# Rorisis/Co-Occ

Measured on AMD Instinct MI355X. Metric: samples/sec (6-cam frame + sweep -> occ+render), 200x200x16 grid, higher is better.
Workload: dtype f32 (split-f16 products, fp32 accumulate)

## Files before the change

co_occ_amd/_lib.py:

```python
import ctypes
import os
import threading
import time

import torch

_HERE = os.path.dirname(os.path.abspath(__file__))
LIB_PATH = os.path.join(_HERE, "libcoocc_hip.so")

c_int, c_float, c_void_p, c_size_t, c_int64 = (ctypes.c_int, ctypes.c_float, ctypes.c_void_p,
                                               ctypes.c_size_t, ctypes.c_int64)


class ConvDesc(ctypes.Structure):
    _fields_ = [(n, c_void_p) for n in ("in_", "w", "out", "scale", "bias", "res", "gather", "out_rows", "ws")] + \
               [("ws_floats", c_int64)] + \
               [(n, c_int) for n in ("M", "Cin", "Cout", "taps", "in_stride", "out_stride", "res_stride",
                                     "B", "Xi", "Yi", "Zi", "Xo", "Yo", "Zo", "ksize", "stride", "pad",
                                     "relu", "res_mode", "splitk", "tile_hint", "kx", "ky", "kz", "px", "py", "pz",
                                     "wgroup_rows", "mfma_dtype")] + [("alpha", ctypes.c_float), ("M_dev", c_void_p), ("gather_stride", c_int), ("out16", c_void_p), ("out16_stride", c_int), ("out_h2", c_int),
                                                                   ("out_h2_twin", c_void_p), ("tile_sem", c_void_p), ("tile_sem_ints", c_int),
                                                                  ("alpha_dev", c_void_p), ("sx", c_int), ("sy", c_int), ("sz", c_int)]


class SearchDesc(ctypes.Structure):
    _fields_ = [("cat4", c_void_p), ("pts", c_void_p), ("pts_rows", c_int), ("pts_stride", c_int)] + \
               [(n, c_int) for n in ("C", "X", "Y", "Z", "K", "fps_num", "max_cluster")] + \
               [("radius", ctypes.c_float), ("dist_thresh", ctypes.c_float), ("offsets", c_void_p), ("noff", c_int)] + \
               [(n, c_void_p) for n in ("lin", "counts", "near_img", "near_pts", "rows", "rows_p", "ws")] + \
               [("ws_bytes", ctypes.c_size_t), ("counts_host", c_void_p)]


P, I, F, Z, L = c_void_p, c_int, c_float, c_size_t, c_int64
SIGNATURES = {
    "coocc_last_error": (ctypes.c_char_p, []),
    "coocc_abi_version": (I, []),
    "coocc_device_cu_count": (I, [P]),
    "coocc_stream_create_cu_mask": (I, [P, I, P]),
    "coocc_stream_destroy": (I, [P]),
    "coocc_event_create": (I, [I, P]),
    "coocc_event_destroy": (I, [P]),
    "coocc_event_record": (I, [P, P]),
    "coocc_stream_wait_event": (I, [P, P]),
    "coocc_event_synchronize": (I, [P]),
    "coocc_event_query": (I, [P]),
    "coocc_event_elapsed_ms": (I, [P, P, P]),
    "coocc_ncdhw_to_ndhwc": (I, [P, P, I, I, I, I, I, P]),
    "coocc_rows_to_bf16": (I, [P, I, L, I, P, P]),
    "coocc_rows_to_h2": (I, [P, I, L, I, F, P, P]),
    "coocc_rows_to_h2_ex": (I, [P, I, L, I, F, P, P, P]),
    "coocc_rows_to_h2_gather": (I, [P, I, P, L, P, I, F, P, P]),
    "coocc_rows_to_f16": (I, [P, I, L, I, P, P]),
    "coocc_wino_input_h2": (I, [P, I, I, I, I, I, I, I, P, I, L, F, P]),
    "coocc_wino_input_h2_ex": (I, [P, I, I, I, I, I, I, I, P, I, L, F, P, P]),
    "coocc_ndhwc_to_ncdhw": (I, [P, P, I, I, I, I, I, P]),
    "coocc_fuser_prepare": (I, [P, P, P, P, P, I, I, I, P]),
    "coocc_fuser_prepare_rows": (I, [P, I, I, P, I, I, P, P, P, I, I, I, P]),
    "coocc_compact_flags": (I, [P, I, P, P, P, Z, P]),
    "coocc_compact_flags_ex": (I, [P, I, P, P, P, P, Z, P]),
    "coocc_lin_to_coords": (I, [P, I, I, I, I, P, P, P]),
    "coocc_furthest_point_sampling": (I, [I, I, I, P, P, P, P]),
    "coocc_fps_voxels_ws": (Z, [I, I, I]),
    "coocc_fps_voxels": (I, [P, I, I, I, I, I, P, P, Z, P]),
    "coocc_fps_voxels_pair": (I, [P, I, P, P, P, I, P, P, Z, I, I, I, I, P]),
    "coocc_ball_query": (I, [I, I, I, F, F, I, P, P, P, P]),
    "coocc_knn_topk": (I, [I, I, I, P, P, P, P, P]),
    "coocc_voxel_index_map": (I, [P, I, I, P, P]),
    "coocc_voxel_index_map_dev": (I, [P, I, P, I, P, P]),
    "coocc_fine_sample_voxel_dev": (I, [P, I, I, I, I, P, I, P, I, P, P, P, I, P]),
    "coocc_fine_sample_img_dev": (I, [P, I, I, I, I, P, P, L, P, P, I, I, P]),
    "coocc_fine_mlp_pre_dev": (I, [P, I, P, I, L, P, I, P, P, P, F, P, P, P, P, F, P, P, I, P, P]),
    "coocc_fine_fused": (I, [P, I, I, I, P, I, I, I, P, P, I, P, I, P, P, P, P, F, P, P, P, P, F, P, P, I, P, P, P]),
    "coocc_fine2_pack": (I, [P, P, I, P, P, P, P, P, P, P, P, P, P]),
    "coocc_fine2_h2": (I, [P, I, I, I, I, P, I, I, I, P, P, I, P, P, P, P, F, F, I, P, P, P, P]),
    "coocc_fine_sample_img_lin": (I, [P, I, I, I, I, P, P, I, I, I, P, P, I, I, P]),
    "coocc_scatter_fine_dev": (I, [P, L, P, I, I, I, P, P, I, I, I, F, P]),
    "coocc_scatter_fine_grouped": (I, [P, I, I, P, I, P, I, I, I, I, P, F, P, P]),
    "coocc_ball_query_voxels": (I, [I, F, F, I, I, I, I, P, P, P, P, P]),
    "coocc_knn_topk_voxels": (I, [I, I, I, I, I, I, P, P, P, P, I, P, P, P, P, P]),
    "coocc_knn_assign": (I, [I, I, I, I, F, P, P, P, P, P, P]),
    "coocc_knn_threshold": (I, [I, F, P, P, P, P]),
    "coocc_index_rows_i32": (I, [P, I, P, I, P, P]),
    "coocc_conv_pack_weights": (L, [P, I, I, I, I, P]),
    "coocc_conv_fwd": (I, [ctypes.POINTER(ConvDesc), P]),
    "coocc_fuser_search_ws": (Z, [ctypes.POINTER(SearchDesc)]),
    "coocc_fuser_search": (I, [ctypes.POINTER(SearchDesc), P, P]),
    "coocc_upsample_add_trilinear": (I, [P, P, I, I, I, I, I, I, I, I, P]),
    "coocc_upsample_add_trilinear_ex": (I, [P, P, I, I, I, I, I, I, I, I, P, P]),
    "coocc_occhead_mix": (I, [P, P, I, P, P, I, I, P]),
    "coocc_occhead_mix_ex": (I, [P, P, I, P, P, I, I, P, P]),
    "coocc_argmax_flags": (I, [P, I, I, I, I, P, P]),
    "coocc_fine_sample_voxel": (I, [P, I, I, I, I, P, I, I, P, P, P, I, P]),
    "coocc_fine_sample_img": (I, [P, I, I, I, I, P, P, L, P, I, I, P]),
    "coocc_fine_mlp_pre": (I, [P, I, P, I, L, P, P, P, F, P, P, P, P, F, P, P, I, P, P]),
    "coocc_fine_mlp": (I, [P, I, P, I, L, P, P, P, P, F, P, P, P, P, F, P, P, I, P, P]),
    "coocc_groupnorm_rows": (I, [P, L, I, I, I, P, P, F, I, P]),
    "coocc_groupnorm_nhwc": (I, [P, I, I, I, I, P, P, F, I, P]),
    "coocc_scatter_fine": (I, [P, L, I, I, P, P, I, I, I, F, P]),
    "coocc_camera_mats": (I, [P, P, P, P, P, P, I, I, I, I, P, P]),
    "coocc_get_geometry": (I, [P, P, P, P, I, I, I, I, P, P]),
    "coocc_bev_pool_forward": (I, [P, P, P, P, I, I, I, I, I, I, I, P, P]),
    "coocc_bev_pool_backward": (I, [P, P, P, P, I, I, I, I, I, I, I, P, P]),
    "coocc_voxel_pool_ws": (Z, [I, I]),
    "coocc_voxel_pool": (I, [P, P, I, I, I, P, I, I, I, I, P, I, P, Z, I, P]),
    "coocc_lift_splat": (I, [P, P, P, I, I, I, I, I, I, P, I, I, I, I, P, I, P, Z, I, P]),
    "coocc_lift_splat_cams": (I, [P, P, P, P, P, P, I, I, I, I, I, I, P, I, I, I, I, P, I, P, Z, I, P]),
    "coocc_lift_splat_reuse": (I, [P, P, I, I, I, I, I, I, I, I, I, P, I, P, Z, P]),
    "coocc_bev_pool_coords": (I, [P, P, I, I, I, I, I, I, P, I, P, Z, I, P]),
    "coocc_render_nearest": (I, [P, I, I, I, P, P, I, I, I, I, P, I, P, P]),
    "coocc_render_nearest_cams": (I, [P, I, I, I, P, P, P, P, P, I, I, I, I, P, I, P, P]),
    "coocc_render_activate_table": (I, [P, I, P]),
    "coocc_upsample_maps": (I, [P, I, I, I, I, P, P, P]),
    "coocc_volume_sampling": (I, [P, I, I, I, I, P, I, P, P, P, P]),
    "coocc_raw2outputs": (I, [P, P, I, I, I, F, F, P, P, P, P]),
    "coocc_render_losses": (I, [P, P, P, P, L, I, P, P, Z, P]),
    "coocc_conv_pack_weights_dev": (L, [P, I, I, I, I, P, P]),
    "coocc_wino_pack_weights_dev": (L, [P, I, I, I, I, P, P]),
    "coocc_wino_pack_weights_h2_dev": (L, [P, I, I, I, I, P, P]),
    "coocc_conv_pack_weights_h2_dev": (L, [P, I, I, I, I, P, P]),
    "coocc_wino_gradout": (I, [P, I, I, I, I, I, I, I, P, L, P]),
    "coocc_wino_ztap_table": (I, [L, I, P, P]),
    "coocc_wino_wgrad": (I, [P, P, L, I, I, I, I, P, P, I, P, L, P]),
    "coocc_rows_to_kh2": (I, [P, I, L, L, I, F, P, P, P]),
    "coocc_wino_operand_kh2": (I, [I, P, I, I, I, I, I, I, I, P, L, F, P, P]),
    "coocc_conv_wgrad_h2": (I, [P, P, L, I, I, F, P, P, I, P, L, P]),
    "coocc_wino_wgrad_h2": (I, [P, P, L, I, I, I, I, F, P, P, I, P, L, P]),
    "coocc_conv_tap_table": (I, [I, I, I, I, I, I, I, I, I, I, I, P, P]),
    "coocc_conv_epilogue_bwd": (I, [P, I, P, I, P, I, I, I, P, I, P, I, I, P, I, P, L, P]),
    "coocc_conv_epilogue_bwd_ex": (I, [P, I, P, I, P, I, I, I, P, I, P, I, I, P, I, P, L, P, P, F, P]),
    "coocc_conv_wgrad": (I, [P, I, I, P, I, P, I, I, I, I, P, I, P, L, P]),
    "coocc_conv_wgrad_h2t": (I, [P, I, I, P, I, P, I, I, I, I, P, P, I, P, L, P]),
    "coocc_gather_rows": (I, [P, I, P, I, I, P, I, P]),
    "coocc_scatter_add_rows": (I, [P, I, P, I, I, P, I, P]),
    "coocc_voxel_pool_bwd": (I, [P, I, P, I, I, I, P, I, I, I, I, P, P]),
    "coocc_lift_splat_bwd": (I, [P, I, P, P, P, I, I, I, I, I, I, P, I, I, I, I, P, P, P]),
    "coocc_render_nearest_bwd": (I, [P, I, I, I, P, P, I, I, I, I, P, P, P, P]),
    "coocc_upsample_maps_bwd": (I, [P, P, I, I, I, I, P, P]),
    "coocc_render_losses_bwd": (I, [P, P, P, P, L, I, P, P, P, P, P]),
    "coocc_upsample_trilinear_bwd": (I, [P, P, I, I, I, I, I, I, I, I, I, P]),
    "coocc_wino_input": (I, [P, I, I, I, I, I, I, I, P, L, P]),
    "coocc_wino_input_strided": (I, [P, I, I, I, I, I, I, I, P, I, L, P]),
    "coocc_sparse_tap_sum": (I, [P, P, I, I, I, I, I, P, P, I, I, P]),
    "coocc_wino_output": (I, [P, L, I, I, I, I, I, I, P, I, P, P, P, I, I, P]),
    "coocc_wino_output_ex": (I, [P, L, I, I, I, I, I, I, P, I, P, P, P, I, I, P, P]),
    "coocc_h2_overflow": (I, [I]),
    "coocc_device_fault": (I, [I]),
    "coocc_render_heads_h2": (I, [P, I, I, I, P, P, P, P, P, P, I, P, P, P, I, P]),
    "coocc_projection_params": (I, [P, P, P, P, P, P, I, P, P, P]),
    "coocc_occhead_mix_bwd": (I, [P, P, I, P, P, P, P, I, I, P]),
    "coocc_fine_sample_voxel_bwd": (I, [P, I, I, I, I, I, P, L, P, P, P]),
    "coocc_groupnorm_rows_bwd": (I, [P, P, P, L, I, I, I, P, F, I, P, P, P, P]),
    "coocc_fine_sample_img_bwd": (I, [P, I, I, I, I, I, P, P, L, P, P]),
    "coocc_groupnorm_nhwc_bwd": (I, [P, P, P, I, I, I, I, P, F, I, P, P, P, P]),
    "coocc_voxelize_ws": (Z, [I]),
    "coocc_voxelize_hard": (I, [P, I, I, P, P, I, I, P, P, P, P, P, Z, P]),
    "coocc_vfe_mean": (I, [P, P, I, I, I, I, P, I, P]),
    "coocc_sparse_index_map": (I, [P, I, I, I, I, P, P]),
    "coocc_sparse_conv_table": (I, [P, I, I, I, I, I, I, I, P, P, P]),
    "coocc_sparse_down_flags": (I, [P, I, I, I, I, I, I, I, P, P]),
    "coocc_sparse_conv_table3": (I, [P, I, I, I, I, I, I, I, I, I, I, I, I, I, P, P, P]),
    "coocc_sparse_down_flags3": (I, [P, I, I, I, I, I, I, I, I, I, I, I, I, I, I, I, I, P, P]),
    "coocc_sparse_lin_to_coors": (I, [P, I, I, I, I, P, P, P]),
    "coocc_bn_stats": (I, [P, I, I, I, P, P, P, Z, P]),
    "coocc_bn_apply": (I, [P, I, I, P, P, P, P, F, P, I, P, P]),
    "coocc_bn_backward": (I, [P, P, P, I, I, P, P, P, F, I, P, P, P, P, P, Z, P]),
    "coocc_bn_backward_sums": (I, [P, P, P, I, I, P, P, F, I, P, P, P, Z, P]),
    "coocc_bn_backward_dx": (I, [P, P, P, I, I, P, P, P, F, I, P, P, ctypes.c_double, P, P, P]),
    "coocc_predict_labels": (I, [P, L, L, L, L, I, I, I, I, I, I, I, P, P]),
    "coocc_eval_semantic": (I, [P, L, L, L, L, I, I, I, I, P, P, I, I, I, I, I, P, P]),
    "coocc_fpn_sum": (I, [P, P, I, I, I, I, I, I, P, I, P, P]),
    "coocc_zyx_to_rows": (I, [P, P, I, I, I, I, I, I, I, P]),
    "coocc_conv_tap_table3": (I, [I] * 17 + [P, P]),
    "coocc_fpn_sum_bwd": (I, [P, I, P, P, I, I, I, I, I, I, P]),
    "coocc_lidarseg_points": (I, [P, L, L, L, L, I, I, I, I, P, L, L, I, I, P, I, I, P, P, I, P, P]),
    "coocc_render_eval_stats": (L, [P, P, P, P, I, I, I, P, P, Z, P]),
    "coocc_render_panels": (I, [P, P, P, P, I, I, I, P, P]),
    "coocc_render_eval_ssim": (L, [P, P, I, I, I, ctypes.c_double, P, P, Z, P]),
    "coocc_sparse_dgrad_table3": (I, [P] + [I] * 16 + [P, P, P, P]),
    "coocc_bn_apply_ex": (I, [P, I, I, P, P, P, P, F, P, I, P, P, P]),
    "coocc_pool_labels": (I, [P, I, I, I, I, I, I, I, P, P]),
    "coocc_occ_loss_ws": (Z, [L, I]),
    "coocc_occ_loss_fwd": (I, [P, L, I, I, P, P, I, I, I, P, P, I, P, P, P, P, Z, P]),
    "coocc_occ_loss_bwd": (I, [P, L, I, I, P, P, I, P, P, P, P, I, P]),
    "coocc_nbr_table2d": (I, [I, I, I, I, P, P]),
    "coocc_dcn_cols": (I, [P, I, P, I, I, I, I, I, I, I, I, P, P]),
    "coocc_se_gate2": (I, [P, I, I, I, I, P, P, P, P, P]),
    "coocc_cam_mean_ws": (Z, [I, I, I]),
    "coocc_cam_mean": (I, [P, I, I, I, I, P, P, Z, P]),
    "coocc_cam_bias_relu": (I, [P, I, I, I, I, P, I, P]),
    "coocc_dcn_cols_bwd": (I, [P, I, P, I, I, I, I, I, I, I, I, P, P, P, P]),
    "coocc_se_gate2_bwd_ws": (Z, [I, I, I]),
    "coocc_se_gate2_bwd": (I, [P, I, I, I, I, P, P, P, P, P, P, P, P, Z, P]),
    "coocc_cam_sum": (I, [P, I, I, I, I, P, P, Z, P]),
    "coocc_cam_add": (I, [P, P, I, I, I, P, F, P]),
    "coocc_dropout_rows": (I, [P, P, L, I, F, P, P]),
    "coocc_img_stem": (I, [P, I, I, I, P, P, P, I, I, I, P, I, P, P]),
}

_lib = None


class KernelTimer:

    def __init__(self):
        self.enabled = False
        self.only = None
        self.records = []

    class _Region:
        def __init__(self, owner, tag, work):
            self.o, self.tag, self.work = owner, tag, work

        def __enter__(self):
            lvl = int(self.o.enabled)
            self.on = lvl >= 2 or (lvl == 1 and self.work > 0 and (self.o.only is None or self.tag.startswith(self.o.only)))
            if self.on:
                self.s = torch.cuda.Event(enable_timing=True)
                self.e = torch.cuda.Event(enable_timing=True)
                self.s.record()
            return self

        def __exit__(self, *a):
            if self.on:
                self.e.record()
                self.o.records.append((self.tag, self.work, self.s, self.e))
            return False

    def region(self, tag, work=0.0):
        return KernelTimer._Region(self, tag, work)

    def summary(self):
        out = {}
        for tag, work, s, e in self.records:
            d = out.setdefault(tag, dict(launches=0, ms=0.0, work=0.0))
            d["launches"] += 1
            d["ms"] += s.elapsed_time(e)
            d["work"] += work
        return out

    def reset(self):
        self.records = []


TIMER = KernelTimer()



def load():
    global _lib
    if _lib is not None:
        return _lib
    if not os.path.exists(LIB_PATH):
        raise ImportError(
            "co_occ_amd: %s is missing -- build it with `python -c 'import __graft_entry__ as g; g.build()'` "
            "(hipcc --offload-arch=gfx950).  There is no CPU fallback." % LIB_PATH)
    lib = ctypes.CDLL(LIB_PATH)
    for name, (res, args) in SIGNATURES.items():
        fn = getattr(lib, name)
        fn.restype, fn.argtypes = res, args
    if os.environ.get("COOCC_FPS_THREADS"):
        lib.coocc_fps_voxels_set_threads(int(os.environ["COOCC_FPS_THREADS"]))
    _lib = lib
    return lib


class CooccError(RuntimeError):
    code = None


class CooccArgError(CooccError):
    """COOCC_EINVAL / COOCC_ENOMEM: the library REFUSED the call (an argument or shape an entry point does not take, a
    workspace that is too small) before launching anything -- nothing ran, the caller may take another route."""


class CooccRangeError(CooccError):
    """The split-f16 engine's range guard fired (``core.check_h2_overflow``): kernels ran and their result is not trustworthy.
    Never a reason to fall back silently."""


def check(rc):
    if rc != 0:
        cls = CooccArgError if rc in (-1, -3) else CooccError
        e = cls("libcoocc_hip: %s (code %d)" % (load().coocc_last_error().decode(), rc))
        e.code = rc
        raise e


def _device_of(args):
    for a in args:
        t = getattr(a, "_keep", None)
        if t is not None:
            return t.device
    return None


_fns = {}


def call(name, *args):
    fn = _fns.get(name)
    if fn is None:
        fn = _fns[name] = getattr(load(), name)
    dev = _device_of(args)
    if dev is not None and dev.index != torch.cuda.current_device():
        with torch.cuda.device(dev):
            with TIMER.region(name):
                check(fn(*args, stream(dev)))
        return
    if not TIMER.enabled:
        rc = fn(*args, stream(dev))
        if rc:
            check(rc)
        return
    with TIMER.region(name):
        check(fn(*args, stream(dev)))


def conv_fwd(desc, device):
    fn = load().coocc_conv_fwd
    if device.index != torch.cuda.current_device():
        with torch.cuda.device(device):
            check(fn(ctypes.byref(desc), stream(device)))
    else:
        check(fn(ctypes.byref(desc), stream(device)))


_raw_stream = getattr(torch._C, "_cuda_getCurrentRawStream", None)


def stream(device=None):
    if _raw_stream is not None:
        idx = device.index if device is not None and device.index is not None else torch.cuda.current_device()
        return c_void_p(_raw_stream(idx))
    return c_void_p(torch.cuda.current_stream(device).cuda_stream)


class DevPtr(ctypes.c_void_p):
    """c_void_p that keeps its tensor alive until the foreign call has been issued, so that
    temporaries such as ``ptr(x.contiguous())`` cannot be recycled by the caching allocator
    while later arguments of the same call are still being built."""


def ptr(t, dtype=None, strided=False, offset=0):
    if t is None:
        return c_void_p(0)
    if not t.is_cuda:
        raise CooccError("co_occ_amd ops run on the GPU only; got a %s tensor (no CPU fallback)" % t.device)
    if dtype is not None and t.dtype != dtype:
        raise CooccError("expected %s, got %s" % (dtype, t.dtype))
    if not strided and not t.is_contiguous():
        raise CooccError("tensor must be contiguous")
    p = DevPtr(t.data_ptr() + offset * t.element_size())
    p._keep = t
    return p


_blocked = threading.local()


def host_read(t):
    t0 = time.perf_counter()
    v = t.tolist()
    _blocked.s = getattr(_blocked, "s", 0.0) + time.perf_counter() - t0
    return v


def blocked_seconds():
    return getattr(_blocked, "s", 0.0)


def host_f32(vals):
    return (c_float * len(vals))(*[float(v) for v in vals])


def host_i32(vals):
    return (c_int * len(vals))(*[int(v) for v in vals])
```

co_occ_amd/csrc/knn.hip:

```cpp
#include "common.h"

typedef unsigned long long u64;

__device__ __forceinline__ u64 shfl_xor_u64(u64 v, int m) {
  unsigned lo = (unsigned)v, hi = (unsigned)(v >> 32);
  lo = __shfl_xor(lo, m);
  hi = __shfl_xor(hi, m);
  return ((u64)hi << 32) | lo;
}
template <int CTRL>
__device__ __forceinline__ u64 dpp_u64(u64 v) {
  int lo = (int)(unsigned)v, hi = (int)(unsigned)(v >> 32);
  lo = __builtin_amdgcn_update_dpp(lo, lo, CTRL, 0xF, 0xF, false);
  hi = __builtin_amdgcn_update_dpp(hi, hi, CTRL, 0xF, 0xF, false);
  return ((u64)(unsigned)hi << 32) | (unsigned)lo;
}
__device__ __forceinline__ u64 readlane_u64(u64 v, int l) {
  unsigned lo = __builtin_amdgcn_readlane((int)(unsigned)v, l);
  unsigned hi = __builtin_amdgcn_readlane((int)(unsigned)(v >> 32), l);
  return ((u64)hi << 32) | lo;
}
#define U64MAX(a, b) ((a) > (b) ? (a) : (b))
#define U64MIN(a, b) ((a) < (b) ? (a) : (b))
__device__ __forceinline__ u64 wave_max_u64(u64 v) {
// ... 300 lines not shown
    }
    sx = gl & 1023; sy = (gl >> 10) & 1023; sz = gl >> 20;
    if (tid == 0) {
      const unsigned rr = (unsigned)(rmask - (g & rmask));
      const unsigned hi = rr / (unsigned)q, lo = rr - hi * (unsigned)q;
      const unsigned rev = L ? (__brev(hi) >> (32 - L)) : 0u;
      idx[j] = (int)((lo << L) | rev);
    }
    if (dbg) { long long c4 = clock64(); tA += c1 - c0; tM += c2 - c1; tB += c3 - c2; tT += c4 - c3; }
  }
  if (dbg && lane == 0) {
    long long* o = dbg + wave * 8;
    o[0] = tA; o[1] = tM; o[2] = tB; o[3] = tT; o[4] = 0; o[5] = nd;
  }
}

#define FPSR_SLOTS 40
struct FpsRegProblem { const int32_t* lin; const FpsCell* cell; int32_t* idx; int n, L, q, RB; };
struct FpsRegArgs { FpsRegProblem p[2]; int m, Y, Z, NBY, NBZ, NB; long long* dbg; };

__global__ __launch_bounds__(1024) void k_fps_voxels_reg(FpsRegArgs a) {
  constexpr int NW = 16;
  __builtin_amdgcn_s_setprio(3);
  __shared__ unsigned wbest[2][NW];
  __shared__ int wloc[2][NW];
  const FpsRegProblem pr = a.p[blockIdx.x];
  const int tid = threadIdx.x, lane = tid & 63, wave = __builtin_amdgcn_readfirstlane(tid >> 6);
  const int RB = pr.RB, Y = a.Y, Z = a.Z, NB = a.NB, m = a.m;
  const unsigned rmask = (1u << RB) - 1u;
  const unsigned tmax = (1u << (32 - RB)) - 1u;
  long long* dbg = a.dbg;
  long long tA = 0, tM = 0, tB = 0, tT = 0, nd = 0;

  typedef unsigned u32x32 __attribute__((ext_vector_type(32)));
  typedef unsigned u32x8 __attribute__((ext_vector_type(8)));
  u32x32 ca0, ca1;
  u32x8 cb0, cb1;
  unsigned key = 0;
  int org = 0, pos = 0;
  {
    const int b = lane * NW + wave;
    if (lane < FPSR_SLOTS && b < NB) {
      int bz = b % a.NBZ; int qq = b / a.NBZ;
      org = ((qq / a.NBY) * FT_X) | (((qq % a.NBY) * FT_Y) << 10) | ((bz * FT_Z) << 20);
    }
  }
#pragma unroll
  for (int i = 0; i < FPSR_SLOTS; ++i) {
    const int b = i * NW + wave;
    unsigned k0 = 0, k1 = 0;
    if (b < NB) {
      const int r0 = pr.cell[(size_t)b * FT_P + lane].r, r1 = pr.cell[(size_t)b * FT_P + lane + 64].r;
      k0 = r0 >= 0 ? ((tmax << RB) | (rmask - (unsigned)r0)) : 0u;
      k1 = r1 >= 0 ? ((tmax << RB) | (rmask - (unsigned)r1)) : 0u;
      const unsigned best = max(k0, k1);
      const int bp = k1 > k0 ? lane + 64 : lane;
      const unsigned wb = wave_max_key(best);
      const u64 own = __ballot(best == wb);
      const int wp = __builtin_amdgcn_readlane(bp, (int)__ffsll((long long)own) - 1);
      if (lane == i) { key = wb; pos = wp; }
    }
    if (i < 32) { ca0[i] = k0; ca1[i] = k1; }
    else { cb0[i - 32] = k0; cb1[i - 32] = k1; }
  }
  if (tid == 0) pr.idx[0] = 0;
  int sx, sy, sz;
  {
    int l = pr.lin[0];
    sz = l % Z; l /= Z;
    sy = l % Y; sx = l / Y;
  }

  for (int j = 1; j < m; ++j) {
    long long c0 = dbg ? clock64() : 0;
    bool d = false;
    if (key) {
      const int x0 = org & 1023, y0 = (org >> 10) & 1023, z0 = org >> 20;
      const int dx = max(max(x0 - sx, sx - (x0 + FT_X - 1)), 0);
      const int dy = max(max(y0 - sy, sy - (y0 + FT_Y - 1)), 0);
      const int dz = max(max(z0 - sz, sz - (z0 + FT_Z - 1)), 0);
      d = (unsigned)(__mul24(dx, dx) + __mul24(dy, dy) + __mul24(dz, dz)) < (key >> RB);
    }
    u64 bal = __ballot(d);
    nd += __popcll(bal);
    const int exb = (lane >> 5) - sx, eyb = ((lane >> 3) & 3) - sy, ezb = (lane & 7) - sz;
    while (bal) {
      const int s0 = __builtin_amdgcn_readfirstlane((int)__ffsll((long long)bal) - 1);
      bal &= bal - 1;
      const int o = __builtin_amdgcn_readlane(org, s0);
      const int ex = (o & 1023) + exb, ey = ((o >> 10) & 1023) + eyb, ez = (o >> 20) + ezb;
      const int yz = __mul24(ey, ey) + __mul24(ez, ez);
      const unsigned d0 = (unsigned)(__mul24(ex, ex) + yz), d1 = (unsigned)(__mul24(ex + 2, ex + 2) + yz);
      unsigned k0, k1;
      if (s0 < 32) { k0 = ca0[s0]; k1 = ca1[s0]; }
      else { k0 = cb0[s0 - 32]; k1 = cb1[s0 - 32]; }
      if (k0) k0 = (min(d0, k0 >> RB) << RB) | (k0 & rmask);
      if (k1) k1 = (min(d1, k1 >> RB) << RB) | (k1 & rmask);
      if (s0 < 32) { ca0[s0] = k0; ca1[s0] = k1; }
      else { cb0[s0 - 32] = k0; cb1[s0 - 32] = k1; }
      const unsigned best = max(k0, k1);
      const int bp = k1 > k0 ? lane + 64 : lane;
      const unsigned wb = wave_max_key(best);
      const int wp = __builtin_amdgcn_readlane(bp, (int)__ffsll((long long)__ballot(best == wb)) - 1);
      if (lane == s0) { key = wb; pos = wp; }
    }
    long long c1 = dbg ? clock64() : 0;
    const int loc = org + (pos >> 5) + (((pos >> 3) & 3) << 10) + ((pos & 7) << 20);
    const unsigned wb = wave_max_key(key);
    if (key == wb && wb) { wbest[j & 1][wave] = wb; wloc[j & 1][wave] = loc; }
    if (!wb && lane == 0) wbest[j & 1][wave] = 0;
    long long c2 = dbg ? clock64() : 0;
    lds_barrier();
    long long c3 = dbg ? clock64() : 0;
    const int li = lane & 15;
    const unsigned mine = wbest[j & 1][li];
    const int ml = wloc[j & 1][li];
    unsigned v = mine;
    v = max(v, dpp_u32<0xB1>(v));
    v = max(v, dpp_u32<0x4E>(v));
    v = max(v, dpp_u32<0x141>(v));
    v = max(v, dpp_u32<0x140>(v));
    const unsigned g = (unsigned)__builtin_amdgcn_readfirstlane((int)v);
    const u64 own = __ballot(mine == g) & 0xFFFFull;
    const int gl = __builtin_amdgcn_readlane(ml, (int)__ffsll((long long)own) - 1);
    sx = gl & 1023; sy = (gl >> 10) & 1023; sz = gl >> 20;
    if (tid == 0) pr.idx[j] = (int)(g & rmask);
    if (dbg) { long long c4 = clock64(); tA += c1 - c0; tM += c2 - c1; tB += c3 - c2; tT += c4 - c3; }
  }
  __syncthreads();
  for (int j = 1 + tid; j < m; j += 1024) {
    const unsigned rr = rmask - (unsigned)pr.idx[j];
    const unsigned hi = rr / (unsigned)pr.q, lo = rr - hi * (unsigned)pr.q;
    const unsigned rev = pr.L ? (__brev(hi) >> (32 - pr.L)) : 0u;
    pr.idx[j] = (int)((lo << pr.L) | rev);
  }
  if (dbg && lane == 0 && blockIdx.x == 0) {
    long long* o = dbg + wave * 8;
    o[0] = tA; o[1] = tM; o[2] = tB; o[3] = tT; o[4] = 0; o[5] = nd;
  }
}

extern "C" size_t coocc_fps_voxels_ws(int X, int Y, int Z) {
  size_t nb = (size_t)((X + FT_X - 1) / FT_X) * ((Y + FT_Y - 1) / FT_Y) * ((Z + FT_Z - 1) / FT_Z);
  return nb * FT_P * sizeof(FpsCell);
}

static int g_fps_threads = 1024;
static long long* g_fps_dbg = nullptr;
extern "C" void coocc_fps_voxels_set_debug(long long* p) { g_fps_dbg = p; }
extern "C" void coocc_fps_voxels_set_threads(int t) { g_fps_threads = t; }

struct FpsPrep { int NBX, NBY, NBZ, L, q, RB, tinit, threads, R; long long NB; bool key32; };

static int fps_prepare(const int32_t* lin, int n, int X, int Y, int Z, int m, const int32_t* idx, void* ws, size_t ws_bytes,
                       hipStream_t s, FpsPrep* o) {
  COOCC_CHECK_ARG(lin && idx && ws && n > 0 && m >= 0 && X > 0 && Y > 0 && Z > 0, "fps_voxels: bad args");
  COOCC_CHECK_ARG(n < (1 << FPS_KBITS), "fps_voxels: n must be < 2^22");
  COOCC_CHECK_ARG(X <= 1020 && Y <= 1020 && Z <= 1016, "fps_voxels: grid dims must fit 10-bit packed coordinates");
  o->NBX = (X + FT_X - 1) / FT_X; o->NBY = (Y + FT_Y - 1) / FT_Y; o->NBZ = (Z + FT_Z - 1) / FT_Z;
  o->NB = (long long)o->NBX * o->NBY * o->NBZ;
  int threads = g_fps_threads;
  while (o->NB > 8ll * threads && threads < 1024) threads *= 2;
  COOCC_CHECK_ARG(o->NB <= 8ll * threads, "fps_voxels: grid has too many buckets (use coocc_furthest_point_sampling)");
  if (ws_bytes < coocc_fps_voxels_ws(X, Y, Z)) return coocc_set_error(COOCC_ENOMEM, "fps_voxels: workspace too small");
  o->threads = threads;
  o->R = (int)((o->NB + threads - 1) / threads);
  int L = 0;
  while ((2 << L) <= n && L < 10) ++L;
  const int q = (n + (1 << L) - 1) >> L;
  int RB = L;
  while ((1ll << RB) <= ((long long)q << L)) ++RB;
  const long long d2max = (long long)(X - 1) * (X - 1) + (long long)(Y - 1) * (Y - 1) + (long long)(Z - 1) * (Z - 1);
  o->key32 = RB < 31 && d2max + 1 < (1ll << (32 - RB)) - 1;
  o->tinit = o->key32 ? (int)((1u << (32 - RB)) - 1u) : 0x7FFFFFFF;
  o->L = L; o->q = q; o->RB = RB;
  if (m == 0) return COOCC_OK;
  FpsCell* cell = (FpsCell*)ws;
  COOCC_HIP(hipMemsetAsync(cell, 0xFF, sizeof(FpsCell) * (size_t)o->NB * FT_P, s));
  hipLaunchKernelGGL(k_fpsv_scatter, dim3(cdiv(n, 256)), dim3(256), 0, s, lin, n, Y, Z, o->NBY, o->NBZ, L, q, o->tinit, cell);
  COOCC_LAUNCH_CHECK("k_fpsv_scatter");
  return COOCC_OK;
}

static int g_fps_reg = -1;
static bool fps_reg_ok(const FpsPrep& o) {
  if (g_fps_reg < 0) g_fps_reg = getenv("COOCC_FPS_REG") ? atoi(getenv("COOCC_FPS_REG")) : 1;
  return g_fps_reg && o.key32 && o.NB <= (long long)FPSR_SLOTS * 16;
}

extern "C" int coocc_fps_voxels(const int32_t* lin, int n, int X, int Y, int Z, int m, int32_t* idx, void* ws,
                                size_t ws_bytes, void* stream) {
  hipStream_t s = as_stream(stream);
  FpsPrep o;
  int rc = fps_prepare(lin, n, X, Y, Z, m, idx, ws, ws_bytes, s, &o);
  if (rc != COOCC_OK || m == 0) return rc;
  FpsCell* cell = (FpsCell*)ws;
  const int NBY = o.NBY, NBZ = o.NBZ, L = o.L, q = o.q, RB = o.RB, R = o.R, threads = o.threads;
  const long long NB = o.NB;
  const bool key32 = o.key32;
  if (fps_reg_ok(o)) {
    FpsRegArgs a = {};
    a.p[0] = FpsRegProblem{lin, cell, idx, n, L, q, RB};
    a.m = m; a.Y = Y; a.Z = Z; a.NBY = NBY; a.NBZ = NBZ; a.NB = (int)NB; a.dbg = g_fps_dbg;
    hipLaunchKernelGGL(k_fps_voxels_reg, dim3(1), dim3(1024), 0, s, a);
    COOCC_LAUNCH_CHECK("k_fps_voxels_reg");
    return COOCC_OK;
  }
#define FPS_LAUNCH(T, RM, KT) \
  hipLaunchKernelGGL((k_fps_voxels<T, RM, KT>), dim3(1), dim3(T), 0, s, n, m, Y, Z, NBY, NBZ, (int)NB, lin, cell, idx, L, q, \
                     key32 ? RB : 32, g_fps_dbg)
#define FPS_PICK_R(T, KT)                     \
  do {                                        \
    if (R <= 2) FPS_LAUNCH(T, 2, KT);         \
    else if (R <= 3) FPS_LAUNCH(T, 3, KT);    \
    else if (R <= 4) FPS_LAUNCH(T, 4, KT);    \
    else if (R <= 5) FPS_LAUNCH(T, 5, KT);    \
    else if (R <= 6) FPS_LAUNCH(T, 6, KT);    \
    else FPS_LAUNCH(T, 8, KT);                \
  } while (0)
#define FPS_PICK(T)                           \
  do {                                        \
    if (key32) FPS_PICK_R(T, unsigned);       \
    else FPS_PICK_R(T, u64);                  \
  } while (0)
  if (threads == 256) FPS_PICK(256);
  else if (threads == 512) FPS_PICK(512);
  else FPS_PICK(1024);
  COOCC_LAUNCH_CHECK("k_fps_voxels");
  return COOCC_OK;
}

extern "C" int coocc_fps_voxels_pair(const int32_t* lin0, int n0, int32_t* idx0, void* ws0, const int32_t* lin1, int n1, int32_t* idx1,
                                     void* ws1, size_t ws_bytes_each, int X, int Y, int Z, int m, void* stream) {
  COOCC_CHECK_ARG(X > 0 && Y > 0 && Z > 0 && n0 > 0 && n1 > 0, "fps_voxels_pair: bad args");
  {
    const long long NB = (long long)((X + FT_X - 1) / FT_X) * ((Y + FT_Y - 1) / FT_Y) * ((Z + FT_Z - 1) / FT_Z);
    if (NB > (long long)FPSR_SLOTS * 16) return 2;
    const long long d2max = (long long)(X - 1) * (X - 1) + (long long)(Y - 1) * (Y - 1) + (long long)(Z - 1) * (Z - 1);
    for (int n : {n0, n1}) {
      int L = 0;
      while ((2 << L) <= n && L < 10) ++L;
      const int q = (n + (1 << L) - 1) >> L;
      int RB = L;
      while ((1ll << RB) <= ((long long)q << L)) ++RB;
      if (!(RB < 31 && d2max + 1 < (1ll << (32 - RB)) - 1)) return 2;
    }
    if (g_fps_reg < 0) g_fps_reg = getenv("COOCC_FPS_REG") ? atoi(getenv("COOCC_FPS_REG")) : 1;
    if (!g_fps_reg) return 2;
  }
  hipStream_t s = as_stream(stream);
  FpsPrep o0, o1;
  int rc = fps_prepare(lin0, n0, X, Y, Z, m, idx0, ws0, ws_bytes_each, s, &o0);
  if (rc != COOCC_OK) return rc;
  rc = fps_prepare(lin1, n1, X, Y, Z, m, idx1, ws1, ws_bytes_each, s, &o1);
  if (rc != COOCC_OK || m == 0) return rc;
  FpsRegArgs a = {};
  a.p[0] = FpsRegProblem{lin0, (const FpsCell*)ws0, idx0, n0, o0.L, o0.q, o0.RB};
  a.p[1] = FpsRegProblem{lin1, (const FpsCell*)ws1, idx1, n1, o1.L, o1.q, o1.RB};
  a.m = m; a.Y = Y; a.Z = Z; a.NBY = o0.NBY; a.NBZ = o0.NBZ; a.NB = (int)o0.NB; a.dbg = g_fps_dbg;
  hipLaunchKernelGGL(k_fps_voxels_reg, dim3(2), dim3(1024), 0, s, a);
  COOCC_LAUNCH_CHECK("k_fps_voxels_reg");
  return COOCC_OK;
}

__global__ __launch_bounds__(256) void k_ball_query(int n, int m, float min_r2, float max_r2, int nsample,
                                                     const float* __restrict__ new_xyz_all,
                                                     const float* __restrict__ xyz_all,
                                                     int32_t* __restrict__ idx_all) {
  const int lane = threadIdx.x & 63;
  const int c = blockIdx.x * 4 + (threadIdx.x >> 6);
  if (c >= m) return;
  const float* new_xyz = new_xyz_all + ((size_t)blockIdx.y * m + c) * 3;
  const float* xyz = xyz_all + (size_t)blockIdx.y * n * 3;
  int32_t* idx = idx_all + ((size_t)blockIdx.y * m + c) * nsample;
  const float cx = new_xyz[0], cy = new_xyz[1], cz = new_xyz[2];
  int cnt = 0, first = 0;
  for (int base = 0; base < n && cnt < nsample; base += 64) {
    int k = base + lane;
    bool hit = false;
    if (k < n) {
      float d2 = sqdist3(xyz[k * 3 + 0], xyz[k * 3 + 1], xyz[k * 3 + 2], cx, cy, cz);
      hit = (d2 == 0.f) || (d2 >= min_r2 && d2 < max_r2);
    }
    u64 bal = __ballot(hit);
    if (bal) {
      if (cnt == 0) first = base + (int)__ffsll((long long)bal) - 1;
      int slot = cnt + __popcll(bal & ((1ull << lane) - 1ull));
      if (hit && slot < nsample) idx[slot] = k;
      cnt += __popcll(bal);
    }
  }
  if (cnt > nsample) cnt = nsample;
  for (int l = cnt + lane; l < nsample; l += 64) idx[l] = first;
}

extern "C" int coocc_ball_query(int b, int n, int m, float min_radius, float max_radius, int nsample,
                                const float* new_xyz, const float* xyz, int32_t* idx, void* stream) {
  COOCC_CHECK_ARG(new_xyz && xyz && idx && b > 0 && n > 0 && m > 0 && nsample > 0, "ball_query: bad args");
  dim3 grid(cdiv(m, 4), b);
  hipLaunchKernelGGL(k_ball_query, grid, dim3(256), 0, as_stream(stream), n, m, min_radius * min_radius,
                     max_radius * max_radius, nsample, new_xyz, xyz, idx);
  COOCC_LAUNCH_CHECK("k_ball_query");
  return COOCC_OK;
}

template <int K>
__global__ __launch_bounds__(256) void k_knn_topk(int nq, int nk, const float* __restrict__ q,
                                                   const float* __restrict__ key, float* __restrict__ val,
                                                   int32_t* __restrict__ idx) {
  const int lane = threadIdx.x & 63;
  const int r = blockIdx.x * 4 + (threadIdx.x >> 6);
  if (r >= nq) return;
  const float qx = q[r * 3 + 0], qy = q[r * 3 + 1], qz = q[r * 3 + 2];
  u64 best[K];
#pragma unroll
  for (int j = 0; j < K; ++j) best[j] = ~0ull;
  for (int k = lane; k < nk; k += 64) {
    float d2 = sqdist3(qx, qy, qz, key[k * 3 + 0], key[k * 3 + 1], key[k * 3 + 2]);
    u64 kk = ((u64)__float_as_uint(d2) << 32) | (unsigned)k;
    if (kk < best[K - 1]) {
      best[K - 1] = kk;
#pragma unroll
      for (int j = K - 1; j > 0; --j) {
        if (best[j] < best[j - 1]) { u64 t = best[j]; best[j] = best[j - 1]; best[j - 1] = t; }
      }
    }
  }
#pragma unroll
  for (int o = 0; o < K; ++o) {
    u64 mn = wave_min_u64(best[0]);
    if (best[0] == mn) {
#pragma unroll
      for (int j = 0; j < K - 1; ++j) best[j] = best[j + 1];
      best[K - 1] = ~0ull;
    }
    if (lane == 0) {
      val[(size_t)r * K + o] = (float)__dsqrt_rn((double)__uint_as_float((unsigned)(mn >> 32)));
      idx[(size_t)r * K + o] = (int32_t)(unsigned)mn;
    }
  }
}

extern "C" int coocc_knn_topk(int nq, int nk, int K, const float* q, const float* key, float* val,
                              int32_t* idx, void* stream) {
  COOCC_CHECK_ARG(q && key && val && idx && nq > 0 && nk > 0, "knn_topk: bad args");
  COOCC_CHECK_ARG(K >= 1 && K <= 8 && K <= nk, "knn_topk: need 1 <= K <= min(8, nk)");
  dim3 grid(cdiv(nq, 4)), block(256);
  hipStream_t s = as_stream(stream);
  switch (K) {
    case 1: hipLaunchKernelGGL(k_knn_topk<1>, grid, block, 0, s, nq, nk, q, key, val, idx); break;
    case 2: hipLaunchKernelGGL(k_knn_topk<2>, grid, block, 0, s, nq, nk, q, key, val, idx); break;
    case 3: hipLaunchKernelGGL(k_knn_topk<3>, grid, block, 0, s, nq, nk, q, key, val, idx); break;
    case 4: hipLaunchKernelGGL(k_knn_topk<4>, grid, block, 0, s, nq, nk, q, key, val, idx); break;
    case 5: hipLaunchKernelGGL(k_knn_topk<5>, grid, block, 0, s, nq, nk, q, key, val, idx); break;
    case 6: hipLaunchKernelGGL(k_knn_topk<6>, grid, block, 0, s, nq, nk, q, key, val, idx); break;
    case 7: hipLaunchKernelGGL(k_knn_topk<7>, grid, block, 0, s, nq, nk, q, key, val, idx); break;
    default: hipLaunchKernelGGL(k_knn_topk<8>, grid, block, 0, s, nq, nk, q, key, val, idx); break;
  }
  COOCC_LAUNCH_CHECK("k_knn_topk");
  return COOCC_OK;
}

__global__ __launch_bounds__(256) void k_index_map_scatter(const int32_t* __restrict__ lin, int n, int32_t* __restrict__ map,
                                                            const int32_t* __restrict__ n_dev) {
  if (n_dev) n = min(n, *n_dev);
  int i = blockIdx.x * blockDim.x + threadIdx.x;
  if (i < n) map[lin[i]] = i;
}

__global__ __launch_bounds__(256) void k_fill_i32(int32_t* __restrict__ p, int n, int32_t v) {
  const int i = blockIdx.x * blockDim.x + threadIdx.x;
  if (i < n) p[i] = v;
}

extern "C" int coocc_voxel_index_map_dev(const int32_t* lin, int n_cap, const int32_t* n_dev, int nvox, int32_t* map, void* stream) {
  COOCC_CHECK_ARG(map && nvox > 0 && n_cap > 0 && lin && n_dev, "voxel_index_map_dev: bad args");
  static const bool fill_kernel = !(getenv("COOCC_MAP_MEMSET") && atoi(getenv("COOCC_MAP_MEMSET")) == 1);
  if (fill_kernel) hipLaunchKernelGGL(k_fill_i32, dim3(cdiv(nvox, 256)), dim3(256), 0, as_stream(stream), map, nvox, -1);
  else COOCC_HIP(hipMemsetAsync(map, 0xFF, (size_t)nvox * 4, as_stream(stream)));
  hipLaunchKernelGGL(k_index_map_scatter, dim3(cdiv(n_cap, 256)), dim3(256), 0, as_stream(stream), lin, n_cap, map, n_dev);
  COOCC_LAUNCH_CHECK("k_index_map_scatter");
  return COOCC_OK;
}

extern "C" int coocc_voxel_index_map(const int32_t* lin, int n, int nvox, int32_t* map, void* stream) {
  COOCC_CHECK_ARG(map && nvox > 0 && n >= 0 && (lin || n == 0), "voxel_index_map: bad args");
  COOCC_HIP(hipMemsetAsync(map, 0xFF, (size_t)nvox * 4, as_stream(stream)));
  if (n) {
    hipLaunchKernelGGL(k_index_map_scatter, dim3(cdiv(n, 256)), dim3(256), 0, as_stream(stream), lin, n, map, (const int32_t*)nullptr);
    COOCC_LAUNCH_CHECK("k_index_map_scatter");
  }
  return COOCC_OK;
}

__global__ __launch_bounds__(256) void k_ball_query_vox(int m, float min_r2, float max_r2, int R, int nsample, int X, int Y, int Z,
                                                         const int32_t* __restrict__ centre_ord, const int32_t* __restrict__ lin_q,
                                                         const int32_t* __restrict__ map_q, int32_t* __restrict__ idx_all) {
  const int lane = threadIdx.x & 63;
  const int c = blockIdx.x * 4 + (threadIdx.x >> 6);
  if (c >= m) return;
  int32_t* idx = idx_all + (size_t)c * nsample;
  const int v0 = lin_q[centre_ord[c]];
  const int cz = v0 % Z, cy = (v0 / Z) % Y, cx = v0 / (Z * Y);
  const int x0 = max(cx - R, 0), x1 = min(cx + R, X - 1);
  const int y0 = max(cy - R, 0), y1 = min(cy + R, Y - 1);
  const int z0 = max(cz - R, 0), z1 = min(cz + R, Z - 1);
  const int wy = y1 - y0 + 1, wz = z1 - z0 + 1;
  const int total = (x1 - x0 + 1) * wy * wz;
  int cnt = 0, first = 0;
  for (int base = 0; base < total && cnt < nsample; base += 64) {
    const int t = base + lane;
    bool hit = false;
    int ord = -1;
    if (t < total) {
      const int iz = z0 + t % wz, r = t / wz;
      const int iy = y0 + r % wy, ix = x0 + r / wy;
      ord = map_q[(ix * Y + iy) * Z + iz];
      const float d2 = sqdist3((float)ix, (float)iy, (float)iz, (float)cx, (float)cy, (float)cz);
      hit = ord >= 0 && ((d2 == 0.f) || (d2 >= min_r2 && d2 < max_r2));
    }
    const u64 bal = __ballot(hit);
    if (bal) {
      if (cnt == 0) first = __shfl(ord, (int)__ffsll((long long)bal) - 1);
      const int slot = cnt + __popcll(bal & ((1ull << lane) - 1ull));
      if (hit && slot < nsample) idx[slot] = ord;
      cnt += __popcll(bal);
    }
  }
  if (cnt > nsample) cnt = nsample;
  for (int l = cnt + lane; l < nsample; l += 64) idx[l] = first;
}

extern "C" int coocc_ball_query_voxels(int m, float min_radius, float max_radius, int nsample, int X, int Y, int Z,
                                       const int32_t* centre_ord, const int32_t* lin_q, const int32_t* map_q, int32_t* idx,
                                       void* stream) {
  COOCC_CHECK_ARG(m > 0 && nsample > 0 && X > 0 && Y > 0 && Z > 0 && centre_ord && lin_q && map_q && idx, "ball_query_voxels: bad args");
  COOCC_CHECK_ARG(max_radius >= 0.f && max_radius < 4096.f, "ball_query_voxels: bad radius");
  const float max_r2 = max_radius * max_radius;
  int R = (int)ceilf(max_radius);
  while (R > 0 && (float)(R * R) >= max_r2) --R;
  hipLaunchKernelGGL(k_ball_query_vox, dim3(cdiv(m, 4)), dim3(256), 0, as_stream(stream), m, min_radius * min_radius, max_r2, R,
                     nsample, X, Y, Z, centre_ord, lin_q, map_q, idx);
  COOCC_LAUNCH_CHECK("k_ball_query_vox");
  return COOCC_OK;
}

template <int K>
__global__ __launch_bounds__(256) void k_knn_topk_vox(int nq, int X, int Y, int Z, const int32_t* __restrict__ rep_ord,
                                                       const int32_t* __restrict__ lin_q, const int32_t* __restrict__ map_k,
                                                       const uint32_t* __restrict__ offsets, int noff, float* __restrict__ val,
                                                       int32_t* __restrict__ idx) {
  const int lane = threadIdx.x & 63;
  const int r = blockIdx.x * 4 + (threadIdx.x >> 6);
  if (r >= nq) return;
  const int v0 = lin_q[rep_ord[r]];
  const int cz = v0 % Z, cy = (v0 / Z) % Y, cx = v0 / (Z * Y);
  int found = 0;
  for (int base = 0; base < noff && found < K; base += 64) {
    const int t = base + lane;
    int ord = -1;
    float d2 = 0.f;
    if (t < noff) {
      const uint32_t o = offsets[t];
      const int dx = (int)(o & 255u) - 128, dy = (int)((o >> 8) & 255u) - 128, dz = (int)((o >> 16) & 255u) - 128;
      const int ix = cx + dx, iy = cy + dy, iz = cz + dz;
      if ((unsigned)ix < (unsigned)X && (unsigned)iy < (unsigned)Y && (unsigned)iz < (unsigned)Z) {
        ord = map_k[(ix * Y + iy) * Z + iz];
        d2 = sqdist3((float)cx, (float)cy, (float)cz, (float)ix, (float)iy, (float)iz);
      }
    }
    const u64 bal = __ballot(ord >= 0);
    const int p = found + __popcll(bal & ((1ull << lane) - 1ull));
    if (ord >= 0 && p < K) {
      val[(size_t)r * K + p] = (float)__dsqrt_rn((double)d2);
      idx[(size_t)r * K + p] = ord;
    }
    found += __popcll(bal);
  }
  if (found < K && lane == 0) idx[(size_t)r * K] = -2;
}

template <int K>
__global__ __launch_bounds__(256) void k_knn_topk_unresolved(int nq, int nk, const float* __restrict__ q,
                                                              const float* __restrict__ key, float* __restrict__ val,
                                                              int32_t* __restrict__ idx) {
  const int lane = threadIdx.x & 63;
  const int r = blockIdx.x * 4 + (threadIdx.x >> 6);
  if (r >= nq || idx[(size_t)r * K] != -2) return;
  const float qx = q[r * 3 + 0], qy = q[r * 3 + 1], qz = q[r * 3 + 2];
  u64 best[K];
#pragma unroll
  for (int j = 0; j < K; ++j) best[j] = ~0ull;
  for (int k = lane; k < nk; k += 64) {
    float d2 = sqdist3(qx, qy, qz, key[k * 3 + 0], key[k * 3 + 1], key[k * 3 + 2]);
    u64 kk = ((u64)__float_as_uint(d2) << 32) | (unsigned)k;
    if (kk < best[K - 1]) {
      best[K - 1] = kk;
#pragma unroll
      for (int j = K - 1; j > 0; --j) {
        if (best[j] < best[j - 1]) { u64 t = best[j]; best[j] = best[j - 1]; best[j - 1] = t; }
      }
    }
  }
#pragma unroll
  for (int o = 0; o < K; ++o) {
    u64 mn = wave_min_u64(best[0]);
    if (best[0] == mn) {
#pragma unroll
      for (int j = 0; j < K - 1; ++j) best[j] = best[j + 1];
      best[K - 1] = ~0ull;
    }
    if (lane == 0) {
      val[(size_t)r * K + o] = (float)__dsqrt_rn((double)__uint_as_float((unsigned)(mn >> 32)));
      idx[(size_t)r * K + o] = (int32_t)(unsigned)mn;
    }
  }
}

template <int K>
static void launch_topk_vox(int nq, int nk, int X, int Y, int Z, const int32_t* rep_ord, const int32_t* lin_q, const int32_t* map_k,
                            const uint32_t* offsets, int noff, const float* q, const float* key, float* val, int32_t* idx,
                            hipStream_t s) {
  hipLaunchKernelGGL(k_knn_topk_vox<K>, dim3(cdiv(nq, 4)), dim3(256), 0, s, nq, X, Y, Z, rep_ord, lin_q, map_k, offsets, noff, val, idx);
  hipLaunchKernelGGL(k_knn_topk_unresolved<K>, dim3(cdiv(nq, 4)), dim3(256), 0, s, nq, nk, q, key, val, idx);
}

extern "C" int coocc_knn_topk_voxels(int nq, int nk, int K, int X, int Y, int Z, const int32_t* rep_ord, const int32_t* lin_q,
                                     const int32_t* map_k, const uint32_t* offsets, int noff, const float* q, const float* key,
                                     float* val, int32_t* idx, void* stream) {
  COOCC_CHECK_ARG(nq > 0 && nk > 0 && X > 0 && Y > 0 && Z > 0 && rep_ord && lin_q && map_k && offsets && noff > 0 && q && key &&
                      val && idx, "knn_topk_voxels: bad args");
  COOCC_CHECK_ARG(K >= 1 && K <= 8 && K <= nk, "knn_topk_voxels: need 1 <= K <= min(8, nk)");
  hipStream_t s = as_stream(stream);
  switch (K) {
    case 1: launch_topk_vox<1>(nq, nk, X, Y, Z, rep_ord, lin_q, map_k, offsets, noff, q, key, val, idx, s); break;
    case 2: launch_topk_vox<2>(nq, nk, X, Y, Z, rep_ord, lin_q, map_k, offsets, noff, q, key, val, idx, s); break;
    case 3: launch_topk_vox<3>(nq, nk, X, Y, Z, rep_ord, lin_q, map_k, offsets, noff, q, key, val, idx, s); break;
    case 4: launch_topk_vox<4>(nq, nk, X, Y, Z, rep_ord, lin_q, map_k, offsets, noff, q, key, val, idx, s); break;
    case 5: launch_topk_vox<5>(nq, nk, X, Y, Z, rep_ord, lin_q, map_k, offsets, noff, q, key, val, idx, s); break;
    case 6: launch_topk_vox<6>(nq, nk, X, Y, Z, rep_ord, lin_q, map_k, offsets, noff, q, key, val, idx, s); break;
    case 7: launch_topk_vox<7>(nq, nk, X, Y, Z, rep_ord, lin_q, map_k, offsets, noff, q, key, val, idx, s); break;
    default: launch_topk_vox<8>(nq, nk, X, Y, Z, rep_ord, lin_q, map_k, offsets, noff, q, key, val, idx, s); break;
  }
  COOCC_LAUNCH_CHECK("k_knn_topk_vox");
  return COOCC_OK;
}

__global__ void k_assign_winner(int nc, int K, int ns, int nq, float thresh, const float* __restrict__ val,
                                const int32_t* __restrict__ group, int32_t* __restrict__ winner) {
  int i = blockIdx.x * blockDim.x + threadIdx.x;
  if (i >= nc * ns) return;
  int c = i / ns;
  int qi = group[i];
  if (i != c * ns && qi == group[c * ns]) return;
  for (int k = 0; k < K; ++k)
    if (val[c * K + k] < thresh) atomicMax(&winner[(size_t)k * nq + qi], c);
}

__global__ void k_assign_lookup(int K, int nq, const int32_t* __restrict__ nn,
                                const int32_t* __restrict__ winner, int32_t* __restrict__ out) {
  int i = blockIdx.x * blockDim.x + threadIdx.x;
  if (i >= K * nq) return;
  int k = i / nq;
  int w = winner[i];
  out[i] = w >= 0 ? nn[w * K + k] : -1;
}

extern "C" int coocc_knn_assign(int nc, int K, int ns, int nq, float dist_thresh, const float* val,
                                const int32_t* nn, const int32_t* group, int32_t* winner, int32_t* out,
                                void* stream) {
  COOCC_CHECK_ARG(val && nn && group && winner && out && nc > 0 && K > 0 && ns > 0 && nq > 0, "knn_assign: bad args");
  hipStream_t s = as_stream(stream);
  COOCC_HIP(hipMemsetAsync(winner, 0xFF, sizeof(int32_t) * (size_t)K * nq, s));
  hipLaunchKernelGGL(k_assign_winner, dim3(cdiv((long long)nc * ns, 256)), dim3(256), 0, s, nc, K, ns, nq,
                     dist_thresh, val, group, winner);
  hipLaunchKernelGGL(k_assign_lookup, dim3(cdiv((long long)K * nq, 256)), dim3(256), 0, s, K, nq, nn, winner, out);
  COOCC_LAUNCH_CHECK("knn_assign");
  return COOCC_OK;
}

__global__ void k_knn_threshold(int nq, float thresh, const float* __restrict__ val,
                                const int32_t* __restrict__ nn, int32_t* __restrict__ out) {
  int i = blockIdx.x * blockDim.x + threadIdx.x;
  if (i < nq) out[i] = val[i] < thresh ? nn[i] : -1;
}

extern "C" int coocc_knn_threshold(int nq, float dist_thresh, const float* val, const int32_t* nn,
                                   int32_t* out, void* stream) {
  COOCC_CHECK_ARG(val && nn && out && nq > 0, "knn_threshold: bad args");
  hipLaunchKernelGGL(k_knn_threshold, dim3(cdiv(nq, 256)), dim3(256), 0, as_stream(stream), nq, dist_thresh, val, nn, out);
  COOCC_LAUNCH_CHECK("k_knn_threshold");
  return COOCC_OK;
}

__global__ void k_index_rows(const int32_t* __restrict__ base, int nbase, const int32_t* __restrict__ sel, int n,
                             int32_t* __restrict__ rows) {
  int i = blockIdx.x * blockDim.x + threadIdx.x;
  if (i >= n) return;
  int s = sel[i];
  if (s < 0) s += nbase;
  rows[i] = (s >= 0 && s < nbase) ? base[s] : -1;
}

extern "C" int coocc_index_rows_i32(const int32_t* base, int nbase, const int32_t* sel, int n, int32_t* rows,
                                    void* stream) {
  COOCC_CHECK_ARG(base && sel && rows && nbase > 0 && n >= 0, "index_rows: bad args");
  if (n == 0) return COOCC_OK;
  hipLaunchKernelGGL(k_index_rows, dim3(cdiv(n, 256)), dim3(256), 0, as_stream(stream), base, nbase, sel, n, rows);
  COOCC_LAUNCH_CHECK("k_index_rows");
  return COOCC_OK;
}
```

co_occ_amd/csrc/layout.hip:

```cpp
#include <stdarg.h>
#include <stdlib.h>

#include "common.h"

typedef float f32x4 __attribute__((ext_vector_type(4)));

static thread_local char g_err[512] = "";

int coocc_set_error(int code, const char* fmt, ...) {
  va_list ap;
  va_start(ap, fmt);
  vsnprintf(g_err, sizeof(g_err), fmt, ap);
  va_end(ap);
  return code;
}

extern "C" const char* coocc_last_error(void) { return g_err; }
extern "C" int coocc_abi_version(void) { return 1; }

#define TV 64
#define TC 128

__global__ __launch_bounds__(256) void k_ncdhw_to_ndhwc(const float* __restrict__ src,
                                                         float* __restrict__ dst, int C, int V,
                                                         int dst_stride, int dst_coff) {
  __shared__ float tile[TV][TC + 1];
  const int b = blockIdx.y;
  const int v0 = blockIdx.x * TV;
  const int t = threadIdx.x;
  const int c0 = blockIdx.z * TC;
  const int cn = min(TC, C - c0);
  if (cn == TC) {
    const int v = v0 + (t & 63);
    const float* sp = src + ((size_t)b * C + c0 + (t >> 6)) * V + v;
    float r[TC / 4];
#pragma unroll
    for (int k = 0; k < TC / 4; ++k) r[k] = v < V ? sp[(size_t)(4 * k) * V] : 0.f;
#pragma unroll
    for (int k = 0; k < TC / 4; ++k) tile[t & 63][(t >> 6) + 4 * k] = r[k];
    __syncthreads();
#pragma unroll 8
    for (int i = t; i < TV * TC; i += 256) {
      const int vv = i >> 7, c = i & (TC - 1);
      if (v0 + vv < V) dst[((size_t)b * V + v0 + vv) * dst_stride + dst_coff + c0 + c] = tile[vv][c];
    }
    return;
  }
  for (int c = t >> 6; c < cn; c += 4) {
    int v = v0 + (t & 63);
    tile[t & 63][c] = v < V ? src[((size_t)b * C + c0 + c) * V + v] : 0.f;
  }
  __syncthreads();
  for (int i = t; i < TV * cn; i += 256) {
    int v = i / cn, c = i - v * cn;
    if (v0 + v < V) dst[((size_t)b * V + v0 + v) * dst_stride + dst_coff + c0 + c] = tile[v][c];
  }
}

__global__ __launch_bounds__(256) void k_ndhwc_to_ncdhw(const float* __restrict__ src,
                                                         float* __restrict__ dst, int C, int V,
                                                         int src_stride, int src_coff) {
  __shared__ float tile[TV][TC + 1];
  const int b = blockIdx.y;
  const int v0 = blockIdx.x * TV;
  const int t = threadIdx.x;
  for (int c0 = 0; c0 < C; c0 += TC) {
    const int cn = min(TC, C - c0);
    for (int i = t; i < TV * cn; i += 256) {
      int v = i / cn, c = i - v * cn;
      tile[v][c] = (v0 + v < V) ? src[((size_t)b * V + v0 + v) * src_stride + src_coff + c0 + c] : 0.f;
    }
    __syncthreads();
    for (int c = t >> 6; c < cn; c += 4) {
      int v = v0 + (t & 63);
      if (v < V) dst[((size_t)b * C + c0 + c) * V + v] = tile[t & 63][c];
    }
    __syncthreads();
  }
}

extern "C" int coocc_ncdhw_to_ndhwc(const float* src, float* dst, int B, int C, int V, int dst_stride,
                                    int dst_coff, void* stream) {
  COOCC_CHECK_ARG(src && dst && B > 0 && C > 0 && V > 0 && dst_stride >= dst_coff + C, "ncdhw_to_ndhwc: bad args");
  dim3 grid(cdiv(V, TV), B, cdiv(C, TC));
  hipLaunchKernelGGL(k_ncdhw_to_ndhwc, grid, dim3(256), 0, as_stream(stream), src, dst, C, V, dst_stride, dst_coff);
  COOCC_LAUNCH_CHECK("k_ncdhw_to_ndhwc");
  return COOCC_OK;
}

extern "C" int coocc_ndhwc_to_ncdhw(const float* src, float* dst, int B, int C, int V, int src_stride,
                                    int src_coff, void* stream) {
  COOCC_CHECK_ARG(src && dst && B > 0 && C > 0 && V > 0 && src_stride >= src_coff + C, "ndhwc_to_ncdhw: bad args");
  dim3 grid(cdiv(V, TV), B);
  hipLaunchKernelGGL(k_ndhwc_to_ncdhw, grid, dim3(256), 0, as_stream(stream), src, dst, C, V, src_stride, src_coff);
  COOCC_LAUNCH_CHECK("k_ndhwc_to_ncdhw");
  return COOCC_OK;
}

__global__ __launch_bounds__(256) void k_fuser_prepare(const float* __restrict__ img,
                                                        const float* __restrict__ pts,
                                                        float* __restrict__ cat4,
                                                        uint8_t* __restrict__ flag_img,
                                                        uint8_t* __restrict__ flag_pts, int C, int V) {
  __shared__ float tile[TV][TC + 1];
  const int b = blockIdx.y;
  const int v0 = blockIdx.x * TV;
  const int t = threadIdx.x;
  const int stride = 4 * C;
  for (int mod = 0; mod < 2; ++mod) {
    const float* src = mod ? pts : img;
    uint8_t* flags = mod ? flag_pts : flag_img;
    float rsum = 0.f;
    for (int c0 = 0; c0 < C; c0 += TC) {
      const int cn = min(TC, C - c0);
      for (int c = t >> 6; c < cn; c += 4) {
        int v = v0 + (t & 63);
        tile[t & 63][c] = v < V ? src[((size_t)b * C + c0 + c) * V + v] : 0.f;
      }
      __syncthreads();
      if (t < TV)
        for (int c = 0; c < cn; ++c) rsum += tile[t][c];
      for (int i = t; i < TV * cn; i += 256) {
        int v = i / cn, c = i - v * cn;
        if (v0 + v < V) cat4[((size_t)b * V + v0 + v) * stride + mod * C + c0 + c] = tile[v][c];
      }
      __syncthreads();
    }
    if (t < TV && v0 + t < V) flags[(size_t)b * V + v0 + t] = rsum != 0.f ? 1 : 0;
  }
  for (int i = t; i < TV * 2 * C; i += 256) {
    int v = i / (2 * C), c = i - v * 2 * C;
    if (v0 + v < V) cat4[((size_t)b * V + v0 + v) * stride + 2 * C + c] = 0.f;
  }
}

extern "C" int coocc_fuser_prepare(const float* img, const float* pts, float* cat4, uint8_t* flag_img,
                                   uint8_t* flag_pts, int B, int C, int V, void* stream) {
  COOCC_CHECK_ARG(img && pts && cat4 && flag_img && flag_pts && B > 0 && C > 0 && V > 0, "fuser_prepare: bad args");
  dim3 grid(cdiv(V, TV), B);
  hipLaunchKernelGGL(k_fuser_prepare, grid, dim3(256), 0, as_stream(stream), img, pts, cat4, flag_img, flag_pts, C, V);
  COOCC_LAUNCH_CHECK("k_fuser_prepare");
  return COOCC_OK;
}

__global__ __launch_bounds__(256) void k_fuser_prepare_rows(const float* __restrict__ img, int img_rows, int img_stride,
                                                             const float* __restrict__ pts, int pts_rows, int pts_stride,
                                                             float* __restrict__ cat4, uint8_t* __restrict__ flag_img,
                                                             uint8_t* __restrict__ flag_pts, int C, int V) {
  __shared__ float tile[TV][TC + 1];
  const int b = blockIdx.y;
  const int v0 = blockIdx.x * TV;
  const int t = threadIdx.x;
  const int stride = 4 * C;
  for (int mod = 0; mod < 2; ++mod) {
    const float* src = mod ? pts : img;
    const int rows = mod ? pts_rows : img_rows, sstride = mod ? pts_stride : img_stride;
    uint8_t* flags = mod ? flag_pts : flag_img;
    const bool in_place = rows && src == cat4 + mod * C && sstride == stride;
    float rsum = 0.f;
    for (int c0 = 0; c0 < C; c0 += TC) {
      const int cn = min(TC, C - c0);
      if (rows) {
        if (cn == TC) {
          for (int i = t; i < TV * (TC / 4); i += 256) {
            const int v = i / (TC / 4), c = (i % (TC / 4)) * 4;
            f32x4 q = {0.f, 0.f, 0.f, 0.f};
            if (v0 + v < V) q = *(const f32x4*)(src + ((size_t)b * V + v0 + v) * sstride + c0 + c);
            tile[v][c] = q[0]; tile[v][c + 1] = q[1]; tile[v][c + 2] = q[2]; tile[v][c + 3] = q[3];
          }
        } else {
          for (int i = t; i < TV * cn; i += 256) {
            int v = i / cn, c = i - v * cn;
            tile[v][c] = v0 + v < V ? src[((size_t)b * V + v0 + v) * sstride + c0 + c] : 0.f;
          }
        }
      } else {
        for (int c = t >> 6; c < cn; c += 4) {
          int v = v0 + (t & 63);
          tile[t & 63][c] = v < V ? src[((size_t)b * C + c0 + c) * V + v] : 0.f;
        }
      }
      __syncthreads();
      if (t < TV)
        for (int c = 0; c < cn; ++c) rsum += tile[t][c];
      if (!in_place)
        for (int i = t; i < TV * cn; i += 256) {
          int v = i / cn, c = i - v * cn;
          if (v0 + v < V) cat4[((size_t)b * V + v0 + v) * stride + mod * C + c0 + c] = tile[v][c];
        }
      __syncthreads();
    }
    if (t < TV && v0 + t < V) flags[(size_t)b * V + v0 + t] = rsum != 0.f ? 1 : 0;
  }
  for (int i = t; i < TV * 2 * C; i += 256) {
    int v = i / (2 * C), c = i - v * 2 * C;
    if (v0 + v < V) cat4[((size_t)b * V + v0 + v) * stride + 2 * C + c] = 0.f;
  }
}

constexpr int FV = 256, FC = 32;
__global__ __launch_bounds__(256) void k_fuser_prepare_rows_fast(const float* __restrict__ img, int img_rows, int img_stride,
                                                                  const float* __restrict__ pts, int pts_rows, int pts_stride,
                                                                  float* __restrict__ cat4, uint8_t* __restrict__ flag_img,
                                                                  uint8_t* __restrict__ flag_pts, int C, int V) {
  __shared__ float tile[FV][FC + 1];
  const int b = blockIdx.y;
  const int v0 = blockIdx.x * FV;
  const int t = threadIdx.x;
  const int stride = 4 * C;
  const int rv = t >> 3, rc = (t & 7) * 4;
  for (int mod = 0; mod < 2; ++mod) {
    const float* src = mod ? pts : img;
    const int rows = mod ? pts_rows : img_rows, sstride = mod ? pts_stride : img_stride;
    uint8_t* flags = mod ? flag_pts : flag_img;
    const bool in_place = rows && src == cat4 + mod * C && sstride == stride;
    float rsum = 0.f;
    for (int c0 = 0; c0 < C; c0 += FC) {
      if (rows) {
#pragma unroll
        for (int ps = 0; ps < FV / 32; ++ps) {
          const int v = ps * 32 + rv;
          f32x4 q = {0.f, 0.f, 0.f, 0.f};
          if (v0 + v < V) q = *(const f32x4*)(src + ((size_t)b * V + v0 + v) * sstride + c0 + rc);
          tile[v][rc] = q[0]; tile[v][rc + 1] = q[1]; tile[v][rc + 2] = q[2]; tile[v][rc + 3] = q[3];
        }
        __syncthreads();
#pragma unroll
        for (int c = 0; c < FC; ++c) rsum += tile[t][c];
      } else {
#pragma unroll 8
        for (int c = 0; c < FC; ++c) {
          const float x = v0 + t < V ? src[((size_t)b * C + c0 + c) * V + v0 + t] : 0.f;
          rsum += x;
          tile[t][c] = x;
        }
        __syncthreads();
      }
      if (!in_place) {
#pragma unroll
        for (int ps = 0; ps < FV / 32; ++ps) {
          const int v = ps * 32 + rv;
          if (v0 + v < V) {
            const f32x4 q = {tile[v][rc], tile[v][rc + 1], tile[v][rc + 2], tile[v][rc + 3]};
            *(f32x4*)(cat4 + ((size_t)b * V + v0 + v) * stride + mod * C + c0 + rc) = q;
          }
        }
      }
      __syncthreads();
    }
    if (v0 + t < V) flags[(size_t)b * V + v0 + t] = rsum != 0.f ? 1 : 0;
  }
  const int vec_per_row = C >> 1;
  const f32x4 z = {0.f, 0.f, 0.f, 0.f};
  if (vec_per_row <= 256 && 256 % vec_per_row == 0) {
    const int vpp = 256 / vec_per_row, tv = t / vec_per_row, c = (t - tv * vec_per_row) * 4;
    for (int v = tv; v < FV; v += vpp)
      if (v0 + v < V) *(f32x4*)(cat4 + ((size_t)b * V + v0 + v) * stride + 2 * C + c) = z;
  } else {
    for (int i = t; i < FV * vec_per_row; i += 256) {
      const int v = i / vec_per_row, c = (i - v * vec_per_row) * 4;
      if (v0 + v < V) *(f32x4*)(cat4 + ((size_t)b * V + v0 + v) * stride + 2 * C + c) = z;
    }
  }
}

extern "C" int coocc_fuser_prepare_rows(const float* img, int img_rows, int img_stride, const float* pts, int pts_rows,
                                        int pts_stride, float* cat4, uint8_t* flag_img, uint8_t* flag_pts, int B, int C, int V,
                                        void* stream) {
  COOCC_CHECK_ARG(img && pts && cat4 && flag_img && flag_pts && B > 0 && C > 0 && V > 0, "fuser_prepare_rows: bad args");
  COOCC_CHECK_ARG((!img_rows || img_stride >= C) && (!pts_rows || pts_stride >= C), "fuser_prepare_rows: row stride < C");
  const bool vec_ok = C % FC == 0 && ((uintptr_t)cat4 & 15) == 0 && (!img_rows || (img_stride % 4 == 0 && ((uintptr_t)img & 15) == 0)) &&
                      (!pts_rows || (pts_stride % 4 == 0 && ((uintptr_t)pts & 15) == 0));
  if (vec_ok) {
    hipLaunchKernelGGL(k_fuser_prepare_rows_fast, dim3(cdiv(V, FV), B), dim3(256), 0, as_stream(stream), img, img_rows, img_stride,
                       pts, pts_rows, pts_stride, cat4, flag_img, flag_pts, C, V);
    COOCC_LAUNCH_CHECK("k_fuser_prepare_rows_fast");
    return COOCC_OK;
  }
  dim3 grid(cdiv(V, TV), B);
  hipLaunchKernelGGL(k_fuser_prepare_rows, grid, dim3(256), 0, as_stream(stream), img, img_rows, img_stride, pts, pts_rows,
                     pts_stride, cat4, flag_img, flag_pts, C, V);
  COOCC_LAUNCH_CHECK("k_fuser_prepare_rows");
  return COOCC_OK;
}

#define CB 1024

__global__ __launch_bounds__(256) void k_flag_count(const uint8_t* __restrict__ flags, int total,
                                                     int32_t* __restrict__ blk) {
  __shared__ int wsum[4];
  int base = blockIdx.x * CB + threadIdx.x * 4;
  int c = 0;
  for (int j = 0; j < 4; ++j)
    if (base + j < total) c += flags[base + j] != 0;
  for (int o = 32; o > 0; o >>= 1) c += __shfl_down(c, o);
  if ((threadIdx.x & 63) == 0) wsum[threadIdx.x >> 6] = c;
  __syncthreads();
  if (threadIdx.x == 0) blk[blockIdx.x] = wsum[0] + wsum[1] + wsum[2] + wsum[3];
}

__global__ __launch_bounds__(1024) void k_scan_blocks(int32_t* __restrict__ blk, int nblk,
                                                       int32_t* __restrict__ count) {
  __shared__ int wsum[16];
  __shared__ int carry_s;
  if (threadIdx.x == 0) carry_s = 0;
  __syncthreads();
  for (int base = 0; base < nblk; base += 1024) {
    int i = base + threadIdx.x;
    int v = i < nblk ? blk[i] : 0;
    int inc = v;
    for (int o = 1; o < 64; o <<= 1) {
      int n = __shfl_up(inc, o);
      if ((threadIdx.x & 63) >= o) inc += n;
    }
    if ((threadIdx.x & 63) == 63) wsum[threadIdx.x >> 6] = inc;
    __syncthreads();
    int woff = 0;
    for (int w = 0; w < (int)(threadIdx.x >> 6); ++w) woff += wsum[w];
    int carry = carry_s;
    if (i < nblk) blk[i] = carry + woff + inc - v;
    __syncthreads();
    if (threadIdx.x == 1023) carry_s = carry + woff + inc;
    __syncthreads();
  }
  if (threadIdx.x == 0) *count = carry_s;
}

__global__ __launch_bounds__(256) void k_flag_write(const uint8_t* __restrict__ flags, int total,
                                                     const int32_t* __restrict__ blk,
                                                     int32_t* __restrict__ lin, int32_t* __restrict__ map) {
  __shared__ int wsum[4];
  int base = blockIdx.x * CB + threadIdx.x * 4;
  int f[4], c = 0;
  for (int j = 0; j < 4; ++j) {
    f[j] = (base + j < total) && flags[base + j] != 0;
    c += f[j];
  }
  int inc = c;
  for (int o = 1; o < 64; o <<= 1) {
    int n = __shfl_up(inc, o);
    if ((threadIdx.x & 63) >= o) inc += n;
  }
  if ((threadIdx.x & 63) == 63) wsum[threadIdx.x >> 6] = inc;
  __syncthreads();
  int off = blk[blockIdx.x] + inc - c;
  for (int w = 0; w < (int)(threadIdx.x >> 6); ++w) off += wsum[w];
  for (int j = 0; j < 4; ++j) {
    if (map && base + j < total) map[base + j] = f[j] ? off : -1;
    if (f[j]) lin[off++] = base + j;
  }
}

__device__ __forceinline__ int block_sum256(int v, int* s) {
  for (int o = 32; o > 0; o >>= 1) v += __shfl_xor(v, o);
  __syncthreads();
  if ((threadIdx.x & 63) == 0) s[threadIdx.x >> 6] = v;
  __syncthreads();
  return s[0] + s[1] + s[2] + s[3];
}

__device__ __forceinline__ int nonzero_bytes(uint32_t x) {
  return __popc((((x & 0x7f7f7f7fu) + 0x7f7f7f7fu) | x) & 0x80808080u);
}

#define ONE_PASS_MAX (128 * CB)
#define TWO_PASS_MAX_BLOCKS 2048
template <bool FROM_FLAGS>
__global__ __launch_bounds__(256) void k_flag_write_px(const uint8_t* __restrict__ flags, int total,
                                                        const int32_t* __restrict__ blk, int32_t* __restrict__ count,
                                                        int32_t* __restrict__ lin, int32_t* __restrict__ map) {
  __shared__ int wsum[4], psum[4];
  int before = 0;
  if (FROM_FLAGS) {
    const uint4* w = (const uint4*)flags;
    const int nw = blockIdx.x * (CB / 16);
    for (int i0 = threadIdx.x; i0 < nw; i0 += 256 * 8) {
      uint4 x[8];
#pragma unroll
      for (int k = 0; k < 8; ++k) x[k] = i0 + k * 256 < nw ? w[i0 + k * 256] : make_uint4(0u, 0u, 0u, 0u);
#pragma unroll
      for (int k = 0; k < 8; ++k) before += nonzero_bytes(x[k].x) + nonzero_bytes(x[k].y) + nonzero_bytes(x[k].z) + nonzero_bytes(x[k].w);
    }
  } else {
    for (int i = threadIdx.x; i < (int)blockIdx.x; i += 256) before += blk[i];
  }
  before = block_sum256(before, psum);
  int base = blockIdx.x * CB + threadIdx.x * 4;
  int f[4], c = 0;
  for (int j = 0; j < 4; ++j) {
    f[j] = (base + j < total) && flags[base + j] != 0;
    c += f[j];
  }
  int inc = c;
  for (int o = 1; o < 64; o <<= 1) {
    int n = __shfl_up(inc, o);
    if ((threadIdx.x & 63) >= o) inc += n;
  }
  if ((threadIdx.x & 63) == 63) wsum[threadIdx.x >> 6] = inc;
  __syncthreads();
  int off = before + inc - c;
  for (int w = 0; w < (int)(threadIdx.x >> 6); ++w) off += wsum[w];
  if (blockIdx.x == gridDim.x - 1 && threadIdx.x == 255) *count = off + c;
  for (int j = 0; j < 4; ++j) {
    if (map && base + j < total) map[base + j] = f[j] ? off : -1;
    if (f[j]) lin[off++] = base + j;
  }
}

extern "C" int coocc_compact_flags_ex(const uint8_t* flags, int total, int32_t* lin, int32_t* count, int32_t* map, void* ws,
                                      size_t ws_bytes, void* stream);
extern "C" int coocc_compact_flags(const uint8_t* flags, int total, int32_t* lin, int32_t* count, void* ws,
                                   size_t ws_bytes, void* stream) {
  return coocc_compact_flags_ex(flags, total, lin, count, nullptr, ws, ws_bytes, stream);
}
extern "C" int coocc_compact_flags_ex(const uint8_t* flags, int total, int32_t* lin, int32_t* count, int32_t* map, void* ws,
                                      size_t ws_bytes, void* stream) {
  COOCC_CHECK_ARG(flags && lin && count && ws && total > 0, "compact_flags: bad args");
  int nblk = (int)cdiv(total, CB);
  if (ws_bytes < sizeof(int32_t) * (size_t)nblk) return coocc_set_error(COOCC_ENOMEM, "compact_flags: workspace too small");
  int32_t* blk = (int32_t*)ws;
  const char* e = getenv("COOCC_COMPACT_SCAN");
  if (e && e[0] == '1') {
    hipLaunchKernelGGL(k_flag_count, dim3(nblk), dim3(256), 0, as_stream(stream), flags, total, blk);
    hipLaunchKernelGGL(k_scan_blocks, dim3(1), dim3(1024), 0, as_stream(stream), blk, nblk, count);
    hipLaunchKernelGGL(k_flag_write, dim3(nblk), dim3(256), 0, as_stream(stream), flags, total, blk, lin, map);
  } else if (total <= ONE_PASS_MAX && ((uintptr_t)flags & 15) == 0) {
    hipLaunchKernelGGL(k_flag_write_px<true>, dim3(nblk), dim3(256), 0, as_stream(stream), flags, total, blk, count, lin, map);
  } else if (nblk <= TWO_PASS_MAX_BLOCKS) {
    hipLaunchKernelGGL(k_flag_count, dim3(nblk), dim3(256), 0, as_stream(stream), flags, total, blk);
    hipLaunchKernelGGL(k_flag_write_px<false>, dim3(nblk), dim3(256), 0, as_stream(stream), flags, total, blk, count, lin, map);
  } else {
    hipLaunchKernelGGL(k_flag_count, dim3(nblk), dim3(256), 0, as_stream(stream), flags, total, blk);
    hipLaunchKernelGGL(k_scan_blocks, dim3(1), dim3(1024), 0, as_stream(stream), blk, nblk, count);
    hipLaunchKernelGGL(k_flag_write, dim3(nblk), dim3(256), 0, as_stream(stream), flags, total, blk, lin, map);
  }
  COOCC_LAUNCH_CHECK("compact_flags");
  return COOCC_OK;
}

__global__ void k_lin_to_coords(const int32_t* __restrict__ lin, int n, int X, int Y, int Z,
                                float* __restrict__ xyz, int64_t* __restrict__ bxyz) {
  int i = blockIdx.x * blockDim.x + threadIdx.x;
  if (i >= n) return;
  int l = lin[i];
  int z = l % Z; l /= Z;
  int y = l % Y; l /= Y;
  int x = l % X; int b = l / X;
  if (xyz) { xyz[i * 3 + 0] = (float)x; xyz[i * 3 + 1] = (float)y; xyz[i * 3 + 2] = (float)z; }
  if (bxyz) { bxyz[i * 4 + 0] = b; bxyz[i * 4 + 1] = x; bxyz[i * 4 + 2] = y; bxyz[i * 4 + 3] = z; }
}

extern "C" int coocc_lin_to_coords(const int32_t* lin, int n, int X, int Y, int Z, float* xyz, int64_t* bxyz,
                                   void* stream) {
  COOCC_CHECK_ARG(lin && n >= 0 && X > 0 && Y > 0 && Z > 0, "lin_to_coords: bad args");
  if (n == 0) return COOCC_OK;
  hipLaunchKernelGGL(k_lin_to_coords, dim3(cdiv(n, 256)), dim3(256), 0, as_stream(stream), lin, n, X, Y, Z, xyz, bxyz);
  COOCC_LAUNCH_CHECK("k_lin_to_coords");
  return COOCC_OK;
}

extern "C" int coocc_device_cu_count(int* n) {
  COOCC_CHECK_ARG(n, "device_cu_count: null");
  int dev = 0;
  COOCC_HIP(hipGetDevice(&dev));
  hipDeviceProp_t prop;
  COOCC_HIP(hipGetDeviceProperties(&prop, dev));
  *n = prop.multiProcessorCount;
  return COOCC_OK;
}

extern "C" int coocc_stream_create_cu_mask(const uint32_t* mask_host, int nwords, void** stream_out) {
  COOCC_CHECK_ARG(mask_host && nwords > 0 && stream_out, "stream_create_cu_mask: bad args");
  hipStream_t s = nullptr;
  COOCC_HIP(hipExtStreamCreateWithCUMask(&s, (uint32_t)nwords, mask_host));
  *stream_out = (void*)s;
  return COOCC_OK;
}

extern "C" int coocc_stream_destroy(void* stream) {
  COOCC_CHECK_ARG(stream, "stream_destroy: null");
  COOCC_HIP(hipStreamDestroy(as_stream(stream)));
  return COOCC_OK;
}

extern "C" int coocc_event_create(int flags, void** event_out) {
  COOCC_CHECK_ARG(event_out && (flags & ~3) == 0, "event_create: bad args");
  hipEvent_t e = nullptr;
  COOCC_HIP(hipEventCreateWithFlags(&e, hipEventDisableSystemFence | ((flags & 1) ? 0u : hipEventDisableTiming) |
                                            ((flags & 2) ? hipEventBlockingSync : 0u)));
  *event_out = (void*)e;
  return COOCC_OK;
}
extern "C" int coocc_event_destroy(void* event) {
  COOCC_CHECK_ARG(event, "event_destroy: null");
  COOCC_HIP(hipEventDestroy((hipEvent_t)event));
  return COOCC_OK;
}
extern "C" int coocc_event_record(void* event, void* stream) {
  COOCC_CHECK_ARG(event, "event_record: null");
  COOCC_HIP(hipEventRecord((hipEvent_t)event, as_stream(stream)));
  return COOCC_OK;
}
extern "C" int coocc_stream_wait_event(void* stream, void* event) {
  COOCC_CHECK_ARG(event, "stream_wait_event: null");
  COOCC_HIP(hipStreamWaitEvent(as_stream(stream), (hipEvent_t)event, 0));
  return COOCC_OK;
}
extern "C" int coocc_event_synchronize(void* event) {
  COOCC_CHECK_ARG(event, "event_synchronize: null");
  COOCC_HIP(hipEventSynchronize((hipEvent_t)event));
  return COOCC_OK;
}
extern "C" int coocc_event_query(void* event) {
  COOCC_CHECK_ARG(event, "event_query: null");
  const hipError_t e = hipEventQuery((hipEvent_t)event);
  if (e == hipSuccess) return 1;
  if (e == hipErrorNotReady) { (void)hipGetLastError(); return 0; }
  return coocc_set_error(COOCC_EHIP, "hipEventQuery failed: %s", hipGetErrorString(e));
}
extern "C" int coocc_event_elapsed_ms(void* start, void* stop, float* ms) {
  COOCC_CHECK_ARG(start && stop && ms, "event_elapsed_ms: null");
  COOCC_HIP(hipEventElapsedTime(ms, (hipEvent_t)start, (hipEvent_t)stop));
  return COOCC_OK;
}
```

co_occ_amd/csrc/search.hip:

```cpp
#include <stdlib.h>
#include <string.h>

#include "common.h"

__global__ __launch_bounds__(256) void k_gather_xyz(const float* __restrict__ xyz, const int32_t* __restrict__ idx, int m,
                                                     float* __restrict__ out) {
  const int i = blockIdx.x * blockDim.x + threadIdx.x;
  if (i >= m) return;
  const int s = idx[i];
  out[i * 3 + 0] = xyz[s * 3 + 0]; out[i * 3 + 1] = xyz[s * 3 + 1]; out[i * 3 + 2] = xyz[s * 3 + 2];
}

static size_t align256(size_t v) { return (v + 255) & ~(size_t)255; }

struct SearchWs {
  uint8_t* flags;
  int32_t* cws;
  float* xyz;
  int32_t* maps;
  int32_t* rep[2];
  float* rep_xyz[2];
  float* val[2];
  int32_t* nn[2];
  int32_t* group[2];
  int32_t* winner[2];
  void* fps[2];
  size_t fps_bytes;
  size_t total;
};

static SearchWs carve(char* base, int V, int K, int fps_num, int max_cluster, int X, int Y, int Z) {
  SearchWs w;
  size_t o = 0;
  auto take = [&](size_t bytes) { char* p = base ? base + o : nullptr; o += align256(bytes); return p; };
  w.flags = (uint8_t*)take((size_t)2 * V);
  w.cws = (int32_t*)take((size_t)2 * (V / 1024 + 2) * 4);
  w.xyz = (float*)take((size_t)2 * V * 3 * 4);
  w.maps = (int32_t*)take((size_t)2 * V * 4);
  w.fps_bytes = coocc_fps_voxels_ws(X, Y, Z);
  for (int d = 0; d < 2; ++d) {
    w.rep[d] = (int32_t*)take((size_t)fps_num * 4);
    w.rep_xyz[d] = (float*)take((size_t)fps_num * 3 * 4);
    w.val[d] = (float*)take((size_t)fps_num * K * 4);
    w.nn[d] = (int32_t*)take((size_t)fps_num * K * 4);
    w.group[d] = (int32_t*)take((size_t)fps_num * max_cluster * 4);
    w.winner[d] = (int32_t*)take((size_t)K * V * 4);
    w.fps[d] = take(w.fps_bytes);
  }
  w.total = o;
  return w;
}

extern "C" size_t coocc_fuser_search_ws(const coocc_search_desc* d) {
  if (!d || d->X <= 0 || d->Y <= 0 || d->Z <= 0 || d->K <= 0) return 0;
  return carve(nullptr, d->X * d->Y * d->Z, d->K, d->fps_num, d->max_cluster, d->X, d->Y, d->Z).total;
}

#define SRC(call)                    \
  do {                               \
    int rc__ = (call);               \
    if (rc__ != COOCC_OK) return rc__; \
  } while (0)

extern "C" int coocc_fuser_search(coocc_search_desc* d, void* stream, void* side_stream) {
  COOCC_CHECK_ARG(d && d->cat4 && d->pts && d->lin && d->counts && d->rows && d->rows_p && d->near_img && d->near_pts && d->ws &&
                      d->offsets && d->counts_host, "fuser_search: null pointer");
  COOCC_CHECK_ARG(d->C > 0 && d->X > 0 && d->Y > 0 && d->Z > 0 && d->K >= 1 && d->K <= 8 && d->fps_num > 0 && d->max_cluster > 0 &&
                      d->noff > 0, "fuser_search: bad sizes");
  COOCC_CHECK_ARG(stream != side_stream && side_stream, "fuser_search: needs a second stream for the img <- pts direction");
  const int V = d->X * d->Y * d->Z, K = d->K, C = d->C;
  SearchWs w = carve((char*)d->ws, V, K, d->fps_num, d->max_cluster, d->X, d->Y, d->Z);
  COOCC_CHECK_ARG(d->ws_bytes >= w.total, "fuser_search: workspace smaller than coocc_fuser_search_ws()");
  hipStream_t s0 = as_stream(stream), s1 = as_stream(side_stream);
  static const int sdiag = [] { const char* e = getenv("COOCC_SEARCH_DIAG_SKIP"); return e ? atoi(e) : 0; }();
  int32_t* lin_img = d->lin;
  int32_t* lin_pts = d->lin + V;

  SRC(coocc_fuser_prepare_rows(d->cat4, 1, 4 * C, d->pts, d->pts_rows, d->pts_stride, d->cat4, w.flags, w.flags + V, 1, C, V, stream));
  SRC(coocc_compact_flags(w.flags, V, lin_img, d->counts, w.cws, (size_t)(V / 1024 + 2) * 4, stream));
  SRC(coocc_compact_flags(w.flags + V, V, lin_pts, d->counts + 1, w.cws + (V / 1024 + 2), (size_t)(V / 1024 + 2) * 4, stream));
  if (!((sdiag & 4) && d->counts_host[0] > 0)) COOCC_HIP(hipMemcpyAsync(d->counts_host, d->counts, 8, hipMemcpyDeviceToHost, s0));
  if (!((sdiag & 4) && d->counts_host[0] > 0)) {
    static const bool fence = [] { const char* e = getenv("COOCC_SEARCH_COUNT_FENCE"); return e && e[0] == '1'; }();
    hipEvent_t got;
    COOCC_HIP(hipEventCreateWithFlags(&got, hipEventBlockingSync | hipEventDisableTiming | (fence ? 0u : hipEventDisableSystemFence)));
    const hipError_t e1 = hipEventRecord(got, s0);
    const hipError_t e2 = e1 == hipSuccess ? hipEventSynchronize(got) : e1;
    (void)hipEventDestroy(got);
    if (e2 != hipSuccess) return coocc_set_error(COOCC_EHIP, "fuser_search: waiting for the voxel counts failed: %s", hipGetErrorString(e2));
  }
  const int Ni = d->counts_host[0], Np = d->counts_host[1];
  if (Ni <= d->fps_num || Np <= d->fps_num) return COOCC_SEARCH_SMALL;

  float* xyz_img = w.xyz;
  float* xyz_pts = w.xyz + (size_t)V * 3;
  SRC(coocc_lin_to_coords(lin_img, Ni, d->X, d->Y, d->Z, xyz_img, nullptr, stream));
  SRC(coocc_lin_to_coords(lin_pts, Np, d->X, d->Y, d->Z, xyz_pts, nullptr, stream));
  int32_t* map_img = w.maps;
  int32_t* map_pts = w.maps + V;
  SRC(coocc_voxel_index_map(lin_img, Ni, V, map_img, stream));
  SRC(coocc_voxel_index_map(lin_pts, Np, V, map_pts, stream));

  const int pair_rc = (sdiag & 1) ? COOCC_OK
                                  : coocc_fps_voxels_pair(lin_pts, Np, w.rep[0], w.fps[0], lin_img, Ni, w.rep[1], w.fps[1], w.fps_bytes, d->X, d->Y,
                                                          d->Z, d->fps_num, stream);
  if (pair_rc != COOCC_OK && pair_rc != 2) return pair_rc;
  const bool paired = pair_rc == COOCC_OK;
  hipEvent_t fork = nullptr, join = nullptr;
  COOCC_HIP(hipEventCreateWithFlags(&fork, hipEventDisableTiming | hipEventDisableSystemFence));
  if (hipEventCreateWithFlags(&join, hipEventDisableTiming | hipEventDisableSystemFence) != hipSuccess) {
    (void)hipEventDestroy(fork);
    return coocc_set_error(COOCC_EHIP, "fuser_search: hipEventCreate failed");
  }
  bool forked = false;
  auto finish = [&](int rc) -> int {
    if (forked) {
      if (hipEventRecord(join, s1) != hipSuccess || hipStreamWaitEvent(s0, join, 0) != hipSuccess) {
        if (rc == COOCC_OK) rc = coocc_set_error(COOCC_EHIP, "fuser_search: joining the side stream failed");
      }
    }
    (void)hipEventDestroy(fork);
    (void)hipEventDestroy(join);
    return rc;
  };
#define SRF(call)                                \
  do {                                           \
    int rc__ = (call);                           \
    if (rc__ != COOCC_OK) return finish(rc__);   \
  } while (0)
  void* side_q = paired ? stream : side_stream;
  if (!paired) {
    if (hipEventRecord(fork, s0) != hipSuccess || hipStreamWaitEvent(s1, fork, 0) != hipSuccess)
      return finish(coocc_set_error(COOCC_EHIP, "fuser_search: forking the side stream failed"));
    forked = true;
  }

  auto direction = [&](int dd, void* st, const int32_t* lin_q, int Q, const float* xyz_q, const int32_t* map_q, int Nk,
                       const float* xyz_k, const int32_t* map_k, int32_t* near) -> int {
    if (sdiag & 2) return COOCC_OK;
    if (!paired) SRC(coocc_fps_voxels(lin_q, Q, d->X, d->Y, d->Z, d->fps_num, w.rep[dd], w.fps[dd], w.fps_bytes, st));
    hipLaunchKernelGGL(k_gather_xyz, dim3(cdiv(d->fps_num, 256)), dim3(256), 0, as_stream(st), xyz_q, w.rep[dd], d->fps_num, w.rep_xyz[dd]);
    COOCC_LAUNCH_CHECK("k_gather_xyz");
    SRC(coocc_knn_topk_voxels(d->fps_num, Nk, K, d->X, d->Y, d->Z, w.rep[dd], lin_q, map_k, d->offsets, d->noff, w.rep_xyz[dd], xyz_k,
                              w.val[dd], w.nn[dd], st));
    SRC(coocc_ball_query_voxels(d->fps_num, 0.f, d->radius, d->max_cluster, d->X, d->Y, d->Z, w.rep[dd], lin_q, map_q, w.group[dd], st));
    SRC(coocc_knn_assign(d->fps_num, K, d->max_cluster, Q, d->dist_thresh, w.val[dd], w.nn[dd], w.group[dd], w.winner[dd], near, st));
    return COOCC_OK;
  };
  SRF(direction(1, side_q, lin_img, Ni, xyz_img, map_img, Np, xyz_pts, map_pts, d->near_pts));
  for (int k = 0; k < K && !(sdiag & 2); ++k)
    SRF(coocc_index_rows_i32(K == 1 ? lin_pts : lin_img, K == 1 ? Np : Ni, d->near_pts + (size_t)k * Ni, Ni, d->rows_p + (size_t)k * V, side_q));
  SRF(direction(0, stream, lin_pts, Np, xyz_pts, map_pts, Ni, xyz_img, map_img, d->near_img));
  for (int k = 0; k < K && !(sdiag & 2); ++k)
    SRF(coocc_index_rows_i32(lin_img, Ni, d->near_img + (size_t)k * Np, Np, d->rows + (size_t)k * V, stream));
#undef SRF
  return finish(COOCC_OK);
}
```

co_occ_amd/fuser.py:

```python
import torch
from torch import nn

from . import _lib, streams
from ._lib import call, ptr
from . import core as _core_mod
from .core import PackCache, PackedConv, Rows, conv_rows, gather_conv_rows
from .registry import FUSION_LAYERS

_I32, _F32, _I64 = torch.int32, torch.float32, torch.int64


_side = {}


def _side_stream(dev, cur, which=0):
    key = (dev.index, cur.cuda_stream, which)
    if key not in _side:
        _side[key] = streams.side_stream_for(cur, which) or torch.cuda.Stream(device=dev, priority=getattr(cur, "priority", 0))
    return _side[key]


FPS_HIGH_PRIORITY = __import__("os").environ.get("COOCC_FPS_HIGH_PRIORITY", "0") != "0"
_fps_hi = {}
FPS_MAX_BUCKETS = 8 * 1024


def _fps_voxels(q_lin, grid, fps_num, which=0, home=None):
    dev = q_lin.device
    cur = torch.cuda.current_stream(dev)
    fstream = streams.fps_stream_for(home if home is not None else cur, which)
    if fstream is None and FPS_HIGH_PRIORITY:
        key = (dev.index, cur.cuda_stream, which)
        if key not in _fps_hi:
            _fps_hi[key] = torch.cuda.Stream(device=dev, priority=-1)
        fstream = _fps_hi[key]
    if fstream is not None:
        fstream.wait_stream(cur)
        with torch.cuda.stream(fstream):
            out = _fps_voxels_on_current(q_lin, grid, fps_num)
        cur.wait_stream(fstream)
        out.record_stream(cur)
        q_lin.record_stream(fstream)
        return out
    return _fps_voxels_on_current(q_lin, grid, fps_num)


def _fps_voxels_on_current(q_lin, grid, fps_num):
    dev = q_lin.device
    X, Y, Z = grid
    ws = _core_mod.stream_buffer(dev, "fps", int(_lib.load().coocc_fps_voxels_ws(X, Y, Z)), torch.uint8)
    out = torch.empty(1, fps_num, device=dev, dtype=_I32)
    call("coocc_fps_voxels", ptr(q_lin), q_lin.numel(), X, Y, Z, fps_num, ptr(out), ptr(ws), ws.numel())
    return out


GRID_SEARCH = __import__("os").environ.get("COOCC_GRID_SEARCH", "1") != "0"
SPLIT_C0 = __import__("os").environ.get("COOCC_SPLIT_C0", "0" if _core_mod.CONV_ENGINE == "h2" else "1") != "0"
SPLIT_C0_MAX_DENSITY = 0.30
DENSE_C0_MAX_VOXELS = 100000
_offset_tables = {}


def offset_table(Z, device, radius=16):
    key = (int(Z), device.index, radius)
    if key not in _offset_tables:
        import numpy as np
        r = np.arange(-radius, radius + 1)
        zr = np.arange(-min(radius, Z - 1), min(radius, Z - 1) + 1)
        dx, dy, dz = np.meshgrid(r, r, zr, indexing="ij")
        dx, dy, dz = dx.ravel(), dy.ravel(), dz.ravel()
        d2 = dx * dx + dy * dy + dz * dz
        keep = d2 <= radius * radius
        dx, dy, dz, d2 = dx[keep], dy[keep], dz[keep], d2[keep]
        order = np.lexsort((dz, dy, dx, d2))
        packed = ((dx[order] + 128) | ((dy[order] + 128) << 8) | ((dz[order] + 128) << 16)).astype(np.int64)
        _offset_tables[key] = torch.from_numpy(packed.astype(np.uint32).view(np.int32)).to(device)
    return _offset_tables[key]


def _fps_nn_xyz(query_xyz, key_xyz, fps_num, radius, max_cluster_samples, dist_thresh, num, q_lin=None, grid=None,
                which=0, home=None, k_lin=None):
    dev = query_xyz.device
    Q, Nk = query_xyz.shape[0], key_xyz.shape[0]
    if Q <= fps_num:
        if num != 1:
            raise IndexError("too many indices for tensor of dimension 1")
        out = torch.full((1, Q), -1, device=dev, dtype=_I32)
        if Q == 0 or Nk == 0:
            return out
        val = torch.empty(Q, 1, device=dev, dtype=_F32)
        nn_ = torch.empty(Q, 1, device=dev, dtype=_I32)
        call("coocc_knn_topk", Q, Nk, 1, ptr(query_xyz), ptr(key_xyz), ptr(val), ptr(nn_))
        call("coocc_knn_threshold", Q, float(dist_thresh), ptr(val), ptr(nn_), ptr(out))
        return out
    if q_lin is not None and grid is not None and (grid[0] + 3) // 4 * ((grid[1] + 3) // 4) * ((grid[2] + 7) // 8) <= FPS_MAX_BUCKETS:
        repr_idx = _fps_voxels(q_lin, grid, fps_num, which, home)
    else:
        repr_idx = torch.empty(1, fps_num, device=dev, dtype=_I32)
        temp = torch.empty(1, Q, device=dev, dtype=_F32)
        call("coocc_furthest_point_sampling", 1, Q, fps_num, ptr(query_xyz), ptr(temp), ptr(repr_idx))
    repr_xyz = query_xyz[repr_idx[0].long()].contiguous()
    val = torch.empty(fps_num, num, device=dev, dtype=_F32)
    nn_ = torch.empty(fps_num, num, device=dev, dtype=_I32)
    group = torch.empty(fps_num, max_cluster_samples, device=dev, dtype=_I32)
    if GRID_SEARCH and q_lin is not None and k_lin is not None and grid is not None:
        X, Y, Z = grid
        maps = torch.empty(2, X * Y * Z, device=dev, dtype=_I32)
        call("coocc_voxel_index_map", ptr(q_lin), Q, X * Y * Z, ptr(maps[0]))
        call("coocc_voxel_index_map", ptr(k_lin), Nk, X * Y * Z, ptr(maps[1]))
        off = offset_table(Z, dev)
        rep = repr_idx[0].contiguous()
        call("coocc_knn_topk_voxels", fps_num, Nk, num, X, Y, Z, ptr(rep), ptr(q_lin), ptr(maps[1]), ptr(off), off.numel(),
             ptr(repr_xyz), ptr(key_xyz), ptr(val), ptr(nn_))
        call("coocc_ball_query_voxels", fps_num, 0.0, float(radius), max_cluster_samples, X, Y, Z, ptr(rep), ptr(q_lin),
             ptr(maps[0]), ptr(group))
    else:
        call("coocc_knn_topk", fps_num, Nk, num, ptr(repr_xyz), ptr(key_xyz), ptr(val), ptr(nn_))
        call("coocc_ball_query", 1, Q, fps_num, 0.0, float(radius), max_cluster_samples, ptr(repr_xyz), ptr(query_xyz),
             ptr(group))
    winner = torch.empty(num, Q, device=dev, dtype=_I32)
    out = torch.empty(num, Q, device=dev, dtype=_I32)
    call("coocc_knn_assign", fps_num, num, max_cluster_samples, Q, float(dist_thresh), ptr(val), ptr(nn_), ptr(group),
         ptr(winner), ptr(out))
    return out


def _as_rows_view(x):
    if isinstance(x, Rows):
        return x
    if x.dim() != 5 or not x.is_cuda or x.dtype != _F32:
        return None
    B, C, X, Y, Z = x.shape
    sb, sc, sx, sy, sz = x.stride()
    S = sz
    if sc != 1 or S < C or S % 4 or sy != Z * S or sx != Y * Z * S or (B > 1 and sb != X * Y * Z * S):
        return None
    off = x.storage_offset()
    coff = off % S
    if coff + C > S or (x.data_ptr() - 4 * coff) % 16:
        return None
    base = torch.as_strided(x, (B * X * Y * Z, S), (S, 1), off - coff)
    return Rows(base, B, X, Y, Z, C, coff)


_concat_buffers = {}


def _register_concat(t):
    import weakref
    for k in [k for k, r in _concat_buffers.items() if r() is None]:
        del _concat_buffers[k]
    _concat_buffers[t.data_ptr()] = weakref.ref(t)


def _is_concat(t):
    r = _concat_buffers.get(t.data_ptr())
    base = r() if r is not None else None
    return base is not None and base.data_ptr() == t.data_ptr() and base.numel() == t.numel()


class SearchSlot:

    def __init__(self, C, knum, grid, device):
        X, Y, Z = grid
        V = X * Y * Z
        self.grid, self.C, self.V = (X, Y, Z), C, V
        self.cat4 = torch.empty(V, 4 * C, device=device, dtype=_F32)
        _register_concat(self.cat4)
        self.lin = torch.zeros(2, V, device=device, dtype=_I32)
        self.counts = torch.zeros(2, device=device, dtype=_I32)
        self.rows = torch.zeros(knum, V, device=device, dtype=_I32)
        self.rows_p = torch.zeros(knum, V, device=device, dtype=_I32)

        self.knum = knum
        self.near = torch.zeros(2, knum * V, device=device, dtype=_I32)
        self._native = None

    def img_rows(self):
        X, Y, Z = self.grid
        return Rows(self.cat4, 1, X, Y, Z, self.C, 0, persistent=True)

    def native_desc(self):
        if self._native is None:
            import ctypes
            X, Y, Z = self.grid
            d = _lib.SearchDesc()
            d.cat4 = self.cat4.data_ptr()
            d.C, d.X, d.Y, d.Z, d.K = self.C, X, Y, Z, self.knum
            d.fps_num, d.max_cluster, d.radius, d.dist_thresh = 2048, 200, 6.0, 13.3
            off = offset_table(Z, self.cat4.device)
            d.offsets, d.noff = off.data_ptr(), off.numel()
            d.lin, d.counts = self.lin.data_ptr(), self.counts.data_ptr()
            d.near_img, d.near_pts = self.near[0].data_ptr(), self.near[1].data_ptr()
            d.rows, d.rows_p = self.rows.data_ptr(), self.rows_p.data_ptr()
            need = int(_lib.load().coocc_fuser_search_ws(ctypes.byref(d)))
            ws = torch.empty(need, device=self.cat4.device, dtype=torch.uint8)
            d.ws, d.ws_bytes = ws.data_ptr(), need
            host = (ctypes.c_int32 * 2)()
            d.counts_host = ctypes.addressof(host)
            self._native = (d, ws, host, off)
        return self._native


class SearchResult:

    def __init__(self, cat4, lin_img, lin_pts):
        self.cat4, self.lin_img, self.lin_pts = cat4, lin_img, lin_pts
        self.rows = self.rows_p = self.near_img = self.near_pts = None
        self.done_main = self.done_side = None
        self.keep = ()
        self.slot = None
        self.counts = (lin_img.numel(), lin_pts.numel())

    def tensors(self):
        out = [self.cat4.t, self.lin_img, self.lin_pts]
        out += [t for t in (self.rows, self.rows_p, self.near_img, self.near_pts) if t is not None]
        return out + [t for t in self.keep if torch.is_tensor(t)]


@FUSION_LAYERS.register_module()
class BiFuser_N(nn.Module):
    def __init__(self, in_channels, out_channels, knum=1, norm_cfg=None):
        super().__init__()
        self.in_channels, self.out_channels, self.knum = in_channels, out_channels, knum
        self.con_enc = nn.Sequential(
            nn.Conv3d(in_channels * 4, out_channels * 2, 3, padding=1, bias=False),
            nn.BatchNorm3d(out_channels * 2), nn.ReLU(True),
            nn.Conv3d(in_channels * 2, out_channels, 3, padding=1, bias=False),
            nn.BatchNorm3d(out_channels), nn.ReLU(True))
        self.knn_enc = nn.Sequential(nn.Linear(in_channels * knum, out_channels), nn.ReLU())
        self._packs = PackCache(self)
        self.last_counts = None
        self.output_readers = None

    def set_conenc_tiles(self, tiles):
        self.conenc_tiles = None if tiles is None else (int(tiles[0]), int(tiles[1]))
        _core_mod.invalidate_packs(self)

    def _packed(self):
        def build():
            d = build_packs()
            import os
            from . import core as _core
            default = "4,4" if _core.CONV_ENGINE == "h2" else "2,2"
            forced = getattr(self, "conenc_tiles", None)
            t0, t3 = forced if forced is not None else [int(v) for v in os.environ.get("COOCC_CONENC_TILES", default).split(",")]
            d["c0"].wino_tile, d["c3"].wino_tile = t0, t3
            d["c0_dense"].wino_tile = t0
            d["conenc_tiles"] = (t0, t3)
            d["conenc_tiles_large"] = (t0, t3) if ("COOCC_CONENC_TILES" in os.environ or forced is not None) else (2, 2)
            return d

        def build_packs():
            C, W0 = self.in_channels, self.con_enc[0].weight
            Co = W0.shape[0]
            dense_idx = list(range(0, C)) + list(range(3 * C, 4 * C))
            w_cols = W0[:, C:3 * C].reshape(Co, 2 * C, 27).permute(2, 0, 1).reshape(27 * Co, 2 * C).contiguous()
            return dict(
                c0_dense=PackedConv(W0[:, dense_idx].contiguous(), bn=self.con_enc[1], ksize=3, pad=1),
                c0_sparse=PackedConv(w_cols),
                c0=PackedConv(self.con_enc[0].weight, bn=self.con_enc[1], ksize=3, pad=1),
                c3=PackedConv(self.con_enc[3].weight, bn=self.con_enc[4], ksize=3, pad=1),
                knn=PackedConv(self.knn_enc[0].weight, bias=self.knn_enc[0].bias, tap_major=True, taps=self.knum))
        return self._packs.get_modules((self.con_enc, self.knn_enc), build)

    def fps_NN_fast(self, query, key, fps_num, radius, max_cluster_samples, dist_thresh, num):
        q = query[:, 1:].float().contiguous()
        k = key[:, 1:].float().contiguous()
        out = _fps_nn_xyz(q, k, fps_num, radius, max_cluster_samples, dist_thresh, num).long()
        return out[0] if num == 1 else out

    def concat_buffer(self, B, X, Y, Z, device):
        C = self.in_channels
        cat4 = torch.empty(B * X * Y * Z, 4 * C, device=device, dtype=_F32)
        _register_concat(cat4)
        return Rows(cat4, B, X, Y, Z, C, 0)

    def search(self, img_voxel_feats, pts_voxel_feats, slot=None):
        img_r, pts_r = _as_rows_view(img_voxel_feats), _as_rows_view(pts_voxel_feats)
        one = img_r if img_r is not None else img_voxel_feats
        if isinstance(one, Rows):
            B, C, X, Y, Z = one.B, one.C, one.X, one.Y, one.Z
            dev = one.t.device
        else:
            B, C, X, Y, Z = one.shape
            dev = one.device
        V = X * Y * Z
        if dev.type != "cuda":
            raise _lib.CooccError("BiFuser_N runs on the GPU only (no CPU fallback)")
        flags = torch.empty(2, B * V, device=dev, dtype=torch.uint8)
        if img_r is None and pts_r is None:
            img = img_voxel_feats.float().contiguous()
            pts = pts_voxel_feats.float().contiguous()
            cat4 = torch.empty(B * V, 4 * C, device=dev, dtype=_F32)
            call("coocc_fuser_prepare", ptr(img), ptr(pts), ptr(cat4), ptr(flags[0]), ptr(flags[1]), B, C, V)
        else:
            in_place = (img_r is not None and img_r.t.shape[1] == 4 * C and img_r.coff == 0 and img_r.t.is_contiguous()
                        and (_is_concat(img_r.t) or (slot is not None and img_r.t.data_ptr() == slot.cat4.data_ptr())))
            if slot is not None:
                assert in_place and img_r.t.data_ptr() == slot.cat4.data_ptr() and B == 1, \
                    "search(slot=...): the camera rows must already sit in slot 0 of the slot's concat buffer"
            cat4 = img_r.t if in_place else torch.empty(B * V, 4 * C, device=dev, dtype=_F32)
            img = img_r if img_r is not None else img_voxel_feats.float().contiguous()
            pts = pts_r if pts_r is not None else pts_voxel_feats.float().contiguous()
            src = lambda r: (r.data(), 1, r.stride) if isinstance(r, Rows) else (ptr(r), 0, 0)
            call("coocc_fuser_prepare_rows", *src(img), *src(pts), ptr(cat4), ptr(flags[0]), ptr(flags[1]), B, C, V)
        assert slot is None or (img_r is not None or pts_r is not None), "search(slot=...) takes channels-last producers"
        lin = slot.lin if slot is not None else torch.empty(2, B * V, device=dev, dtype=_I32)
        counts = slot.counts if slot is not None else torch.empty(2, device=dev, dtype=_I32)
        ws = torch.empty(2, B * V // 1024 + 2, device=dev, dtype=_I32)
        for i in range(2):
            call("coocc_compact_flags", ptr(flags[i]), B * V, ptr(lin[i]), ptr(counts[i:i + 1]), ptr(ws[i]),
                 ws[i].numel() * 4)
        Ni, Np = (int(v) for v in _lib.host_read(counts))
        self.last_counts = (Ni, Np)
        lin_img, lin_pts = lin[0, :Ni], lin[1, :Np]
        xyz = torch.empty(Ni + Np, 3, device=dev, dtype=_F32)
        if Ni:
            call("coocc_lin_to_coords", ptr(lin_img), Ni, X, Y, Z, ptr(xyz[:Ni]), None)
        if Np:
            call("coocc_lin_to_coords", ptr(lin_pts), Np, X, Y, Z, ptr(xyz[Ni:]), None)
        xyz_img, xyz_pts = xyz[:Ni], xyz[Ni:]
        K = self.knum
        kw = dict(fps_num=2048, radius=6, max_cluster_samples=200, dist_thresh=13.3, num=K)
        sr = SearchResult(Rows(cat4, B, X, Y, Z, 4 * C), lin_img, lin_pts)
        sr.slot = slot
        cur = torch.cuda.current_stream(dev)
        if Np and Ni:
            vox = (X, Y, Z) if B == 1 else None
            side = _side_stream(dev, cur)
            side.wait_stream(cur)
            with torch.cuda.stream(side):
                sr.near_pts = _fps_nn_xyz(xyz_img, xyz_pts, q_lin=lin_img if vox else None, k_lin=lin_pts if vox else None, grid=vox,
                                          which=1, home=cur, **kw)
                sr.rows_p = slot.rows_p[:, :Ni] if slot is not None else torch.empty(K, Ni, device=dev, dtype=_I32)
                base, nbase = (lin_pts, Np) if K == 1 else (lin_img, Ni)
                for k in range(K):
                    call("coocc_index_rows_i32", ptr(base), nbase, ptr(sr.near_pts[k]), Ni, ptr(sr.rows_p[k]))
                sr.done_side = streams.new_event()
                sr.done_side.record()
            sr.near_img = _fps_nn_xyz(xyz_pts, xyz_img, q_lin=lin_pts if vox else None, k_lin=lin_img if vox else None, grid=vox,
                                      which=0, home=cur, **kw)
            sr.rows = slot.rows[:, :Np] if slot is not None else torch.empty(K, Np, device=dev, dtype=_I32)
            for k in range(K):
                call("coocc_index_rows_i32", ptr(lin_img), Ni, ptr(sr.near_img[k]), Np, ptr(sr.rows[k]))
            sr.keep = (xyz, lin, img, pts)
        elif Np or Ni:
            raise IndexError("BiFuser_N: one modality has no non-empty voxel (the reference fails on empty keys)")
        sr.done_main = streams.new_event()
        sr.done_main.record()
        return sr

    def search_native(self, pts_voxel_feats, slot):
        import ctypes
        X, Y, Z = slot.grid
        dev = slot.cat4.device
        pts_r = _as_rows_view(pts_voxel_feats)
        B = pts_r.B if pts_r is not None else pts_voxel_feats.shape[0]
        if B != 1 or (X + 3) // 4 * ((Y + 3) // 4) * ((Z + 7) // 8) > FPS_MAX_BUCKETS:
            return self.search(slot.img_rows().as_ncdhw(), pts_voxel_feats, slot=slot)
        d, _, host, _ = slot.native_desc()
        if pts_r is not None:
            d.pts, d.pts_rows, d.pts_stride = pts_r.t.data_ptr() + 4 * pts_r.coff, 1, pts_r.stride
            keep = pts_r.t
        else:
            keep = pts_voxel_feats.float().contiguous()
            d.pts, d.pts_rows, d.pts_stride = keep.data_ptr(), 0, 0
        cur = torch.cuda.current_stream(dev)
        side = _side_stream(dev, cur)
        rc = _lib.load().coocc_fuser_search(ctypes.byref(d), ctypes.c_void_p(cur.cuda_stream), ctypes.c_void_p(side.cuda_stream))
        if rc == 1:
            return self.search(slot.img_rows().as_ncdhw(), pts_voxel_feats, slot=slot)
        _lib.check(rc)
        Ni, Np = int(host[0]), int(host[1])
        self.last_counts = (Ni, Np)
        K, V = self.knum, slot.V
        sr = SearchResult(Rows(slot.cat4, 1, X, Y, Z, 4 * self.in_channels), slot.lin[0, :Ni], slot.lin[1, :Np])
        sr.slot = slot
        sr.near_img = slot.near[0, :K * Np].view(K, Np)
        sr.near_pts = slot.near[1, :K * Ni].view(K, Ni)
        sr.rows, sr.rows_p = slot.rows[:, :Np], slot.rows_p[:, :Ni]
        sr.keep = (keep,)
        sr.done_main = streams.new_event()
        sr.done_main.record()
        sr.done_side = sr.done_main
        return sr

    def finish(self, sr):
        cat4 = sr.cat4.t
        dev = cat4.device
        C = self.in_channels
        cur = torch.cuda.current_stream(dev)
        packs = self._packed()
        sr.done_main.wait(cur)
        for t in sr.tensors():
            t.record_stream(cur)
        if sr.rows is not None and sr.slot is not None:
            sr.done_side.wait(cur)
            self.finish_static(sr.slot)
            self.last_near = (sr.near_img, sr.near_pts)
        elif sr.rows is not None:
            sr.done_side.wait(cur)
            h2 = self._g1_h2(cat4, packs)
            gather_conv_rows(cat4, 0, packs["knn"], sr.rows, sr.lin_pts, cat4, 2 * C, C, C, src_h2=h2)
            gather_conv_rows(cat4, C, packs["knn"], sr.rows_p, sr.lin_img, cat4, 3 * C, 0, C, src_h2=h2)
            self.last_near = (sr.near_img, sr.near_pts)
        return sr.cat4, (sr.lin_img, sr.lin_pts)

    def _g1_h2(self, cat4, packs):
        import os
        from . import core
        if os.environ.get("COOCC_G1_H2_ONCE", "1") == "0":
            return None
        sh = core.g1_sources_h2(cat4, self.in_channels, packs["knn"])
        return None if sh is None else (sh, 0, 2 * self.in_channels)

    def finish_static(self, slot):
        C = self.in_channels
        packs = self._packed()
        cat4 = slot.cat4
        h2 = self._g1_h2(cat4, packs)
        gather_conv_rows(cat4, 0, packs["knn"], slot.rows, slot.lin[1], cat4, 2 * C, C, C, count_dev=slot.counts[1:2], src_h2=h2)
        gather_conv_rows(cat4, C, packs["knn"], slot.rows_p, slot.lin[0], cat4, 3 * C, 0, C, count_dev=slot.counts[0:1], src_h2=h2)
        X, Y, Z = slot.grid
        return Rows(cat4, 1, X, Y, Z, 4 * C)

    def forward_static(self, slot):
        packs = self._packed()
        cat4 = self.finish_static(slot)
        x = self.con_enc0(cat4, slot.lin[1], packs, count_dev=slot.counts[1:2])
        return conv_rows(x, packs["c3"], relu=True, twin_for=self._readers())

    def finish_bookkeeping(self, sr):
        cur = torch.cuda.current_stream(sr.cat4.t.device)
        sr.done_main.wait(cur)
        if sr.done_side is not None:
            sr.done_side.wait(cur)
        for t in sr.tensors():
            t.record_stream(cur)
        if sr.rows is not None:
            self.last_near = (sr.near_img, sr.near_pts)

    def fuse(self, img_voxel_feats, pts_voxel_feats, search=None):
        return self.finish(search if search is not None else self.search(img_voxel_feats, pts_voxel_feats))

    def forward(self, img_voxel_feats, pts_voxel_feats, search=None):
        if not (img_voxel_feats.t if isinstance(img_voxel_feats, Rows) else img_voxel_feats).is_cuda:
            raise _lib.CooccError("BiFuser_N runs on the GPU only (no CPU fallback)")
        if self.training:
            from . import autograd as ag
            assert img_voxel_feats.shape[0] == 1, "BiFuser_N training path: batch size 1 per GPU (samples_per_gpu=1 upstream)"
            with torch.no_grad():
                sr = search if search is not None else self.search(img_voxel_feats.detach(), pts_voxel_feats.detach())
            (ri, geom), (rp, _) = ag.rows_from_ncdhw(img_voxel_feats), ag.rows_from_ncdhw(pts_voxel_feats)
            self.finish_bookkeeping(sr)
            x, g = ag.con_enc_train(self.con_enc, ag.fuser_fuse_train(self, ri, rp, sr), geom)
            return ag.ncdhw_from_rows(x, g)
        packs = self._packed()
        cat4, (_, lin_pts) = self.fuse(img_voxel_feats, pts_voxel_feats, search)
        x = self.con_enc0(cat4, lin_pts, packs)
        x = conv_rows(x, packs["c3"], relu=True, twin_for=self._readers())
        return x.as_ncdhw()

    def _readers(self):
        return tuple(self.output_readers()) if self.output_readers is not None else ()

    @staticmethod
    def c0_capacity(V):
        return int(SPLIT_C0_MAX_DENSITY * V)

    def con_enc0(self, cat4, lin_pts, packs, count_dev=None):
        from . import core
        C, V, dev = self.in_channels, cat4.V * cat4.B, cat4.t.device
        Np = int(lin_pts.numel())
        pd = packs["c0_dense"]
        if "conenc_tiles" in packs:
            t0, t3 = packs["conenc_tiles_large"] if cat4.V > DENSE_C0_MAX_VOXELS else packs["conenc_tiles"]
            packs["c0"].wino_tile = pd.wino_tile = t0
            packs["c3"].wino_tile = t3
        split = SPLIT_C0 or (core.CONV_ENGINE == "h2" and V > DENSE_C0_MAX_VOXELS and "COOCC_SPLIT_C0" not in __import__("os").environ)
        plan = core.wino_plan(cat4, pd, V, 1) if (split and core.CONV_DTYPE == "f32") else None
        if count_dev is not None:
            if plan is None or cat4.B != 1:
                return conv_rows(cat4, packs["c0"], relu=True)
            Np = self.c0_capacity(V)
        elif plan is None or Np == 0 or Np > SPLIT_C0_MAX_DENSITY * V or cat4.B != 1:
            return conv_rows(cat4, packs["c0"], relu=True)
        ps = packs["c0_sparse"]
        Co = pd.Cout
        P = core.scratch(dev, "c0P", Np * 27 * Co)
        src = ptr(cat4.t, offset=cat4.coff + C)
        d = core.conv_desc(dev, in_=src, w=ptr(ps.w), out=ptr(P), gather=ptr(lin_pts), M=Np, Cin=2 * C, Cout=27 * Co, taps=1,
                           in_stride=cat4.stride, out_stride=27 * Co, B=1, Yi=1, Zi=1, Xo=1, Yo=1, Zo=1,
                           Xi=V,
                           ksize=1, stride=1, splitk=1, tile_hint=core.TILE_HINT)
        if count_dev is not None:
            d.M_dev, d.gather_stride = ptr(count_dev, _I32), lin_pts.numel()
        h2 = core.CONV_ENGINE == "h2" and core.H2_DIRECT and (2 * C) % 32 == 0
        if h2:
            rh = core.scratch(dev, "c0rows", Np * 2 * C)
            call("coocc_rows_to_h2_gather", src, cat4.stride, ptr(lin_pts), Np, ptr(count_dev, _I32) if count_dev is not None else None,
                 2 * C, 1.0, ptr(rh))
            d.in_, d.in_stride, d.w, d.gather, d.gather_stride = ptr(rh), 2 * C, ptr(ps.h2_pack()), None, 0
            d.Xi, d.Xo = Np, Np
            d.mfma_dtype, d.alpha = 3, 1.0
        core.launch_conv(d, dev, "k_gemm_h2w c0-sparse" if h2 else lambda: core.conv_kernel_name(Np, 27 * Co, True) + " c0-sparse",
                         2.0 * Np * 2 * C * 27 * Co)
        vmap = torch.empty(V, device=dev, dtype=_I32)
        if count_dev is not None:
            call("coocc_voxel_index_map_dev", ptr(lin_pts), int(lin_pts.numel()), ptr(count_dev, _I32), V, ptr(vmap))
        else:
            call("coocc_voxel_index_map", ptr(lin_pts), Np, V, ptr(vmap))
        S = core.Rows(torch.empty(V, Co, device=dev, dtype=_F32), cat4.B, cat4.X, cat4.Y, cat4.Z, Co)
        call("coocc_sparse_tap_sum", ptr(P), ptr(vmap), cat4.B, cat4.X, cat4.Y, cat4.Z, Co, ptr(pd.scale), ptr(S.t), Co, int(Np))
        out = core.Rows(torch.empty(V, Co, device=dev, dtype=_F32), cat4.B, cat4.X, cat4.Y, cat4.Z, Co)
        return core.conv_rows_wino(cat4, pd, out, True, S, plan, in_ranges=[(0, C), (3 * C, C)])
```

co_occ_amd/serving.py:

```python
import collections
import os
import threading
import time
from concurrent.futures import ThreadPoolExecutor

import torch

from . import core, graph as cg, streams as cstreams_

CAM_KEYS = ("rots", "trans", "intrins", "post_rots", "post_trans", "bda")


def _tensors_of(obj):
    if torch.is_tensor(obj):
        yield obj
    elif isinstance(obj, dict):
        for v in obj.values():
            yield from _tensors_of(v)
    elif isinstance(obj, (list, tuple)):
        for v in obj:
            yield from _tensors_of(v)


class Ticket:

    __slots__ = ("pipe", "index", "slot", "frame", "search", "out", "done", "copy", "events", "fallback", "ready", "pts_vol", "stream")

    def __init__(self, pipe, index, slot, frame, copy):
        self.pipe, self.index, self.slot, self.frame, self.copy = pipe, index, slot, frame, copy
        self.search = self.out = self.done = self.events = self.pts_vol = self.stream = None
        self.fallback = False
        self.ready = cstreams_.new_event()
        self.ready.record(torch.cuda.current_stream(pipe.dev))

    def result(self, wait=True):
        self.pipe._issue_through(self.index)
        if wait:
            self.done.synchronize()
            core.check_h2_overflow()
        return self.out


_DIAG_SKIP = int(os.environ.get("COOCC_SERVING_DIAG_SKIP", "0"))
SLOT_WAIT_HOST = os.environ.get("COOCC_SLOT_WAIT", "host") != "device"


def _clone_frame_item(v):
    if torch.is_tensor(v):
        return v.detach().clone()
    if isinstance(v, (list, tuple)):
        return type(v)(_clone_frame_item(x) for x in v)
    return v


class ServingPipeline:

    def __init__(self, model, example, slots=6, dense_streams=3, ahead=0, render=None, search_priority=0, after_replay=None,
                 time_dense=False, after_done=None):
        assert not model.training, "ServingPipeline serves the eval-mode (folded-BN) path"
        self.model = model
        pts = example.get("pts")
        if pts is None:
            with torch.no_grad():
                pts = model.extract_pts_feat(example["points"])[0]
        self.dev = dev = pts.device
        _, _, X, Y, Z = pts.shape
        self.grid = (X, Y, Z)
        self.render = (X >= 100 and Y >= 100 and Z >= 8 and model.use_rendering) if render is None else render
        self.n = n = max(1, int(slots))
        self.ndense = max(1, min(int(dense_streams), max(1, n - 1)))
        most = max(1, n - self.ndense) if n > 1 else 1
        self.ahead = most if ahead <= 0 else max(1, min(int(ahead), most))
        self.after_replay, self.after_done, self.time_dense = after_replay, after_done, time_dense
        self.dense_streams = [torch.cuda.Stream(device=dev) for _ in range(self.ndense)]
        self.search_streams = [torch.cuda.Stream(device=dev, priority=search_priority) for _ in range(n)]
        self.slots = [cg.make_slot(model, self.grid, dev) for _ in range(n)]
        self.static = [self._make_static(example) for _ in range(n)]
        self.slot_done = [None] * n
        self.graphs = [None] * n
        self.tpool = ThreadPoolExecutor(self.ahead)
        self.fallbacks = 0
        self.dense_ev = []
        self.trace = [] if os.environ.get("COOCC_SERVING_TRACE", "0") == "1" else None
        self._lock = threading.Lock()
        self._pending = collections.deque()
        self._queue = collections.deque()
        self._submitted = self._issued = 0
        self._issued_of_slot = [0] * n
        self._dispatched_of_slot = [0] * n
        self._last_sr = [None] * n
        self._example = {k: _clone_frame_item(v) for k, v in example.items()}
        self.recaptures = 0
        self._capture(example)
        self._watch = core.WeightWatch(model)

    def _make_static(self, fr):
        dev = self.dev
        cams = fr.get("cams")
        tr = fr["transform"]
        size = tr[-1]
        size = tuple(int(v[0]) if torch.is_tensor(v) else int(v) for v in size)
        st = dict(img_feats=[torch.empty_like(fr["img_feats"][0], device=dev)],
                  cams=tuple(torch.empty_like(t, device=dev) for t in cams) if cams is not None else None,
                  transform=tuple(torch.empty_like(t, device=dev) if torch.is_tensor(t) else t for t in tr[:-1]) + (size,),
                  gemo=None)
        if cams is None:
            st["gemo"] = torch.empty_like(fr["gemo"], device=dev) if fr.get("gemo") is not None else None
        return st

    def _copy_in(self, k, fr):
        st = self.static[k]
        st["img_feats"][0].copy_(fr["img_feats"][0], non_blocking=True)
        if st["cams"] is not None:
            for d, s in zip(st["cams"], fr["cams"]):
                d.copy_(s, non_blocking=True)
        for d, s in zip(st["transform"][:-1], fr["transform"][:-1]):
            if torch.is_tensor(d):
                d.copy_(s, non_blocking=True)
        if st["gemo"] is not None:
            st["gemo"].copy_(fr["gemo"], non_blocking=True)

    def _mark(self, t, tag):
        if self.trace is not None:
            self.trace.append((t.index, tag, time.perf_counter()))

    def _search(self, t):
        k, fr = t.slot, t.frame
        torch.cuda.set_device(self.dev)
        self._mark(t, "search_begin")
        st = self.search_streams[k]
        with torch.cuda.stream(st), torch.no_grad():
            t.ready.wait(st)
            if self.slot_done[k] is not None:
                if SLOT_WAIT_HOST:
                    self.slot_done[k].synchronize()
                else:
                    self.slot_done[k].wait(st)
            if self.time_dense:
                e0 = cstreams_.new_event(timing=True)
                e0.record()
            for v in _tensors_of(fr):
                if v.is_cuda:
                    v.record_stream(st)
            diag = _DIAG_SKIP if t.index >= 0 else 0
            if not diag & 1:
                self._copy_in(k, fr)
            pts = fr.get("pts")
            if pts is None:
                pts = self.model.extract_pts_feat(fr["points"])[0]
            t.pts_vol = pts
            self._mark(t, "search_native")
            slot = self.slots[k]
            if diag & 6 and fr.get("depth") is not None and self._last_sr[k] is not None:
                if not diag & 2:
                    self.model.img_view_transformer.lift_splat(fr["depth"], fr["ctx"], cams=fr["cams"], out=slot.img_rows())
                if not diag & 4:
                    sr = self.model.occ_fuser.search_native(pts, slot)
                else:
                    sr = self._last_sr[k]
                    sr.done_main = cstreams_.new_event()
                    sr.done_main.record()
                    sr.done_side = sr.done_main
            elif fr.get("depth") is not None:
                sr = cg.search_into_slot(self.model, slot, fr["depth"], fr["ctx"], fr["cams"], pts)
                self._last_sr[k] = sr
            else:
                vol = fr["img_voxel_feats"]
                slot.img_rows().as_ncdhw().copy_(vol)
                sr = self.model.occ_fuser.search_native(pts, slot) if cg.NATIVE_SEARCH else \
                    self.model.occ_fuser.search(slot.img_rows().as_ncdhw(), pts, slot=slot)
            if self.time_dense:
                if sr.done_side is not None:
                    sr.done_side.wait(st)
                e1 = cstreams_.new_event(timing=True)
                e1.record()
                t.events = (e0, e1)
        self._mark(t, "search_end")
        return sr

    def _capture(self, example):
        for k in range(self.n):
            t = Ticket(self, -1, k, example, False)
            sr = self._search(t)
            ds = self.dense_streams[k % self.ndense]
            sr.done_main.wait(ds)
            if sr.done_side is not None:
                sr.done_side.wait(ds)
            self.graphs[k] = cg.DenseGraph(self.model, self.slots[k], self.static[k], ds, render=self.render).capture()
        torch.cuda.synchronize(self.dev)
        core.check_h2_overflow()

    def submit(self, frame, copy=False):
        if self._watch.changed():
            self._recapture()
        with self._lock:
            i = self._submitted
            self._submitted += 1
            t = Ticket(self, i, i % self.n, frame, copy)
            self._pending.append(t)
        self._pump()
        return t

    def _pump(self, block_until=None):
        while True:
            with self._lock:
                while self._pending and len(self._queue) < self.ahead:
                    t = self._pending[0]
                    if self._dispatched_of_slot[t.slot] > self._issued_of_slot[t.slot]:
                        break
                    self._pending.popleft()
                    self._dispatched_of_slot[t.slot] += 1
                    self._mark(t, "dispatch")
                    t.search = self.tpool.submit(self._search, t)
                    self._queue.append(t)
                head = self._queue[0] if self._queue else None
            if head is None:
                return
            must = block_until is not None and self._issued <= block_until
            if not (must or head.search.done()):
                return
            sr = head.search.result()
            self._mark(head, "issue_begin")
            self._issue(head, sr)
            self._mark(head, "issue_end")
            with self._lock:
                self._queue.popleft()
                self._issued += 1
                self._issued_of_slot[head.slot] += 1

    def _issue_through(self, index):
        if self._issued <= index:
            self._pump(block_until=index)
        assert self._issued > index

    def _issue(self, t, sr):
        k = t.slot
        ds = self.dense_streams[k % self.ndense]
        sr.done_main.wait(ds)
        if sr.done_side is not None:
            sr.done_side.wait(ds)
        with torch.cuda.stream(ds), torch.no_grad():
            if self.time_dense:
                e0 = cstreams_.new_event(timing=True)
                e0.record()
            g = self.graphs[k]
            if g.fits(sr.counts):
                out = g.replay()
            else:
                self.fallbacks += 1
                t.fallback = True
                st = self.static[k]
                vf = self.model.occ_fuser(self.slots[k].img_rows().as_ncdhw(), t.pts_vol, search=sr)
                cam_geo = None
                if self.render and st["cams"] is not None:
                    cam_geo = self.model.img_view_transformer._camera_mats(*st["cams"])
                    cam_geo = (cam_geo[0].reshape(-1, cam_geo[0].shape[-1]),) + tuple(cam_geo[1:])
                out = self.model.decode(vf, st["gemo"], st["img_feats"], st["transform"], self.render, cam_geo=cam_geo)
            if self.time_dense:
                e1 = cstreams_.new_event(timing=True)
                e1.record()
                self.dense_ev.append((e0, e1, t.index, t.events))
            if t.copy:
                out = {kk: (v.clone() if torch.is_tensor(v) else (v.as_ncdhw().clone() if isinstance(v, core.Rows) else v))
                       for kk, v in out.items()}
            if self.after_replay is not None:
                self.after_replay(out)
            ev = cstreams_.new_event(blocking=True)
            ev.record()
        self.slot_done[k] = ev
        if self.after_done is not None:
            self.after_done(out, ev)
        t.out, t.done, t.stream = out, ev, ds
        t.frame = t.pts_vol = None
# ... 36 lines not shown
```

include/coocc_hip.h:

```cpp
#ifndef COOCC_HIP_H
#define COOCC_HIP_H

#include <stddef.h>
#include <stdint.h>

#ifdef __cplusplus
extern "C" {
#endif

#define COOCC_OK 0
#define COOCC_EINVAL (-1)
#define COOCC_EHIP (-2)
#define COOCC_ENOMEM (-3)

const char* coocc_last_error(void);
int coocc_abi_version(void);

int coocc_device_cu_count(int* n);
int coocc_stream_create_cu_mask(const uint32_t* mask_host, int nwords, void** stream_out);
int coocc_stream_destroy(void* stream);

int coocc_event_create(int flags, void** event_out);
int coocc_event_destroy(void* event);
int coocc_event_record(void* event, void* stream);
int coocc_stream_wait_event(void* stream, void* event);
int coocc_event_synchronize(void* event);
int coocc_event_query(void* event);
int coocc_event_elapsed_ms(void* start, void* stop, float* ms);


int coocc_ncdhw_to_ndhwc(const float* src, float* dst, int B, int C, int V, int dst_stride,
                         int dst_coff, void* stream);
int coocc_ndhwc_to_ncdhw(const float* src, float* dst, int B, int C, int V, int src_stride,
                         int src_coff, void* stream);

int coocc_fuser_prepare(const float* img, const float* pts, float* cat4, uint8_t* flag_img,
                        uint8_t* flag_pts, int B, int C, int V, void* stream);
int coocc_fuser_prepare_rows(const float* img, int img_rows, int img_stride, const float* pts, int pts_rows,
                             int pts_stride, float* cat4, uint8_t* flag_img, uint8_t* flag_pts, int B, int C, int V,
                             void* stream);

int coocc_compact_flags(const uint8_t* flags, int total, int32_t* lin, int32_t* count, void* ws,
                        size_t ws_bytes, void* stream);
int coocc_compact_flags_ex(const uint8_t* flags, int total, int32_t* lin, int32_t* count, int32_t* map, void* ws,
                           size_t ws_bytes, void* stream);
int coocc_lin_to_coords(const int32_t* lin, int n, int X, int Y, int Z, float* xyz, int64_t* bxyz,
                        void* stream);


int coocc_furthest_point_sampling(int b, int n, int m, const float* points, float* temp,
                                  int32_t* idx, void* stream);

size_t coocc_fps_voxels_ws(int X, int Y, int Z);
int coocc_fps_voxels(const int32_t* lin, int n, int X, int Y, int Z, int m, int32_t* idx, void* ws,
                     size_t ws_bytes, void* stream);
int coocc_fps_voxels_pair(const int32_t* lin0, int n0, int32_t* idx0, void* ws0, const int32_t* lin1, int n1, int32_t* idx1,
                          void* ws1, size_t ws_bytes_each, int X, int Y, int Z, int m, void* stream);

int coocc_ball_query(int b, int n, int m, float min_radius, float max_radius, int nsample,
                     const float* new_xyz, const float* xyz, int32_t* idx, void* stream);

#define COOCC_SEARCH_SMALL 1
typedef struct coocc_search_desc {
  float* cat4;
  const float* pts;
  int pts_rows, pts_stride;
  int C, X, Y, Z, K;
  int fps_num, max_cluster;
  float radius, dist_thresh;
  const uint32_t* offsets;
  int noff;
  int32_t* lin;
  int32_t* counts;
  int32_t* near_img;
  int32_t* near_pts;
  int32_t* rows;
  int32_t* rows_p;
  void* ws;
  size_t ws_bytes;
  int32_t* counts_host;
} coocc_search_desc;
size_t coocc_fuser_search_ws(const coocc_search_desc* d);
int coocc_fuser_search(coocc_search_desc* d, void* stream, void* side_stream);

int coocc_voxel_index_map(const int32_t* lin, int n, int nvox, int32_t* map, void* stream);
int coocc_voxel_index_map_dev(const int32_t* lin, int n_cap, const int32_t* n_dev, int nvox, int32_t* map, void* stream);
int coocc_ball_query_voxels(int m, float min_radius, float max_radius, int nsample, int X, int Y, int Z,
                            const int32_t* centre_ord, const int32_t* lin_q, const int32_t* map_q, int32_t* idx,
                            void* stream);
int coocc_knn_topk_voxels(int nq, int nk, int K, int X, int Y, int Z, const int32_t* rep_ord, const int32_t* lin_q,
                          const int32_t* map_k, const uint32_t* offsets, int noff, const float* q, const float* key,
                          float* val, int32_t* idx, void* stream);

int coocc_knn_topk(int nq, int nk, int K, const float* q, const float* key, float* val,
                   int32_t* idx, void* stream);

int coocc_knn_assign(int nc, int K, int ns, int nq, float dist_thresh, const float* val,
                     const int32_t* nn, const int32_t* group, int32_t* winner, int32_t* out,
                     void* stream);
int coocc_knn_threshold(int nq, float dist_thresh, const float* val, const int32_t* nn,
                        int32_t* out, void* stream);
int coocc_index_rows_i32(const int32_t* base, int nbase, const int32_t* sel, int n, int32_t* rows,
                         void* stream);


int64_t coocc_conv_pack_weights(const float* w_host, int Cout, int Cin, int taps, int tap_major,
                                float* packed_host);

typedef struct coocc_conv_desc {
  const float* in;
  const float* w;
  float* out;
  const float* scale;
  const float* bias;
  const float* res;
  const int32_t* gather;
  const int32_t* out_rows;
  float* ws;
  int64_t ws_floats;
  int M, Cin, Cout, taps;
  int in_stride, out_stride, res_stride;
  int B, Xi, Yi, Zi, Xo, Yo, Zo, ksize, stride, pad;
  int relu, res_mode;
  int splitk;
  int tile_hint;
  int kx, ky, kz;
  int px, py, pz;
  int wgroup_rows;
  int mfma_dtype;
  float alpha;
  const int32_t* M_dev;
  int gather_stride;
  void* out16;
  int out16_stride;
  int out_h2;
  void* out_h2_twin;
  int32_t* tile_sem;
  int tile_sem_ints;
  const float* alpha_dev;
  int sx, sy, sz;
} coocc_conv_desc;

int coocc_conv_fwd(const coocc_conv_desc* d, void* stream);

int coocc_rows_to_bf16(const float* in, int in_stride, int64_t rows, int C, void* out_bf16, void* stream);

int coocc_rows_to_h2(const float* in, int in_stride, int64_t rows, int C, float scale, void* out_h2, void* stream);
int coocc_rows_to_h2_ex(const float* in, int in_stride, int64_t rows, int C, float scale, const float* scale_dev, void* out_h2,
                        void* stream);
int coocc_rows_to_f16(const float* in, int in_stride, int64_t rows, int C, void* out_f16, void* stream);
int coocc_rows_to_h2_gather(const float* in, int in_stride, const int32_t* row_ids, int64_t n_cap, const int32_t* n_dev,
                            int C, float scale, void* out_h2, void* stream);

int coocc_wino_input(const float* in, int in_stride, int B, int X, int Y, int Z, int C, int tile, float* V,
                     int64_t group_rows, void* stream);
int coocc_wino_input_strided(const float* in, int in_stride, int B, int X, int Y, int Z, int C, int tile, float* V,
                             int vstride, int64_t group_rows, void* stream);
int coocc_wino_input_h2(const float* in, int in_stride, int B, int X, int Y, int Z, int C, int tile, void* V,
                        int vstride, int64_t group_rows, float scale, void* stream);
int coocc_wino_input_h2_ex(const float* in, int in_stride, int B, int X, int Y, int Z, int C, int tile, void* V,
                           int vstride, int64_t group_rows, float scale, const float* scale_dev, void* stream);
int coocc_sparse_tap_sum(const float* P, const int32_t* map, int B, int X, int Y, int Z, int Cout, const float* scale,
                         float* S, int s_stride, int p_rows, void* stream);
int coocc_wino_output(const float* Mb, int64_t group_rows, int B, int X, int Y, int Z, int C, int tile, float* out,
                      int out_stride, const float* scale, const float* bias, const float* res, int res_stride,
                      int relu, void* stream);
int coocc_wino_output_ex(const float* Mb, int64_t group_rows, int B, int X, int Y, int Z, int C, int tile, float* out,
                         int out_stride, const float* scale, const float* bias, const float* res, int res_stride,
                         int relu, void* out_h2_twin, void* stream);
int coocc_render_heads_h2(const void* x_h2, int V, int Cin, int width, const void* ws0_pack, const float* bs0,
                          const float* ws1, const float* bs1, const void* const* wr_packs_host,
                          const float* const* br_host, int n_rgb_hidden, const float* wr_out, const float* br_out,
                          float* table, int activate, void* stream);
int64_t coocc_wino_pack_weights_h2_dev(const float* w, int Cout, int Cin, int tile, int dgrad, void* packed, void* stream);
int64_t coocc_conv_pack_weights_h2_dev(const float* w, int Cout, int Cin, int taps, int mode, void* packed, void* stream);
int coocc_h2_overflow(int reset);
#define COOCC_FAULT_SPARSE_ORDINAL 1
int coocc_device_fault(int reset);
int64_t coocc_wino_pack_weights_dev(const float* w, int Cout, int Cin, int tile, int dgrad, float* packed, void* stream);
int coocc_wino_gradout(const float* dy, int dy_stride, int B, int X, int Y, int Z, int C, int tile, float* dM,
                       int64_t group_rows, void* stream);
int coocc_wino_ztap_table(int64_t rows_total, int Z, int32_t* table, void* stream);
int coocc_wino_wgrad(const float* V, const float* dM, int64_t group_rows, int Z, int Cin, int Cout, int tile,
                     const int32_t* ztap_table, float* dw, int accumulate, float* ws, int64_t ws_floats,
                     void* stream);
int coocc_rows_to_kh2(const float* x, int stride, int64_t rows, int64_t rows_pad, int C, float scale, const float* scale_dev,
                      void* out_kh2, void* stream);
int coocc_wino_operand_kh2(int which, const float* x, int x_stride, int B, int X, int Y, int Z, int C, int tile, void* out_kh2,
                           int64_t group_rows, float scale, const float* scale_dev, void* stream);
int coocc_conv_wgrad_h2(const void* x_kh2, const void* dy_kh2, int64_t rows_pad, int Cin, int Cout, float alpha,
                        const float* alpha_dev, float* dw, int accumulate, float* ws, int64_t ws_floats, void* stream);
int coocc_wino_wgrad_h2(const void* V_kh2, const void* dM_kh2, int64_t group_rows, int Z, int Cin, int Cout, int tile,
                        float alpha, const float* alpha_dev, float* dw, int accumulate, float* ws, int64_t ws_floats,
                        void* stream);

int64_t coocc_conv_pack_weights_dev(const float* w, int Cout, int Cin, int taps, int mode, float* packed,
                                    void* stream);
int coocc_conv_tap_table(int B, int Xi, int Yi, int Zi, int Xo, int Yo, int Zo, int ksize, int stride, int pad,
                         int dgrad, int32_t* table, void* stream);
int coocc_conv_epilogue_bwd(const float* dout, int dout_stride, const float* out, int out_stride,
                            const float* scale, int M, int C, int relu, float* dacc, int dacc_stride,
                            float* dres, int dres_stride, int dres_accumulate, float* dbias,
                            int dbias_accumulate, float* ws, int64_t ws_floats, void* stream);
#define COOCC_AMAX_WORDS 2048
int coocc_conv_epilogue_bwd_ex(const float* dout, int dout_stride, const float* out, int out_stride,
                               const float* scale, int M, int C, int relu, float* dacc, int dacc_stride,
                               float* dres, int dres_stride, int dres_accumulate, float* dbias,
                               int dbias_accumulate, float* ws, int64_t ws_floats, uint32_t* amax_word, float* scale2,
                               float target, void* stream);
int coocc_conv_wgrad(const float* in, int in_rows, int in_stride, const float* dacc, int dacc_stride,
                     const int32_t* table, int M, int Cin, int Cout, int taps, float* dw, int accumulate,
                     float* ws, int64_t ws_floats, void* stream);
int coocc_conv_wgrad_h2t(const float* in, int in_rows, int in_stride, const float* dacc, int dacc_stride,
                         const int32_t* table, int M, int Cin, int Cout, int taps, const float* scale2,
                         float* dw, int accumulate, float* ws, int64_t ws_floats, void* stream);

int coocc_gather_rows(const float* src, int src_stride, const int32_t* idx, int n, int C, float* dst,
                      int dst_stride, void* stream);
int coocc_scatter_add_rows(const float* src, int src_stride, const int32_t* idx, int n, int C, float* dst,
                           int dst_stride, void* stream);
int coocc_voxel_pool_bwd(const float* dout, int dout_stride, const float* geom, int npts, int pts_per_batch,
                         int C, const float* lo_dx_host, int B, int X, int Y, int Z, float* dx, void* stream);
int coocc_lift_splat_bwd(const float* dout, int dout_stride, const float* depth, const float* feat_nhwc,
                         const float* geom, int N, int D, int H, int W, int C, int pts_per_batch,
                         const float* lo_dx_host, int B, int X, int Y, int Z, float* d_depth,
                         float* d_feat_nhwc, void* stream);
int coocc_render_nearest_bwd(const float* table, int X, int Y, int Z, const float* geom, const float* zvals,
                             int N, int D, int H, int W, const float* bounds_host, const float* dmaps,
                             float* dtable, void* stream);
int coocc_upsample_maps_bwd(const float* drgbs, const float* ddepths, int N, int H, int W, int scale,
                            float* dmaps, void* stream);
int coocc_render_losses_bwd(const float* rgbs, const float* depths, const float* rgb_gt, const float* depth_gt,
                            int64_t npix, int D, const float* losses_out, const float* gl, float* drgbs,
                            float* ddepths, void* stream);

int coocc_upsample_trilinear_bwd(const float* dfine, float* dcoarse, int B, int C, int Xc, int Yc, int Zc, int Xf,
// ... 245 lines not shown
```

Measured before the change: 269.7.

## Batch fuser voxel search into paired kernels and fuse small input copies

```diff
diff --git a/co_occ_amd/_lib.py b/co_occ_amd/_lib.py
--- a/co_occ_amd/_lib.py
+++ b/co_occ_amd/_lib.py
@@ -28,7 +28,17 @@
                [(n, c_int) for n in ("C", "X", "Y", "Z", "K", "fps_num", "max_cluster")] + \
                [("radius", ctypes.c_float), ("dist_thresh", ctypes.c_float), ("offsets", c_void_p), ("noff", c_int)] + \
                [(n, c_void_p) for n in ("lin", "counts", "near_img", "near_pts", "rows", "rows_p", "ws")] + \
-               [("ws_bytes", ctypes.c_size_t), ("counts_host", c_void_p)]
+               [("ws_bytes", ctypes.c_size_t), ("counts_host", c_void_p), ("g1_h2", c_void_p)]
+
+
+class VoxSearchDir(ctypes.Structure):
+    _fields_ = [(n, c_void_p) for n in ("rep", "lin_q", "map_q", "map_k", "xyz_q", "xyz_k", "val", "nn", "group", "winner", "near", "base",
+                                        "rows")] + [(n, c_int) for n in ("nbase", "rows_stride", "nq", "nk")]
+
+
+class VoxSearchPair(ctypes.Structure):
+    _fields_ = [("dir", VoxSearchDir * 2)] + [(n, c_int) for n in ("ndir", "m", "K", "nsample", "X", "Y", "Z", "noff")] + \
+               [(n, ctypes.c_float) for n in ("min_radius", "max_radius", "dist_thresh")] + [("offsets", c_void_p)]
 
 
 P, I, F, Z, L = c_void_p, c_int, c_float, c_size_t, c_int64
@@ -56,13 +66,17 @@
     "coocc_ndhwc_to_ncdhw": (I, [P, P, I, I, I, I, I, P]),
     "coocc_fuser_prepare": (I, [P, P, P, P, P, I, I, I, P]),
     "coocc_fuser_prepare_rows": (I, [P, I, I, P, I, I, P, P, P, I, I, I, P]),
+    "coocc_fuser_prepare_rows_h2": (I, [P, I, I, P, I, I, P, P, P, I, I, I, P, P]),
     "coocc_compact_flags": (I, [P, I, P, P, P, Z, P]),
     "coocc_compact_flags_ex": (I, [P, I, P, P, P, P, Z, P]),
+    "coocc_copy_many": (I, [P, P, P, I, P]),
     "coocc_lin_to_coords": (I, [P, I, I, I, I, P, P, P]),
     "coocc_furthest_point_sampling": (I, [I, I, I, P, P, P, P]),
     "coocc_fps_voxels_ws": (Z, [I, I, I]),
     "coocc_fps_voxels": (I, [P, I, I, I, I, I, P, P, Z, P]),
     "coocc_fps_voxels_pair": (I, [P, I, P, P, P, I, P, P, Z, I, I, I, I, P]),
+    "coocc_fps_voxels_pair_ex": (I, [P, I, P, P, P, I, P, P, Z, I, I, I, I, I, P]),
+    "coocc_search_tables": (I, [P, I, P, P, P, P, I, P, P, P, Z, I, I, I, P]),
     "coocc_ball_query": (I, [I, I, I, F, F, I, P, P, P, P]),
     "coocc_knn_topk": (I, [I, I, I, P, P, P, P, P]),
     "coocc_voxel_index_map": (I, [P, I, I, P, P]),
@@ -85,6 +99,7 @@
     "coocc_conv_fwd": (I, [ctypes.POINTER(ConvDesc), P]),
     "coocc_fuser_search_ws": (Z, [ctypes.POINTER(SearchDesc)]),
     "coocc_fuser_search": (I, [ctypes.POINTER(SearchDesc), P, P]),
+    "coocc_voxel_search_pair": (I, [ctypes.POINTER(VoxSearchPair), P]),
     "coocc_upsample_add_trilinear": (I, [P, P, I, I, I, I, I, I, I, I, P]),
     "coocc_upsample_add_trilinear_ex": (I, [P, P, I, I, I, I, I, I, I, I, P, P]),
     "coocc_occhead_mix": (I, [P, P, I, P, P, I, I, P]),
@@ -316,6 +331,27 @@
         check(fn(*args, stream(dev)))
 
 
+COPY_MANY_MAX = 16
+COPY_MANY_BYTES = 64 << 10
+
+
+def copy_many(pairs):
+    small = []
+    for d, s in pairs:
+        if (s.is_cuda and s.device == d.device and s.dtype == d.dtype and s.shape == d.shape and s.is_contiguous() and d.is_contiguous()
+                and d.numel() * d.element_size() <= COPY_MANY_BYTES):
+            small.append((d, s))
+        else:
+            d.copy_(s, non_blocking=True)
+    for i in range(0, len(small), COPY_MANY_MAX):
+        part = small[i:i + COPY_MANY_MAX]
+        n = len(part)
+        src = (c_void_p * n)(*[s.data_ptr() for _, s in part])
+        dst = (c_void_p * n)(*[d.data_ptr() for d, _ in part])
+        nb = (c_int64 * n)(*[d.numel() * d.element_size() for d, _ in part])
+        check(load().coocc_copy_many(src, dst, nb, n, stream(part[0][0].device)))
+
+
 def conv_fwd(desc, device):
     fn = load().coocc_conv_fwd
     if device.index != torch.cuda.current_device():
diff --git a/co_occ_amd/csrc/knn.hip b/co_occ_amd/csrc/knn.hip
--- a/co_occ_amd/csrc/knn.hip
+++ b/co_occ_amd/csrc/knn.hip
@@ -476,8 +476,20 @@
 
 struct FpsPrep { int NBX, NBY, NBZ, L, q, RB, tinit, threads, R; long long NB; bool key32; };
 
+static void fps_layout(int n, int X, int Y, int Z, int* L_, int* q_, int* RB_, bool* key32_, int* tinit_) {
+  int L = 0;
+  while ((2 << L) <= n && L < 10) ++L;
+  const int q = (n + (1 << L) - 1) >> L;
+  int RB = L;
+  while ((1ll << RB) <= ((long long)q << L)) ++RB;
+  const long long d2max = (long long)(X - 1) * (X - 1) + (long long)(Y - 1) * (Y - 1) + (long long)(Z - 1) * (Z - 1);
+  const bool key32 = RB < 31 && d2max + 1 < (1ll << (32 - RB)) - 1;
+  *L_ = L; *q_ = q; *RB_ = RB; *key32_ = key32;
+  *tinit_ = key32 ? (int)((1u << (32 - RB)) - 1u) : 0x7FFFFFFF;
+}
+
 static int fps_prepare(const int32_t* lin, int n, int X, int Y, int Z, int m, const int32_t* idx, void* ws, size_t ws_bytes,
-                       hipStream_t s, FpsPrep* o) {
+                       hipStream_t s, FpsPrep* o, bool fill = true) {
   COOCC_CHECK_ARG(lin && idx && ws && n > 0 && m >= 0 && X > 0 && Y > 0 && Z > 0, "fps_voxels: bad args");
   COOCC_CHECK_ARG(n < (1 << FPS_KBITS), "fps_voxels: n must be < 2^22");
   COOCC_CHECK_ARG(X <= 1020 && Y <= 1020 && Z <= 1016, "fps_voxels: grid dims must fit 10-bit packed coordinates");
@@ -489,19 +501,11 @@
   if (ws_bytes < coocc_fps_voxels_ws(X, Y, Z)) return coocc_set_error(COOCC_ENOMEM, "fps_voxels: workspace too small");
   o->threads = threads;
   o->R = (int)((o->NB + threads - 1) / threads);
-  int L = 0;
-  while ((2 << L) <= n && L < 10) ++L;
-  const int q = (n + (1 << L) - 1) >> L;
-  int RB = L;
-  while ((1ll << RB) <= ((long long)q << L)) ++RB;
-  const long long d2max = (long long)(X - 1) * (X - 1) + (long long)(Y - 1) * (Y - 1) + (long long)(Z - 1) * (Z - 1);
-  o->key32 = RB < 31 && d2max + 1 < (1ll << (32 - RB)) - 1;
-  o->tinit = o->key32 ? (int)((1u << (32 - RB)) - 1u) : 0x7FFFFFFF;
-  o->L = L; o->q = q; o->RB = RB;
-  if (m == 0) return COOCC_OK;
+  fps_layout(n, X, Y, Z, &o->L, &o->q, &o->RB, &o->key32, &o->tinit);
+  if (m == 0 || !fill) return COOCC_OK;
   FpsCell* cell = (FpsCell*)ws;
   COOCC_HIP(hipMemsetAsync(cell, 0xFF, sizeof(FpsCell) * (size_t)o->NB * FT_P, s));
-  hipLaunchKernelGGL(k_fpsv_scatter, dim3(cdiv(n, 256)), dim3(256), 0, s, lin, n, Y, Z, o->NBY, o->NBZ, L, q, o->tinit, cell);
+  hipLaunchKernelGGL(k_fpsv_scatter, dim3(cdiv(n, 256)), dim3(256), 0, s, lin, n, Y, Z, o->NBY, o->NBZ, o->L, o->q, o->tinit, cell);
   COOCC_LAUNCH_CHECK("k_fpsv_scatter");
   return COOCC_OK;
 }
@@ -554,29 +558,28 @@
   return COOCC_OK;
 }
 
-extern "C" int coocc_fps_voxels_pair(const int32_t* lin0, int n0, int32_t* idx0, void* ws0, const int32_t* lin1, int n1, int32_t* idx1,
-                                     void* ws1, size_t ws_bytes_each, int X, int Y, int Z, int m, void* stream) {
+static bool fps_pair_eligible(int n0, int n1, int X, int Y, int Z) {
+  const long long NB = (long long)((X + FT_X - 1) / FT_X) * ((Y + FT_Y - 1) / FT_Y) * ((Z + FT_Z - 1) / FT_Z);
+  if (NB > (long long)FPSR_SLOTS * 16) return false;
+  for (int n : {n0, n1}) {
+    int L, q, RB, tinit;
+    bool key32;
+    fps_layout(n, X, Y, Z, &L, &q, &RB, &key32, &tinit);
+    if (!key32) return false;
+  }
+  if (g_fps_reg < 0) g_fps_reg = getenv("COOCC_FPS_REG") ? atoi(getenv("COOCC_FPS_REG")) : 1;
+  return g_fps_reg != 0;
+}
+
+extern "C" int coocc_fps_voxels_pair_ex(const int32_t* lin0, int n0, int32_t* idx0, void* ws0, const int32_t* lin1, int n1, int32_t* idx1,
+                                        void* ws1, size_t ws_bytes_each, int X, int Y, int Z, int m, int tables_ready, void* stream) {
   COOCC_CHECK_ARG(X > 0 && Y > 0 && Z > 0 && n0 > 0 && n1 > 0, "fps_voxels_pair: bad args");
-  {
-    const long long NB = (long long)((X + FT_X - 1) / FT_X) * ((Y + FT_Y - 1) / FT_Y) * ((Z + FT_Z - 1) / FT_Z);
-    if (NB > (long long)FPSR_SLOTS * 16) return 2;
-    const long long d2max = (long long)(X - 1) * (X - 1) + (long long)(Y - 1) * (Y - 1) + (long long)(Z - 1) * (Z - 1);
-    for (int n : {n0, n1}) {
-      int L = 0;
-      while ((2 << L) <= n && L < 10) ++L;
-      const int q = (n + (1 << L) - 1) >> L;
-      int RB = L;
-      while ((1ll << RB) <= ((long long)q << L)) ++RB;
-      if (!(RB < 31 && d2max + 1 < (1ll << (32 - RB)) - 1)) return 2;
-    }
-    if (g_fps_reg < 0) g_fps_reg = getenv("COOCC_FPS_REG") ? atoi(getenv("COOCC_FPS_REG")) : 1;
-    if (!g_fps_reg) return 2;
-  }
+  if (!fps_pair_eligible(n0, n1, X, Y, Z)) return 2;
   hipStream_t s = as_stream(stream);
   FpsPrep o0, o1;
-  int rc = fps_prepare(lin0, n0, X, Y, Z, m, idx0, ws0, ws_bytes_each, s, &o0);
+  int rc = fps_prepare(lin0, n0, X, Y, Z, m, idx0, ws0, ws_bytes_each, s, &o0, !tables_ready);
   if (rc != COOCC_OK) return rc;
-  rc = fps_prepare(lin1, n1, X, Y, Z, m, idx1, ws1, ws_bytes_each, s, &o1);
+  rc = fps_prepare(lin1, n1, X, Y, Z, m, idx1, ws1, ws_bytes_each, s, &o1, !tables_ready);
   if (rc != COOCC_OK || m == 0) return rc;
   FpsRegArgs a = {};
   a.p[0] = FpsRegProblem{lin0, (const FpsCell*)ws0, idx0, n0, o0.L, o0.q, o0.RB};
@@ -585,6 +588,68 @@
   hipLaunchKernelGGL(k_fps_voxels_reg, dim3(2), dim3(1024), 0, s, a);
   COOCC_LAUNCH_CHECK("k_fps_voxels_reg");
   return COOCC_OK;
+}
+
+extern "C" int coocc_fps_voxels_pair(const int32_t* lin0, int n0, int32_t* idx0, void* ws0, const int32_t* lin1, int n1, int32_t* idx1,
+                                     void* ws1, size_t ws_bytes_each, int X, int Y, int Z, int m, void* stream) {
+  return coocc_fps_voxels_pair_ex(lin0, n0, idx0, ws0, lin1, n1, idx1, ws1, ws_bytes_each, X, Y, Z, m, 0, stream);
+}
+
+struct SearchTableProblem { const int32_t* lin; const int32_t* map; float* xyz; FpsCell* cell; int n, L, q, tinit; };
+struct SearchTableArgs { SearchTableProblem p[2]; int X, Y, Z, NBY, NBZ, ncell; };
+
+__global__ __launch_bounds__(256) void k_search_tables(SearchTableArgs a) {
+  const SearchTableProblem& p = a.p[blockIdx.y];
+  const int i = blockIdx.x * blockDim.x + threadIdx.x;
+  if (i < p.n) {
+    int l = p.lin[i];
+    const int z = l % a.Z; l /= a.Z;
+    const int y = l % a.Y, x = l / a.Y;
+    p.xyz[i * 3 + 0] = (float)x; p.xyz[i * 3 + 1] = (float)y; p.xyz[i * 3 + 2] = (float)z;
+  }
+  if (p.cell && i < a.ncell) {
+    const int b = i / FT_P, pos = i - b * FT_P;
+    const int bz = b % a.NBZ, t = b / a.NBZ;
+    const int by = t % a.NBY, bx = t / a.NBY;
+    const int x = bx * FT_X + pos / (FT_Y * FT_Z), y = by * FT_Y + (pos / FT_Z) % FT_Y, z = bz * FT_Z + pos % FT_Z;
+    FpsCell c{-1, -1};
+    if (x < a.X && y < a.Y && z < a.Z) {
+      const int k = p.map[(x * a.Y + y) * a.Z + z];
+      if (k >= 0) {
+        const unsigned rev = p.L ? (__brev((unsigned)k & ((1u << p.L) - 1u)) >> (32 - p.L)) : 0u;
+        c = FpsCell{p.tinit, (int)(rev * (unsigned)p.q + ((unsigned)k >> p.L))};
+      }
+    }
+    p.cell[i] = c;
+  }
+}
+
+extern "C" int coocc_search_tables(const int32_t* lin0, int n0, const int32_t* map0, float* xyz0, void* cell0, const int32_t* lin1, int n1,
+                                   const int32_t* map1, float* xyz1, void* cell1, size_t ws_bytes_each, int X, int Y, int Z, void* stream) {
+  COOCC_CHECK_ARG(lin0 && lin1 && xyz0 && xyz1 && n0 > 0 && n1 > 0 && X > 0 && Y > 0 && Z > 0, "search_tables: bad args");
+  COOCC_CHECK_ARG((cell0 != nullptr) == (cell1 != nullptr) && (!cell0 || (map0 && map1)), "search_tables: cell tables need both workspaces and both maps");
+  COOCC_CHECK_ARG((long long)X * Y * Z < (1ll << 31) && n0 <= (long long)X * Y * Z && n1 <= (long long)X * Y * Z, "search_tables: bad sizes");
+  const bool cells = cell0 && fps_pair_eligible(n0, n1, X, Y, Z);
+  if (cells && ws_bytes_each < coocc_fps_voxels_ws(X, Y, Z)) return coocc_set_error(COOCC_ENOMEM, "search_tables: workspace too small");
+  SearchTableArgs a = {};
+  const int32_t* lin[2] = {lin0, lin1};
+  const int32_t* map[2] = {map0, map1};
+  float* xyz[2] = {xyz0, xyz1};
+  void* cell[2] = {cell0, cell1};
+  const int n[2] = {n0, n1};
+  for (int i = 0; i < 2; ++i) {
+    int L, q, RB, tinit;
+    bool key32;
+    fps_layout(n[i], X, Y, Z, &L, &q, &RB, &key32, &tinit);
+    a.p[i] = SearchTableProblem{lin[i], map[i], xyz[i], cells ? (FpsCell*)cell[i] : nullptr, n[i], L, q, tinit};
+  }
+  a.X = X; a.Y = Y; a.Z = Z;
+  a.NBY = (Y + FT_Y - 1) / FT_Y; a.NBZ = (Z + FT_Z - 1) / FT_Z;
+  a.ncell = cells ? (int)(coocc_fps_voxels_ws(X, Y, Z) / sizeof(FpsCell)) : 0;
+  const int work = a.ncell > n0 ? (a.ncell > n1 ? a.ncell : n1) : (n0 > n1 ? n0 : n1);
+  hipLaunchKernelGGL(k_search_tables, dim3(cdiv(work, 256), 2), dim3(256), 0, as_stream(stream), a);
+  COOCC_LAUNCH_CHECK("k_search_tables");
+  return cell0 && !cells ? 2 : COOCC_OK;
 }
 
 __global__ __launch_bounds__(256) void k_ball_query(int n, int m, float min_r2, float max_r2, int nsample,
@@ -717,13 +782,24 @@
   return COOCC_OK;
 }
 
-__global__ __launch_bounds__(256) void k_ball_query_vox(int m, float min_r2, float max_r2, int R, int nsample, int X, int Y, int Z,
-                                                         const int32_t* __restrict__ centre_ord, const int32_t* __restrict__ lin_q,
-                                                         const int32_t* __restrict__ map_q, int32_t* __restrict__ idx_all) {
+struct VoxSearchArgs {
+  coocc_vox_search_dir p[2];
+  int m, K, ns, X, Y, Z, noff, R, xyz_is_rep;
+  float min_r2, max_r2, thresh;
+  const uint32_t* offsets;
+};
+
+__global__ __launch_bounds__(256) void k_ball_query_vox(VoxSearchArgs a) {
+  const coocc_vox_search_dir& p = a.p[blockIdx.y];
+  const int m = a.m, R = a.R, nsample = a.ns, X = a.X, Y = a.Y, Z = a.Z;
+  const float min_r2 = a.min_r2, max_r2 = a.max_r2;
+  const int32_t* __restrict__ centre_ord = p.rep;
+  const int32_t* __restrict__ lin_q = p.lin_q;
+  const int32_t* __restrict__ map_q = p.map_q;
   const int lane = threadIdx.x & 63;
   const int c = blockIdx.x * 4 + (threadIdx.x >> 6);
   if (c >= m) return;
-  int32_t* idx = idx_all + (size_t)c * nsample;
+  int32_t* idx = p.group + (size_t)c * nsample;
   const int v0 = lin_q[centre_ord[c]];
   const int cz = v0 % Z, cy = (v0 / Z) % Y, cx = v0 / (Z * Y);
   const int x0 = max(cx - R, 0), x1 = min(cx + R, X - 1);
@@ -763,17 +839,28 @@
   const float max_r2 = max_radius * max_radius;
   int R = (int)ceilf(max_radius);
   while (R > 0 && (float)(R * R) >= max_r2) --R;
-  hipLaunchKernelGGL(k_ball_query_vox, dim3(cdiv(m, 4)), dim3(256), 0, as_stream(stream), m, min_radius * min_radius, max_r2, R,
-                     nsample, X, Y, Z, centre_ord, lin_q, map_q, idx);
+  VoxSearchArgs a = {};
+  a.p[0].rep = centre_ord; a.p[0].lin_q = lin_q; a.p[0].map_q = map_q; a.p[0].group = idx;
+  a.m = m; a.ns = nsample; a.X = X; a.Y = Y; a.Z = Z; a.R = R; a.min_r2 = min_radius * min_radius; a.max_r2 = max_r2;
+  hipLaunchKernelGGL(k_ball_query_vox, dim3(cdiv(m, 4)), dim3(256), 0, as_stream(stream), a);
   COOCC_LAUNCH_CHECK("k_ball_query_vox");
   return COOCC_OK;
 }
 
 template <int K>
-__global__ __launch_bounds__(256) void k_knn_topk_vox(int nq, int X, int Y, int Z, const int32_t* __restrict__ rep_ord,
-                                                       const int32_t* __restrict__ lin_q, const int32_t* __restrict__ map_k,
-                                                       const uint32_t* __restrict__ offsets, int noff, float* __restrict__ val,
-                                                       int32_t* __restrict__ idx) {
+__global__ __launch_bounds__(256) void k_knn_topk_vox(VoxSearchArgs a) {
+  const coocc_vox_search_dir& p = a.p[blockIdx.y];
+  const int nq = a.m, X = a.X, Y = a.Y, Z = a.Z, noff = a.noff;
+  const int32_t* __restrict__ rep_ord = p.rep;
+  const int32_t* __restrict__ lin_q = p.lin_q;
+  const int32_t* __restrict__ map_k = p.map_k;
+  const uint32_t* __restrict__ offsets = a.offsets;
+  float* __restrict__ val = p.val;
+  int32_t* __restrict__ idx = p.nn;
+  if (p.winner) {
+    const long long nw = (long long)K * p.nq;
+    for (long long i = (long long)blockIdx.x * blockDim.x + threadIdx.x; i < nw; i += (long long)gridDim.x * blockDim.x) p.winner[i] = -1;
+  }
   const int lane = threadIdx.x & 63;
   const int r = blockIdx.x * 4 + (threadIdx.x >> 6);
   if (r >= nq) return;
@@ -805,13 +892,18 @@
 }
 
 template <int K>
-__global__ __launch_bounds__(256) void k_knn_topk_unresolved(int nq, int nk, const float* __restrict__ q,
-                                                              const float* __restrict__ key, float* __restrict__ val,
-                                                              int32_t* __restrict__ idx) {
+__global__ __launch_bounds__(256) void k_knn_topk_unresolved(VoxSearchArgs a) {
+  const coocc_vox_search_dir& p = a.p[blockIdx.y];
+  const int nq = a.m, nk = p.nk;
+  const float* __restrict__ q = p.xyz_q;
+  const float* __restrict__ key = p.xyz_k;
+  float* __restrict__ val = p.val;
+  int32_t* __restrict__ idx = p.nn;
   const int lane = threadIdx.x & 63;
   const int r = blockIdx.x * 4 + (threadIdx.x >> 6);
   if (r >= nq || idx[(size_t)r * K] != -2) return;
-  const float qx = q[r * 3 + 0], qy = q[r * 3 + 1], qz = q[r * 3 + 2];
+  const int qr = a.xyz_is_rep ? r : p.rep[r];
+  const float qx = q[qr * 3 + 0], qy = q[qr * 3 + 1], qz = q[qr * 3 + 2];
   u64 best[K];
 #pragma unroll
   for (int j = 0; j < K; ++j) best[j] = ~0ull;
@@ -841,12 +933,20 @@
   }
 }
 
-template <int K>
-static void launch_topk_vox(int nq, int nk, int X, int Y, int Z, const int32_t* rep_ord, const int32_t* lin_q, const int32_t* map_k,
-                            const uint32_t* offsets, int noff, const float* q, const float* key, float* val, int32_t* idx,
-                            hipStream_t s) {
-  hipLaunchKernelGGL(k_knn_topk_vox<K>, dim3(cdiv(nq, 4)), dim3(256), 0, s, nq, X, Y, Z, rep_ord, lin_q, map_k, offsets, noff, val, idx);
-  hipLaunchKernelGGL(k_knn_topk_unresolved<K>, dim3(cdiv(nq, 4)), dim3(256), 0, s, nq, nk, q, key, val, idx);
+static void launch_topk_vox(const VoxSearchArgs& a, int ndir, hipStream_t s) {
+  const dim3 grid(cdiv(a.m, 4), ndir), block(256);
+#define TOPK_VOX(KK)                                                            \
+  case KK:                                                                      \
+    hipLaunchKernelGGL(k_knn_topk_vox<KK>, grid, block, 0, s, a);               \
+    hipLaunchKernelGGL(k_knn_topk_unresolved<KK>, grid, block, 0, s, a);        \
+    break
+  switch (a.K) {
+    TOPK_VOX(1); TOPK_VOX(2); TOPK_VOX(3); TOPK_VOX(4); TOPK_VOX(5); TOPK_VOX(6); TOPK_VOX(7);
+    default:
+      hipLaunchKernelGGL(k_knn_topk_vox<8>, grid, block, 0, s, a);
+      hipLaunchKernelGGL(k_knn_topk_unresolved<8>, grid, block, 0, s, a);
+  }
+#undef TOPK_VOX
 }
 
 extern "C" int coocc_knn_topk_voxels(int nq, int nk, int K, int X, int Y, int Z, const int32_t* rep_ord, const int32_t* lin_q,
@@ -855,23 +955,22 @@
   COOCC_CHECK_ARG(nq > 0 && nk > 0 && X > 0 && Y > 0 && Z > 0 && rep_ord && lin_q && map_k && offsets && noff > 0 && q && key &&
                       val && idx, "knn_topk_voxels: bad args");
   COOCC_CHECK_ARG(K >= 1 && K <= 8 && K <= nk, "knn_topk_voxels: need 1 <= K <= min(8, nk)");
-  hipStream_t s = as_stream(stream);
-  switch (K) {
-    case 1: launch_topk_vox<1>(nq, nk, X, Y, Z, rep_ord, lin_q, map_k, offsets, noff, q, key, val, idx, s); break;
-    case 2: launch_topk_vox<2>(nq, nk, X, Y, Z, rep_ord, lin_q, map_k, offsets, noff, q, key, val, idx, s); break;
-    case 3: launch_topk_vox<3>(nq, nk, X, Y, Z, rep_ord, lin_q, map_k, offsets, noff, q, key, val, idx, s); break;
-    case 4: launch_topk_vox<4>(nq, nk, X, Y, Z, rep_ord, lin_q, map_k, offsets, noff, q, key, val, idx, s); break;
-    case 5: launch_topk_vox<5>(nq, nk, X, Y, Z, rep_ord, lin_q, map_k, offsets, noff, q, key, val, idx, s); break;
-    case 6: launch_topk_vox<6>(nq, nk, X, Y, Z, rep_ord, lin_q, map_k, offsets, noff, q, key, val, idx, s); break;
-    case 7: launch_topk_vox<7>(nq, nk, X, Y, Z, rep_ord, lin_q, map_k, offsets, noff, q, key, val, idx, s); break;
-    default: launch_topk_vox<8>(nq, nk, X, Y, Z, rep_ord, lin_q, map_k, offsets, noff, q, key, val, idx, s); break;
-  }
+  VoxSearchArgs a = {};
+  a.p[0].rep = rep_ord; a.p[0].lin_q = lin_q; a.p[0].map_k = map_k; a.p[0].xyz_q = q; a.p[0].xyz_k = key; a.p[0].val = val; a.p[0].nn = idx;
+  a.p[0].nk = nk;
+  a.m = nq; a.K = K; a.X = X; a.Y = Y; a.Z = Z; a.noff = noff; a.offsets = offsets; a.xyz_is_rep = 1;
+  launch_topk_vox(a, 1, as_stream(stream));
   COOCC_LAUNCH_CHECK("k_knn_topk_vox");
   return COOCC_OK;
 }
 
-__global__ void k_assign_winner(int nc, int K, int ns, int nq, float thresh, const float* __restrict__ val,
-                                const int32_t* __restrict__ group, int32_t* __restrict__ winner) {
+__global__ void k_assign_winner(VoxSearchArgs a) {
+  const coocc_vox_search_dir& p = a.p[blockIdx.y];
+  const int nc = a.m, K = a.K, ns = a.ns, nq = p.nq;
+  const float thresh = a.thresh;
+  const float* __restrict__ val = p.val;
+  const int32_t* __restrict__ group = p.group;
+  int32_t* __restrict__ winner = p.winner;
   int i = blockIdx.x * blockDim.x + threadIdx.x;
   if (i >= nc * ns) return;
   int c = i / ns;
@@ -881,13 +980,20 @@
     if (val[c * K + k] < thresh) atomicMax(&winner[(size_t)k * nq + qi], c);
 }
 
-__global__ void k_assign_lookup(int K, int nq, const int32_t* __restrict__ nn,
-                                const int32_t* __restrict__ winner, int32_t* __restrict__ out) {
+__global__ void k_assign_lookup(VoxSearchArgs a) {
+  const coocc_vox_search_dir& p = a.p[blockIdx.y];
+  const int K = a.K, nq = p.nq;
   int i = blockIdx.x * blockDim.x + threadIdx.x;
   if (i >= K * nq) return;
   int k = i / nq;
-  int w = winner[i];
-  out[i] = w >= 0 ? nn[w * K + k] : -1;
+  int w = p.winner[i];
+  const int o = w >= 0 ? p.nn[w * K + k] : -1;
+  p.near[i] = o;
+  if (p.rows) {
+    int s = o;
+    if (s < 0) s += p.nbase;
+    p.rows[(size_t)k * p.rows_stride + (i - k * nq)] = (s >= 0 && s < p.nbase) ? p.base[s] : -1;
+  }
 }
 
 extern "C" int coocc_knn_assign(int nc, int K, int ns, int nq, float dist_thresh, const float* val,
@@ -896,10 +1002,45 @@
   COOCC_CHECK_ARG(val && nn && group && winner && out && nc > 0 && K > 0 && ns > 0 && nq > 0, "knn_assign: bad args");
   hipStream_t s = as_stream(stream);
   COOCC_HIP(hipMemsetAsync(winner, 0xFF, sizeof(int32_t) * (size_t)K * nq, s));
-  hipLaunchKernelGGL(k_assign_winner, dim3(cdiv((long long)nc * ns, 256)), dim3(256), 0, s, nc, K, ns, nq,
-                     dist_thresh, val, group, winner);
-  hipLaunchKernelGGL(k_assign_lookup, dim3(cdiv((long long)K * nq, 256)), dim3(256), 0, s, K, nq, nn, winner, out);
+  VoxSearchArgs a = {};
+  a.p[0].val = const_cast<float*>(val); a.p[0].nn = const_cast<int32_t*>(nn); a.p[0].group = const_cast<int32_t*>(group);
+  a.p[0].winner = winner; a.p[0].near = out; a.p[0].nq = nq;
+  a.m = nc; a.K = K; a.ns = ns; a.thresh = dist_thresh;
+  hipLaunchKernelGGL(k_assign_winner, dim3(cdiv((long long)nc * ns, 256)), dim3(256), 0, s, a);
+  hipLaunchKernelGGL(k_assign_lookup, dim3(cdiv((long long)K * nq, 256)), dim3(256), 0, s, a);
   COOCC_LAUNCH_CHECK("knn_assign");
+  return COOCC_OK;
+}
+
+extern "C" int coocc_voxel_search_pair(const coocc_vox_search_pair* d, void* stream) {
+  COOCC_CHECK_ARG(d && (d->ndir == 1 || d->ndir == 2), "voxel_search_pair: null descriptor or ndir not 1 / 2");
+  COOCC_CHECK_ARG(d->m > 0 && d->nsample > 0 && d->X > 0 && d->Y > 0 && d->Z > 0 && d->offsets && d->noff > 0 && d->K >= 1 && d->K <= 8,
+                  "voxel_search_pair: bad sizes");
+  COOCC_CHECK_ARG(d->max_radius >= 0.f && d->max_radius < 4096.f, "voxel_search_pair: bad radius");
+  int nq_max = 0;
+  for (int i = 0; i < d->ndir; ++i) {
+    const coocc_vox_search_dir& p = d->dir[i];
+    COOCC_CHECK_ARG(p.rep && p.lin_q && p.map_q && p.map_k && p.xyz_q && p.xyz_k && p.val && p.nn && p.group && p.winner && p.near,
+                    "voxel_search_pair: null pointer");
+    COOCC_CHECK_ARG(p.nq > 0 && p.nk >= d->K && (long long)d->K * p.nq < (1ll << 31), "voxel_search_pair: bad list sizes");
+    COOCC_CHECK_ARG(!p.rows || (p.base && p.nbase > 0 && p.rows_stride >= p.nq), "voxel_search_pair: bad row table");
+    nq_max = p.nq > nq_max ? p.nq : nq_max;
+  }
+  hipStream_t s = as_stream(stream);
+  VoxSearchArgs a = {};
+  for (int i = 0; i < d->ndir; ++i) a.p[i] = d->dir[i];
+  a.m = d->m; a.K = d->K; a.ns = d->nsample; a.X = d->X; a.Y = d->Y; a.Z = d->Z; a.noff = d->noff; a.offsets = d->offsets;
+  a.thresh = d->dist_thresh;
+  a.min_r2 = d->min_radius * d->min_radius;
+  a.max_r2 = d->max_radius * d->max_radius;
+  int R = (int)ceilf(d->max_radius);
+  while (R > 0 && (float)(R * R) >= a.max_r2) --R;
+  a.R = R;
+  launch_topk_vox(a, d->ndir, s);
+  hipLaunchKernelGGL(k_ball_query_vox, dim3(cdiv(a.m, 4), d->ndir), dim3(256), 0, s, a);
+  hipLaunchKernelGGL(k_assign_winner, dim3(cdiv((long long)a.m * a.ns, 256), d->ndir), dim3(256), 0, s, a);
+  hipLaunchKernelGGL(k_assign_lookup, dim3(cdiv((long long)a.K * nq_max, 256), d->ndir), dim3(256), 0, s, a);
+  COOCC_LAUNCH_CHECK("voxel_search_pair");
   return COOCC_OK;
 }
 
diff --git a/co_occ_amd/csrc/layout.hip b/co_occ_amd/csrc/layout.hip
--- a/co_occ_amd/csrc/layout.hip
+++ b/co_occ_amd/csrc/layout.hip
@@ -2,8 +2,9 @@
 #include <stdlib.h>
 
 #include "common.h"
-
-typedef float f32x4 __attribute__((ext_vector_type(4)));
+#include "h2_rows.h"
+
+int coocc_h2_flag_ptr(int** out);
 
 static thread_local char g_err[512] = "";
 
@@ -199,17 +200,20 @@
 }
 
 constexpr int FV = 256, FC = 32;
+template <bool H2>
 __global__ __launch_bounds__(256) void k_fuser_prepare_rows_fast(const float* __restrict__ img, int img_rows, int img_stride,
                                                                   const float* __restrict__ pts, int pts_rows, int pts_stride,
                                                                   float* __restrict__ cat4, uint8_t* __restrict__ flag_img,
-                                                                  uint8_t* __restrict__ flag_pts, int C, int V) {
+                                                                  uint8_t* __restrict__ flag_pts, int C, int V,
+                                                                  void* __restrict__ out_h2, int* __restrict__ h2_flag) {
   __shared__ float tile[FV][FC + 1];
   const int b = blockIdx.y;
   const int v0 = blockIdx.x * FV;
   const int t = threadIdx.x;
   const int stride = 4 * C;
   const int rv = t >> 3, rc = (t & 7) * 4;
-  for (int mod = 0; mod < 2; ++mod) {
+  const int part = gridDim.z == 3 ? (int)blockIdx.z : -1;
+  for (int mod = part < 0 ? 0 : part; mod < (part < 0 ? 2 : min(part + 1, 2)); ++mod) {
     const float* src = mod ? pts : img;
     const int rows = mod ? pts_rows : img_rows, sstride = mod ? pts_stride : img_stride;
     uint8_t* flags = mod ? flag_pts : flag_img;
@@ -221,7 +225,13 @@
         for (int ps = 0; ps < FV / 32; ++ps) {
           const int v = ps * 32 + rv;
           f32x4 q = {0.f, 0.f, 0.f, 0.f};
-          if (v0 + v < V) q = *(const f32x4*)(src + ((size_t)b * V + v0 + v) * sstride + c0 + rc);
+          if (v0 + v < V) {
+            q = *(const f32x4*)(src + ((size_t)b * V + v0 + v) * sstride + c0 + rc);
+            if (H2) {
+              store_h2_pair(out_h2, (size_t)b * V + v0 + v, 2 * C, mod * C + c0 + rc, q);
+              h2_guard(h2_flag, q);
+            }
+          }
           tile[v][rc] = q[0]; tile[v][rc + 1] = q[1]; tile[v][rc + 2] = q[2]; tile[v][rc + 3] = q[3];
         }
         __syncthreads();
@@ -236,13 +246,17 @@
         }
         __syncthreads();
       }
-      if (!in_place) {
+      if (!in_place || (H2 && !rows)) {
 #pragma unroll
         for (int ps = 0; ps < FV / 32; ++ps) {
           const int v = ps * 32 + rv;
           if (v0 + v < V) {
             const f32x4 q = {tile[v][rc], tile[v][rc + 1], tile[v][rc + 2], tile[v][rc + 3]};
-            *(f32x4*)(cat4 + ((size_t)b * V + v0 + v) * stride + mod * C + c0 + rc) = q;
+            if (!in_place) *(f32x4*)(cat4 + ((size_t)b * V + v0 + v) * stride + mod * C + c0 + rc) = q;
+            if (H2 && !rows) {
+              store_h2_pair(out_h2, (size_t)b * V + v0 + v, 2 * C, mod * C + c0 + rc, q);
+              h2_guard(h2_flag, q);
+            }
           }
         }
       }
@@ -250,6 +264,7 @@
     }
     if (v0 + t < V) flags[(size_t)b * V + v0 + t] = rsum != 0.f ? 1 : 0;
   }
+  if (part == 0 || part == 1) return;
   const int vec_per_row = C >> 1;
   const f32x4 z = {0.f, 0.f, 0.f, 0.f};
   if (vec_per_row <= 256 && 256 % vec_per_row == 0) {
@@ -267,13 +282,28 @@
 extern "C" int coocc_fuser_prepare_rows(const float* img, int img_rows, int img_stride, const float* pts, int pts_rows,
                                         int pts_stride, float* cat4, uint8_t* flag_img, uint8_t* flag_pts, int B, int C, int V,
                                         void* stream) {
+  return coocc_fuser_prepare_rows_h2(img, img_rows, img_stride, pts, pts_rows, pts_stride, cat4, flag_img, flag_pts, B, C, V, nullptr, stream);
+}
+
+extern "C" int coocc_fuser_prepare_rows_h2(const float* img, int img_rows, int img_stride, const float* pts, int pts_rows,
+                                           int pts_stride, float* cat4, uint8_t* flag_img, uint8_t* flag_pts, int B, int C, int V,
+                                           void* out_h2, void* stream) {
   COOCC_CHECK_ARG(img && pts && cat4 && flag_img && flag_pts && B > 0 && C > 0 && V > 0, "fuser_prepare_rows: bad args");
   COOCC_CHECK_ARG((!img_rows || img_stride >= C) && (!pts_rows || pts_stride >= C), "fuser_prepare_rows: row stride < C");
   const bool vec_ok = C % FC == 0 && ((uintptr_t)cat4 & 15) == 0 && (!img_rows || (img_stride % 4 == 0 && ((uintptr_t)img & 15) == 0)) &&
                       (!pts_rows || (pts_stride % 4 == 0 && ((uintptr_t)pts & 15) == 0));
+  if (out_h2) {
+    COOCC_CHECK_ARG(vec_ok && ((uintptr_t)out_h2 & 15) == 0, "fuser_prepare_rows_h2: H2 rows need C %% 32 == 0 and 16-byte aligned rows");
+    int* flag = nullptr;
+    if (coocc_h2_flag_ptr(&flag) != COOCC_OK) return COOCC_EHIP;
+    hipLaunchKernelGGL(k_fuser_prepare_rows_fast<true>, dim3(cdiv(V, FV), B, 3), dim3(256), 0, as_stream(stream), img, img_rows, img_stride,
+                       pts, pts_rows, pts_stride, cat4, flag_img, flag_pts, C, V, out_h2, flag);
+    COOCC_LAUNCH_CHECK("k_fuser_prepare_rows_fast");
+    return COOCC_OK;
+  }
   if (vec_ok) {
-    hipLaunchKernelGGL(k_fuser_prepare_rows_fast, dim3(cdiv(V, FV), B), dim3(256), 0, as_stream(stream), img, img_rows, img_stride,
-                       pts, pts_rows, pts_stride, cat4, flag_img, flag_pts, C, V);
+    hipLaunchKernelGGL(k_fuser_prepare_rows_fast<false>, dim3(cdiv(V, FV), B, 3), dim3(256), 0, as_stream(stream), img, img_rows, img_stride,
+                       pts, pts_rows, pts_stride, cat4, flag_img, flag_pts, C, V, (void*)nullptr, (int*)nullptr);
     COOCC_LAUNCH_CHECK("k_fuser_prepare_rows_fast");
     return COOCC_OK;
   }
@@ -438,6 +468,37 @@
   return COOCC_OK;
 }
 
+constexpr int COPY_MANY_MAX = 16;
+struct CopyManyArgs { const char* src[COPY_MANY_MAX]; char* dst[COPY_MANY_MAX]; unsigned bytes[COPY_MANY_MAX]; };
+__global__ __launch_bounds__(256) void k_copy_many(CopyManyArgs a) {
+  const char* __restrict__ s = a.src[blockIdx.y];
+  char* __restrict__ d = a.dst[blockIdx.y];
+  const unsigned nb = a.bytes[blockIdx.y];
+  const unsigned i0 = blockIdx.x * blockDim.x + threadIdx.x, step = gridDim.x * blockDim.x;
+  if ((((uintptr_t)s | (uintptr_t)d | nb) & 3) == 0) {
+    for (unsigned i = i0; i < nb / 4; i += step) ((uint32_t*)d)[i] = ((const uint32_t*)s)[i];
+  } else {
+    for (unsigned i = i0; i < nb; i += step) d[i] = s[i];
+  }
+}
+
+extern "C" int coocc_copy_many(const void* const* src, void* const* dst, const int64_t* bytes, int n, void* stream) {
+  COOCC_CHECK_ARG(src && dst && bytes && n >= 0 && n <= COPY_MANY_MAX, "copy_many: null table or more than 16 copies");
+  if (n == 0) return COOCC_OK;
+  CopyManyArgs a = {};
+  int64_t most = 0;
+  for (int i = 0; i < n; ++i) {
+    COOCC_CHECK_ARG(bytes[i] >= 0 && bytes[i] < (1ll << 31) && (bytes[i] == 0 || (src[i] && dst[i])), "copy_many: bad copy %d", i);
+    a.src[i] = (const char*)src[i]; a.dst[i] = (char*)dst[i]; a.bytes[i] = (unsigned)bytes[i];
+    most = bytes[i] > most ? bytes[i] : most;
+  }
+  if (most == 0) return COOCC_OK;
+  const unsigned gx = cdiv(cdiv(most, 4), 256);
+  hipLaunchKernelGGL(k_copy_many, dim3(gx < 64 ? gx : 64, n), dim3(256), 0, as_stream(stream), a);
+  COOCC_LAUNCH_CHECK("k_copy_many");
+  return COOCC_OK;
+}
+
 __global__ void k_lin_to_coords(const int32_t* __restrict__ lin, int n, int X, int Y, int Z,
                                 float* __restrict__ xyz, int64_t* __restrict__ bxyz) {
   int i = blockIdx.x * blockDim.x + threadIdx.x;
diff --git a/co_occ_amd/csrc/search.hip b/co_occ_amd/csrc/search.hip
--- a/co_occ_amd/csrc/search.hip
+++ b/co_occ_amd/csrc/search.hip
@@ -56,6 +56,25 @@
   return carve(nullptr, d->X * d->Y * d->Z, d->K, d->fps_num, d->max_cluster, d->X, d->Y, d->Z).total;
 }
 
+struct SearchEvents { int dev = -1; bool fence = false; hipEvent_t got = nullptr, fork = nullptr, join = nullptr; };
+static SearchEvents* search_events(bool fence) {
+  static thread_local SearchEvents ev;
+  int dev = -1;
+  if (hipGetDevice(&dev) != hipSuccess) return nullptr;
+  if (ev.dev == dev && ev.fence == fence) return &ev;
+  for (hipEvent_t* e : {&ev.got, &ev.fork, &ev.join}) {
+    if (*e) (void)hipEventDestroy(*e);
+    *e = nullptr;
+  }
+  ev.dev = -1;
+  const unsigned ordering = hipEventDisableTiming | hipEventDisableSystemFence;
+  if (hipEventCreateWithFlags(&ev.got, hipEventBlockingSync | hipEventDisableTiming | (fence ? 0u : hipEventDisableSystemFence)) != hipSuccess ||
+      hipEventCreateWithFlags(&ev.fork, ordering) != hipSuccess || hipEventCreateWithFlags(&ev.join, ordering) != hipSuccess)
+    return nullptr;
+  ev.dev = dev; ev.fence = fence;
+  return &ev;
+}
+
 #define SRC(call)                    \
   do {                               \
     int rc__ = (call);               \
@@ -73,20 +92,23 @@
   COOCC_CHECK_ARG(d->ws_bytes >= w.total, "fuser_search: workspace smaller than coocc_fuser_search_ws()");
   hipStream_t s0 = as_stream(stream), s1 = as_stream(side_stream);
   static const int sdiag = [] { const char* e = getenv("COOCC_SEARCH_DIAG_SKIP"); return e ? atoi(e) : 0; }();
+  static const bool fence = [] { const char* e = getenv("COOCC_SEARCH_COUNT_FENCE"); return e && e[0] == '1'; }();
   int32_t* lin_img = d->lin;
   int32_t* lin_pts = d->lin + V;
 
-  SRC(coocc_fuser_prepare_rows(d->cat4, 1, 4 * C, d->pts, d->pts_rows, d->pts_stride, d->cat4, w.flags, w.flags + V, 1, C, V, stream));
-  SRC(coocc_compact_flags(w.flags, V, lin_img, d->counts, w.cws, (size_t)(V / 1024 + 2) * 4, stream));
-  SRC(coocc_compact_flags(w.flags + V, V, lin_pts, d->counts + 1, w.cws + (V / 1024 + 2), (size_t)(V / 1024 + 2) * 4, stream));
+  int32_t* map_img = w.maps;
+  int32_t* map_pts = w.maps + V;
+
+  SRC(coocc_fuser_prepare_rows_h2(d->cat4, 1, 4 * C, d->pts, d->pts_rows, d->pts_stride, d->cat4, w.flags, w.flags + V, 1, C, V, d->g1_h2,
+                                  stream));
+  SRC(coocc_compact_flags_ex(w.flags, V, lin_img, d->counts, map_img, w.cws, (size_t)(V / 1024 + 2) * 4, stream));
+  SRC(coocc_compact_flags_ex(w.flags + V, V, lin_pts, d->counts + 1, map_pts, w.cws + (V / 1024 + 2), (size_t)(V / 1024 + 2) * 4, stream));
   if (!((sdiag & 4) && d->counts_host[0] > 0)) COOCC_HIP(hipMemcpyAsync(d->counts_host, d->counts, 8, hipMemcpyDeviceToHost, s0));
   if (!((sdiag & 4) && d->counts_host[0] > 0)) {
-    static const bool fence = [] { const char* e = getenv("COOCC_SEARCH_COUNT_FENCE"); return e && e[0] == '1'; }();
-    hipEvent_t got;
-    COOCC_HIP(hipEventCreateWithFlags(&got, hipEventBlockingSync | hipEventDisableTiming | (fence ? 0u : hipEventDisableSystemFence)));
-    const hipError_t e1 = hipEventRecord(got, s0);
-    const hipError_t e2 = e1 == hipSuccess ? hipEventSynchronize(got) : e1;
-    (void)hipEventDestroy(got);
+    SearchEvents* ev = search_events(fence);
+    if (!ev) return coocc_set_error(COOCC_EHIP, "fuser_search: hipEventCreate failed");
+    const hipError_t e1 = hipEventRecord(ev->got, s0);
+    const hipError_t e2 = e1 == hipSuccess ? hipEventSynchronize(ev->got) : e1;
     if (e2 != hipSuccess) return coocc_set_error(COOCC_EHIP, "fuser_search: waiting for the voxel counts failed: %s", hipGetErrorString(e2));
   }
   const int Ni = d->counts_host[0], Np = d->counts_host[1];
@@ -94,24 +116,37 @@
 
   float* xyz_img = w.xyz;
   float* xyz_pts = w.xyz + (size_t)V * 3;
-  SRC(coocc_lin_to_coords(lin_img, Ni, d->X, d->Y, d->Z, xyz_img, nullptr, stream));
-  SRC(coocc_lin_to_coords(lin_pts, Np, d->X, d->Y, d->Z, xyz_pts, nullptr, stream));
-  int32_t* map_img = w.maps;
-  int32_t* map_pts = w.maps + V;
-  SRC(coocc_voxel_index_map(lin_img, Ni, V, map_img, stream));
-  SRC(coocc_voxel_index_map(lin_pts, Np, V, map_pts, stream));
+  const int tab_rc = coocc_search_tables(lin_pts, Np, map_pts, xyz_pts, w.fps[0], lin_img, Ni, map_img, xyz_img, w.fps[1], w.fps_bytes,
+                                         d->X, d->Y, d->Z, stream);
+  if (tab_rc != COOCC_OK && tab_rc != 2) return tab_rc;
+  const bool paired = tab_rc == COOCC_OK;
+  if (paired) {
+    if (!(sdiag & 1)) {
+      const int rc = coocc_fps_voxels_pair_ex(lin_pts, Np, w.rep[0], w.fps[0], lin_img, Ni, w.rep[1], w.fps[1], w.fps_bytes, d->X, d->Y, d->Z,
+                                              d->fps_num, 1, stream);
+      if (rc == 2) return coocc_set_error(COOCC_EHIP, "fuser_search: the FPS pair refused lists its tables were built for");
+      if (rc != COOCC_OK) return rc;
+    }
+    if (sdiag & 2) return COOCC_OK;
+    coocc_vox_search_pair a = {};
+    a.dir[0].rep = w.rep[0]; a.dir[0].lin_q = lin_pts; a.dir[0].map_q = map_pts; a.dir[0].map_k = map_img;
+    a.dir[0].xyz_q = xyz_pts; a.dir[0].xyz_k = xyz_img; a.dir[0].nq = Np; a.dir[0].nk = Ni;
+    a.dir[0].near = d->near_img; a.dir[0].base = lin_img; a.dir[0].nbase = Ni; a.dir[0].rows = d->rows;
+    a.dir[1].rep = w.rep[1]; a.dir[1].lin_q = lin_img; a.dir[1].map_q = map_img; a.dir[1].map_k = map_pts;
+    a.dir[1].xyz_q = xyz_img; a.dir[1].xyz_k = xyz_pts; a.dir[1].nq = Ni; a.dir[1].nk = Np;
+    a.dir[1].near = d->near_pts; a.dir[1].base = K == 1 ? lin_pts : lin_img; a.dir[1].nbase = K == 1 ? Np : Ni; a.dir[1].rows = d->rows_p;
+    for (int dd = 0; dd < 2; ++dd) {
+      a.dir[dd].val = w.val[dd]; a.dir[dd].nn = w.nn[dd]; a.dir[dd].group = w.group[dd]; a.dir[dd].winner = w.winner[dd];
+      a.dir[dd].rows_stride = V;
+    }
+    a.ndir = 2; a.m = d->fps_num; a.K = K; a.nsample = d->max_cluster; a.X = d->X; a.Y = d->Y; a.Z = d->Z; a.noff = d->noff;
+    a.min_radius = 0.f; a.max_radius = d->radius; a.dist_thresh = d->dist_thresh; a.offsets = d->offsets;
+    return coocc_voxel_search_pair(&a, stream);
+  }
 
-  const int pair_rc = (sdiag & 1) ? COOCC_OK
-                                  : coocc_fps_voxels_pair(lin_pts, Np, w.rep[0], w.fps[0], lin_img, Ni, w.rep[1], w.fps[1], w.fps_bytes, d->X, d->Y,
-                                                          d->Z, d->fps_num, stream);
-  if (pair_rc != COOCC_OK && pair_rc != 2) return pair_rc;
-  const bool paired = pair_rc == COOCC_OK;
-  hipEvent_t fork = nullptr, join = nullptr;
-  COOCC_HIP(hipEventCreateWithFlags(&fork, hipEventDisableTiming | hipEventDisableSystemFence));
-  if (hipEventCreateWithFlags(&join, hipEventDisableTiming | hipEventDisableSystemFence) != hipSuccess) {
-    (void)hipEventDestroy(fork);
-    return coocc_set_error(COOCC_EHIP, "fuser_search: hipEventCreate failed");
-  }
+  SearchEvents* ev = search_events(fence);
+  if (!ev) return coocc_set_error(COOCC_EHIP, "fuser_search: hipEventCreate failed");
+  const hipEvent_t fork = ev->fork, join = ev->join;
   bool forked = false;
   auto finish = [&](int rc) -> int {
     if (forked) {
@@ -119,8 +154,6 @@
         if (rc == COOCC_OK) rc = coocc_set_error(COOCC_EHIP, "fuser_search: joining the side stream failed");
       }
     }
-    (void)hipEventDestroy(fork);
-    (void)hipEventDestroy(join);
     return rc;
   };
 #define SRF(call)                                \
@@ -128,17 +161,15 @@
     int rc__ = (call);                           \
     if (rc__ != COOCC_OK) return finish(rc__);   \
   } while (0)
-  void* side_q = paired ? stream : side_stream;
-  if (!paired) {
-    if (hipEventRecord(fork, s0) != hipSuccess || hipStreamWaitEvent(s1, fork, 0) != hipSuccess)
-      return finish(coocc_set_error(COOCC_EHIP, "fuser_search: forking the side stream failed"));
-    forked = true;
-  }
+  if (hipEventRecord(fork, s0) != hipSuccess || hipStreamWaitEvent(s1, fork, 0) != hipSuccess)
+    return finish(coocc_set_error(COOCC_EHIP, "fuser_search: forking the side stream failed"));
+  forked = true;
+  void* side_q = side_stream;
 
   auto direction = [&](int dd, void* st, const int32_t* lin_q, int Q, const float* xyz_q, const int32_t* map_q, int Nk,
                        const float* xyz_k, const int32_t* map_k, int32_t* near) -> int {
     if (sdiag & 2) return COOCC_OK;
-    if (!paired) SRC(coocc_fps_voxels(lin_q, Q, d->X, d->Y, d->Z, d->fps_num, w.rep[dd], w.fps[dd], w.fps_bytes, st));
+    if (!(sdiag & 1)) SRC(coocc_fps_voxels(lin_q, Q, d->X, d->Y, d->Z, d->fps_num, w.rep[dd], w.fps[dd], w.fps_bytes, st));
     hipLaunchKernelGGL(k_gather_xyz, dim3(cdiv(d->fps_num, 256)), dim3(256), 0, as_stream(st), xyz_q, w.rep[dd], d->fps_num, w.rep_xyz[dd]);
     COOCC_LAUNCH_CHECK("k_gather_xyz");
     SRC(coocc_knn_topk_voxels(d->fps_num, Nk, K, d->X, d->Y, d->Z, w.rep[dd], lin_q, map_k, d->offsets, d->noff, w.rep_xyz[dd], xyz_k,
diff --git a/co_occ_amd/fuser.py b/co_occ_amd/fuser.py
--- a/co_occ_amd/fuser.py
+++ b/co_occ_amd/fuser.py
@@ -175,6 +175,8 @@
         self.knum = knum
         self.near = torch.zeros(2, knum * V, device=device, dtype=_I32)
         self._native = None
+        h2 = _core_mod.CONV_ENGINE == "h2" and _core_mod.H2_DIRECT and C % 32 == 0
+        self.g1_h2 = torch.empty(V, 2 * C, device=device, dtype=_F32) if h2 else None
 
     def img_rows(self):
         X, Y, Z = self.grid
@@ -198,6 +200,7 @@
             d.ws, d.ws_bytes = ws.data_ptr(), need
             host = (ctypes.c_int32 * 2)()
             d.counts_host = ctypes.addressof(host)
+            d.g1_h2 = self.g1_h2.data_ptr() if self.g1_h2 is not None else None
             self._native = (d, ws, host, off)
         return self._native
 
@@ -304,7 +307,8 @@
             img = img_r if img_r is not None else img_voxel_feats.float().contiguous()
             pts = pts_r if pts_r is not None else pts_voxel_feats.float().contiguous()
             src = lambda r: (r.data(), 1, r.stride) if isinstance(r, Rows) else (ptr(r), 0, 0)
-            call("coocc_fuser_prepare_rows", *src(img), *src(pts), ptr(cat4), ptr(flags[0]), ptr(flags[1]), B, C, V)
+            call("coocc_fuser_prepare_rows_h2", *src(img), *src(pts), ptr(cat4), ptr(flags[0]), ptr(flags[1]), B, C, V,
+                 ptr(slot.g1_h2 if slot is not None else None))
         assert slot is None or (img_r is not None or pts_r is not None), "search(slot=...) takes channels-last producers"
         lin = slot.lin if slot is not None else torch.empty(2, B * V, device=dev, dtype=_I32)
         counts = slot.counts if slot is not None else torch.empty(2, device=dev, dtype=_I32)
@@ -407,11 +411,13 @@
             self.last_near = (sr.near_img, sr.near_pts)
         return sr.cat4, (sr.lin_img, sr.lin_pts)
 
-    def _g1_h2(self, cat4, packs):
+    def _g1_h2(self, cat4, packs, slot=None):
         import os
         from . import core
         if os.environ.get("COOCC_G1_H2_ONCE", "1") == "0":
             return None
+        if slot is not None and slot.g1_h2 is not None and core.g1_h2_capable(packs["knn"], self.in_channels):
+            return (slot.g1_h2, 0, 2 * self.in_channels)
         sh = core.g1_sources_h2(cat4, self.in_channels, packs["knn"])
         return None if sh is None else (sh, 0, 2 * self.in_channels)
 
@@ -419,7 +425,7 @@
         C = self.in_channels
         packs = self._packed()
         cat4 = slot.cat4
-        h2 = self._g1_h2(cat4, packs)
+        h2 = self._g1_h2(cat4, packs, slot)
         gather_conv_rows(cat4, 0, packs["knn"], slot.rows, slot.lin[1], cat4, 2 * C, C, C, count_dev=slot.counts[1:2], src_h2=h2)
         gather_conv_rows(cat4, C, packs["knn"], slot.rows_p, slot.lin[0], cat4, 3 * C, 0, C, count_dev=slot.counts[0:1], src_h2=h2)
         X, Y, Z = slot.grid
diff --git a/co_occ_amd/serving.py b/co_occ_amd/serving.py
--- a/co_occ_amd/serving.py
+++ b/co_occ_amd/serving.py
@@ -6,7 +6,7 @@
 
 import torch
 
-from . import core, graph as cg, streams as cstreams_
+from . import _lib, core, graph as cg, streams as cstreams_
 
 CAM_KEYS = ("rots", "trans", "intrins", "post_rots", "post_trans", "bda")
 
@@ -111,14 +111,11 @@
     def _copy_in(self, k, fr):
         st = self.static[k]
         st["img_feats"][0].copy_(fr["img_feats"][0], non_blocking=True)
-        if st["cams"] is not None:
-            for d, s in zip(st["cams"], fr["cams"]):
-                d.copy_(s, non_blocking=True)
-        for d, s in zip(st["transform"][:-1], fr["transform"][:-1]):
-            if torch.is_tensor(d):
-                d.copy_(s, non_blocking=True)
+        pairs = list(zip(st["cams"], fr["cams"])) if st["cams"] is not None else []
+        pairs += [(d, s) for d, s in zip(st["transform"][:-1], fr["transform"][:-1]) if torch.is_tensor(d)]
         if st["gemo"] is not None:
-            st["gemo"].copy_(fr["gemo"], non_blocking=True)
+            pairs.append((st["gemo"], fr["gemo"]))
+        _lib.copy_many(pairs)
 
     def _mark(self, t, tag):
         if self.trace is not None:
diff --git a/include/coocc_hip.h b/include/coocc_hip.h
--- a/include/coocc_hip.h
+++ b/include/coocc_hip.h
@@ -39,11 +39,15 @@
 int coocc_fuser_prepare_rows(const float* img, int img_rows, int img_stride, const float* pts, int pts_rows,
                              int pts_stride, float* cat4, uint8_t* flag_img, uint8_t* flag_pts, int B, int C, int V,
                              void* stream);
+int coocc_fuser_prepare_rows_h2(const float* img, int img_rows, int img_stride, const float* pts, int pts_rows,
+                                int pts_stride, float* cat4, uint8_t* flag_img, uint8_t* flag_pts, int B, int C, int V,
+                                void* out_h2, void* stream);
 
 int coocc_compact_flags(const uint8_t* flags, int total, int32_t* lin, int32_t* count, void* ws,
                         size_t ws_bytes, void* stream);
 int coocc_compact_flags_ex(const uint8_t* flags, int total, int32_t* lin, int32_t* count, int32_t* map, void* ws,
                            size_t ws_bytes, void* stream);
+int coocc_copy_many(const void* const* src, void* const* dst, const int64_t* bytes, int n, void* stream);
 int coocc_lin_to_coords(const int32_t* lin, int n, int X, int Y, int Z, float* xyz, int64_t* bxyz,
                         void* stream);
 
@@ -56,6 +60,10 @@
                      size_t ws_bytes, void* stream);
 int coocc_fps_voxels_pair(const int32_t* lin0, int n0, int32_t* idx0, void* ws0, const int32_t* lin1, int n1, int32_t* idx1,
                           void* ws1, size_t ws_bytes_each, int X, int Y, int Z, int m, void* stream);
+int coocc_fps_voxels_pair_ex(const int32_t* lin0, int n0, int32_t* idx0, void* ws0, const int32_t* lin1, int n1, int32_t* idx1,
+                             void* ws1, size_t ws_bytes_each, int X, int Y, int Z, int m, int tables_ready, void* stream);
+int coocc_search_tables(const int32_t* lin0, int n0, const int32_t* map0, float* xyz0, void* cell0, const int32_t* lin1, int n1,
+                        const int32_t* map1, float* xyz1, void* cell1, size_t ws_bytes_each, int X, int Y, int Z, void* stream);
 
 int coocc_ball_query(int b, int n, int m, float min_radius, float max_radius, int nsample,
                      const float* new_xyz, const float* xyz, int32_t* idx, void* stream);
@@ -79,9 +87,35 @@
   void* ws;
   size_t ws_bytes;
   int32_t* counts_host;
+  void* g1_h2;
 } coocc_search_desc;
 size_t coocc_fuser_search_ws(const coocc_search_desc* d);
 int coocc_fuser_search(coocc_search_desc* d, void* stream, void* side_stream);
+
+typedef struct coocc_vox_search_dir {
+  const int32_t* rep;
+  const int32_t* lin_q;
+  const int32_t* map_q;
+  const int32_t* map_k;
+  const float* xyz_q;
+  const float* xyz_k;
+  float* val;
+  int32_t* nn;
+  int32_t* group;
+  int32_t* winner;
+  int32_t* near;
+  const int32_t* base;
+  int32_t* rows;
+  int nbase, rows_stride, nq, nk;
+} coocc_vox_search_dir;
+typedef struct coocc_vox_search_pair {
+  coocc_vox_search_dir dir[2];
+  int ndir;
+  int m, K, nsample, X, Y, Z, noff;
+  float min_radius, max_radius, dist_thresh;
+  const uint32_t* offsets;
+} coocc_vox_search_pair;
+int coocc_voxel_search_pair(const coocc_vox_search_pair* a, void* stream);
 
 int coocc_voxel_index_map(const int32_t* lin, int n, int nvox, int32_t* map, void* stream);
 int coocc_voxel_index_map_dev(const int32_t* lin, int n_cap, const int32_t* n_dev, int nvox, int32_t* map, void* stream);
```

After: 266.9. 1.1% lower.
